# google/speedy

Measured on AMD Instinct MI355X. Metric: Msamples/s processed (16 kHz mono, 3.5x nonlinear), higher is better.
Workload: dtype int16 samples; f64 DFT, f32 features, int32 AMDF/OLA

## Files before the change

include/speedy_hip.h:

```cpp
#ifndef SPEEDY_HIP_H_
#define SPEEDY_HIP_H_
#include <stddef.h>
#include <stdint.h>
#ifdef __cplusplus
extern "C" {
#endif

#ifndef SPX_FEATURE_COUNT
#define SPX_FEATURE_COUNT 15
#endif

typedef struct spx_plan* spx_plan_t;

typedef struct {
  int64_t in_off;
  int64_t n_in;
  int64_t out_off;
  int64_t out_cap;
  int32_t channels;
  float speed;
  float nonlinear;
  float feedback;
} spx_stream_job;

typedef struct {
  float* tension;
  float* speed;
  float* features;
  float* spectrogram;
  float* normalized;
} spx_taps;

const char* spx_last_error(void);
int spx_abi_version(void);

spx_plan_t spx_plan_create(int sample_rate, int match_matlab);
void spx_plan_destroy(spx_plan_t plan);
int spx_plan_frame_step(spx_plan_t plan);
int spx_plan_window_size(spx_plan_t plan);
int spx_plan_fft_size(spx_plan_t plan);
int spx_plan_future(spx_plan_t plan);
int spx_plan_max_required(spx_plan_t plan);
int64_t spx_plan_frames(spx_plan_t plan, int64_t n_in);
int64_t spx_plan_out_capacity(spx_plan_t plan, int64_t n_in, float speed);
int64_t spx_plan_out_capacity_for(spx_plan_t plan, int64_t n_in, float speed, float nonlinear);

size_t spx_batch_workspace_bytes(spx_plan_t plan, const spx_stream_job* jobs, int n_streams);

int spx_batch_run(spx_plan_t plan, const spx_stream_job* jobs, int n_streams, const int16_t* in,
                  int16_t* out, int64_t* n_out, void* workspace, size_t workspace_bytes,
                  const spx_taps* taps, void* hip_stream);

int spx_batch_run_rate(spx_plan_t plan, const spx_stream_job* jobs, const float* rates, int n_streams, const int16_t* in,
                       int16_t* out, int64_t* n_out, void* workspace, size_t workspace_bytes,
                       const spx_taps* taps, void* hip_stream);
size_t spx_batch_workspace_bytes_rate(spx_plan_t plan, const spx_stream_job* jobs, const float* rates, int n_streams);
int64_t spx_plan_out_capacity_rate(spx_plan_t plan, int64_t n_in, float speed, float nonlinear, float rate);

int64_t spx_plan_map_rows(spx_plan_t plan, int64_t n_in, float nonlinear);
int spx_batch_run_map(spx_plan_t plan, const spx_stream_job* jobs, int n_streams, const int16_t* in,
                      int16_t* out, int64_t* n_out, int64_t* map, void* workspace, size_t workspace_bytes,
                      const spx_taps* taps, void* hip_stream);
int spx_map_lookup(spx_plan_t plan, const spx_stream_job* jobs, int n_streams, const int64_t* map, const int64_t* q_off,
                   const int64_t* q, int64_t* r, int inverse, void* hip_stream);
int spx_batch_run_rate_map(spx_plan_t plan, const spx_stream_job* jobs, const float* rates, int n_streams, const int16_t* in,
                           int16_t* out, int64_t* n_out, int64_t* map, void* workspace, size_t workspace_bytes,
                           const spx_taps* taps, void* hip_stream);
int spx_batch_run_float_map(spx_plan_t plan, const spx_stream_job* jobs, const float* rates, int n_streams, const float* in,
                            float* out, int64_t* n_out, int64_t* map, void* workspace, size_t workspace_bytes,
                            const spx_taps* taps, void* hip_stream);

typedef struct { int32_t out_at, a, b, n; } spx_edit_op;
typedef struct { int64_t in_off, out_off; int32_t channels, reserved; } spx_edit_track;
int64_t spx_plan_edit_ops(spx_plan_t plan, int64_t n_in, float speed, float nonlinear);
int spx_batch_run_edits(spx_plan_t plan, const spx_stream_job* jobs, int n_streams, const int16_t* in, int16_t* out, int64_t* n_out,
                        spx_edit_op* ops, const int64_t* ops_cap, int64_t* n_ops, void* workspace, size_t workspace_bytes,
                        const spx_taps* taps, void* hip_stream);
int spx_edit_replay(spx_plan_t plan, const spx_stream_job* jobs, int n_streams, const spx_edit_op* ops, const int64_t* ops_cap,
                    const int64_t* n_ops, const int64_t* n_out, const spx_edit_track* tracks, const int16_t* y_in, int16_t* y_out,
                    void* hip_stream);

typedef struct { int64_t a_off, b_off; int64_t path_off; int32_t n_a, n_b; } spx_dtw_job;
typedef struct { float cost, slope, local_mean, local_std; int32_t n_path, n_local; } spx_dtw_result;
size_t spx_dtw_workspace_bytes(const spx_dtw_job* jobs, int n_pairs, int dim);
int spx_batch_dtw(spx_plan_t plan, const spx_dtw_job* jobs, int n_pairs, int dim, int ld_a, int ld_b, int half_width,
                  const float* a, const float* b, spx_dtw_result* results, int32_t* path,
                  void* workspace, size_t workspace_bytes, void* hip_stream);

size_t spx_batch_workspace_bytes_twopass(spx_plan_t plan, const spx_stream_job* jobs, const double* seconds, int n_streams);
int64_t spx_plan_out_capacity_twopass(spx_plan_t plan, int64_t n_in, double want, float nonlinear);
int spx_batch_run_twopass(spx_plan_t plan, const spx_stream_job* jobs, const double* seconds, int n_streams, const int16_t* in,
                          int16_t* out, int64_t* n_out, int64_t* n_probe, float* speeds, void* workspace, size_t workspace_bytes,
                          const spx_taps* taps, void* hip_stream);
int spx_debug_last_twopass(void);

size_t spx_batch_workspace_bytes_float(spx_plan_t plan, const spx_stream_job* jobs, const float* rates, int n_streams);
int spx_batch_run_float(spx_plan_t plan, const spx_stream_job* jobs, const float* rates, int n_streams, const float* in,
                        float* out, int64_t* n_out, void* workspace, size_t workspace_bytes,
                        const spx_taps* taps, void* hip_stream);
int spx_float_to_short(const float* in, int16_t* out, size_t n, int nonlinear_scale, void* hip_stream);
int spx_short_to_float(const int16_t* in, float* out, size_t n, void* hip_stream);

int spx_batch_run_ahead(spx_plan_t plan, const spx_stream_job* jobs, int n_streams, const int16_t* in,
                        int16_t* out, int64_t* n_out, void* workspace, size_t workspace_bytes,
                        const spx_taps* taps, void* hip_stream);

int spx_batch_run_overlapped(spx_plan_t plan, const spx_stream_job* jobs, int n_streams, const int16_t* in,
                             int16_t* out, int64_t* n_out, void* workspace, size_t workspace_bytes,
                             const spx_taps* taps, void* hip_stream);

int spx_batch_run_ahead_when(spx_plan_t plan, const spx_stream_job* jobs, int n_streams, const int16_t* in,
                             int16_t* out, int64_t* n_out, void* workspace, size_t workspace_bytes,
                             const spx_taps* taps, void* hip_stream, void* in_ready_event);

typedef struct spx_pipeline* spx_pipeline_t;
#define SPX_PIPELINE_DEVICE_OUT 1u
#define SPX_PIPELINE_FLOAT 2u
spx_pipeline_t spx_pipeline_create(spx_plan_t plan, const spx_stream_job* jobs, int n_streams, int depth, unsigned flags);
spx_pipeline_t spx_pipeline_create_mixed(const spx_plan_t* plans, int n_plans, const spx_stream_job* jobs, const int* plan_index,
                                         int n_streams, int depth, unsigned flags);
void spx_pipeline_destroy(spx_pipeline_t p);
int spx_pipeline_depth(spx_pipeline_t p);
size_t spx_pipeline_input_values(spx_pipeline_t p);
int16_t* spx_pipeline_host_input(spx_pipeline_t p);
int64_t spx_pipeline_submit(spx_pipeline_t p, const int16_t* in, int in_is_device);
int64_t spx_pipeline_submit_jobs(spx_pipeline_t p, const spx_stream_job* jobs, const int16_t* in, int in_is_device);
int spx_pipeline_jobs_fit(spx_pipeline_t p, const spx_stream_job* jobs);
int spx_pipeline_input_consumed(spx_pipeline_t p, int64_t ticket);
int spx_pipeline_wait(spx_pipeline_t p, int64_t ticket, const int16_t** out, const int64_t** offsets, const int64_t** counts);

float* spx_pipeline_host_input_float(spx_pipeline_t p);
int64_t spx_pipeline_submit_float(spx_pipeline_t p, const float* in, int in_is_device);
int64_t spx_pipeline_submit_jobs_float(spx_pipeline_t p, const spx_stream_job* jobs, const float* in, int in_is_device);
int spx_pipeline_wait_float(spx_pipeline_t p, int64_t ticket, const float** out, const int64_t** offsets, const int64_t** counts);

spx_pipeline_t spx_pipeline_create_rate(spx_plan_t plan, const spx_stream_job* jobs, const float* rates, int n_streams, int depth,
                                        unsigned flags);
int spx_pipeline_jobs_fit_rate(spx_pipeline_t p, const spx_stream_job* jobs, const float* rates);
int64_t spx_pipeline_submit_jobs_rate(spx_pipeline_t p, const spx_stream_job* jobs, const float* rates, const int16_t* in,
                                      int in_is_device);
int64_t spx_pipeline_submit_jobs_rate_float(spx_pipeline_t p, const spx_stream_job* jobs, const float* rates, const float* in,
                                            int in_is_device);

void* spx_host_alloc(size_t bytes);
void spx_host_free(void* p);

int spx_batch_analyze(spx_plan_t plan, const spx_stream_job* jobs, int n_streams, const int16_t* in,
                      void* workspace, size_t workspace_bytes, const spx_taps* taps, void* hip_stream);
int spx_batch_walk(spx_plan_t plan, const spx_stream_job* jobs, int n_streams, const int16_t* in,
                   int16_t* out, int64_t* n_out, void* workspace, size_t workspace_bytes,
                   const spx_taps* taps, void* hip_stream);

size_t spx_batch_workspace_bytes_mixed(const spx_plan_t* plans, int n_plans, const spx_stream_job* jobs,
                                       const int* plan_index, int n_streams);
int spx_batch_run_mixed(const spx_plan_t* plans, int n_plans, const spx_stream_job* jobs, const int* plan_index,
                        int n_streams, const int16_t* in, int16_t* out, int64_t* n_out, void* workspace,
                        size_t workspace_bytes, void* hip_stream);

int spx_batch_run_mixed_taps(const spx_plan_t* plans, int n_plans, const spx_stream_job* jobs, const int* plan_index,
                             int n_streams, const int16_t* in, int16_t* out, int64_t* n_out, void* workspace,
                             size_t workspace_bytes, const spx_taps* taps, void* hip_stream);
int spx_batch_run_mixed_ahead(const spx_plan_t* plans, int n_plans, const spx_stream_job* jobs, const int* plan_index,
                              int n_streams, const int16_t* in, int16_t* out, int64_t* n_out, void* workspace,
                              size_t workspace_bytes, void* hip_stream);

void spx_set_timing(int enabled);
void spx_set_pipeline_chunks(int chunks);
void spx_set_concurrent(int on);
void spx_set_tension_form(int form);
int spx_debug_last_tension_form(void);
int spx_debug_last_call_chunks(void);
int spx_debug_last_lookup_grid(int* launches);
int spx_debug_last_replay_grid(int* launches);
int spx_debug_last_dtw_grid(int* launches);
int spx_timing_collect(double* sum_ms_analyze, double* sum_ms_walk, int* n_calls);
const char* spx_batch_kernel_names(spx_plan_t plan, int n_streams, int max_channels, int speedup_only);
const char* spx_batch_kernel_names_lean(spx_plan_t plan, int n_streams, int max_channels, int speedup_only);
int spx_debug_last_walk_form(void);
int spx_debug_kernel_vgprs(int which);
int spx_debug_walk_info(int sample_rate, int channels, int n_streams, int speedup_only, int short_jobs, int lean, int* out5);
int spx_debug_analysis_info(int sample_rate, int* out4);
int spx_debug_lane_consts(int sample_rate, void* out, double* tw, double* tw2, float* win);
int spx_debug_mode_resources(int sample_rate, int channels, int n_streams, int speedup_only, long long* out22);
long long spx_debug_fdiv_check(unsigned seed, unsigned denominators, int exp_lo, int exp_hi);
long long spx_debug_xfade_check(int n_lo, int n_hi);
long long spx_debug_arith_check(unsigned seed, unsigned threads, unsigned per_thread);
int spx_debug_select_check(const unsigned* d, int n_vectors, int p0, int n_lags, int max_period, int two_per_lane, int* lag_index,
                           unsigned* kmin);
int spx_debug_select_fold_check(const unsigned* d, int n_vectors, int p0, int n_lags, int want_max, int fresh, int* out3);
int spx_debug_log_check(unsigned first_block, unsigned end_block, unsigned long long* sums);
int spx_debug_last_call_concurrent(void);
double spx_timing_last_tension_ms(void);
double spx_timing_last_rate_ms(void);
double spx_timing_last_map_rows_ms(void);
double spx_timing_last_dtw_ms(void);
double spx_timing_last_dtw_tail_ms(void);

int spx_batch_read_steps(spx_plan_t plan, const spx_stream_job* jobs, int n_streams, const void* workspace,
                         int32_t* steps, void* hip_stream);
int spx_batch_read_steps_mixed(const spx_plan_t* plans, int n_plans, const spx_stream_job* jobs, const int* plan_index,
                               int n_streams, const void* workspace, int32_t* steps, void* hip_stream);

void* spx_device_alloc(size_t bytes);
void spx_device_free(void* p);
int spx_batch_pack_outputs(const spx_stream_job* jobs, int n_streams, const int16_t* out, const int64_t* n_out,
                           int16_t* packed, int64_t* offsets, void* hip_stream);
int spx_copy_to_device(void* dst, const void* src, size_t bytes, void* hip_stream);
int spx_copy_to_host(void* dst, const void* src, size_t bytes, void* hip_stream);
int spx_stream_synchronize(void* hip_stream);

#ifdef __cplusplus
}
#endif
#endif
```

speedy_amd/_lib.py:

```python
import ctypes as C
import os
import subprocess

_HERE = os.path.dirname(os.path.abspath(__file__))
LIB_PATH = os.environ.get("SPEEDY_HIP_LIB") or os.path.join(_HERE, "lib", "libspeedy_hip.so")
_LIB = None

c_short_p = C.POINTER(C.c_short)
c_float_p = C.POINTER(C.c_float)
c_int64_p = C.POINTER(C.c_int64)


class StreamJob(C.Structure):
    _fields_ = [("in_off", C.c_int64), ("n_in", C.c_int64), ("out_off", C.c_int64), ("out_cap", C.c_int64),
                ("channels", C.c_int32), ("speed", C.c_float), ("nonlinear", C.c_float), ("feedback", C.c_float)]


class Taps(C.Structure):
    _fields_ = [("tension", C.c_void_p), ("speed", C.c_void_p), ("features", C.c_void_p),
                ("spectrogram", C.c_void_p), ("normalized", C.c_void_p)]


class EditTrack(C.Structure):
    _fields_ = [("in_off", C.c_int64), ("out_off", C.c_int64), ("channels", C.c_int32), ("reserved", C.c_int32)]


class DtwJob(C.Structure):
    _fields_ = [("a_off", C.c_int64), ("b_off", C.c_int64), ("path_off", C.c_int64), ("n_a", C.c_int32), ("n_b", C.c_int32)]


TENSION_FN =C.CFUNCTYPE(None, C.c_void_p, C.c_int, C.c_float)
FEATURES_FN = C.CFUNCTYPE(None, C.c_void_p, C.c_int, c_float_p)

SYMBOLS = {
    "spx_last_error": (C.c_char_p, []),
    "spx_abi_version": (C.c_int, []),
    "spx_plan_create": (C.c_void_p, [C.c_int, C.c_int]),
    "spx_plan_destroy": (None, [C.c_void_p]),
    "spx_plan_frame_step": (C.c_int, [C.c_void_p]),
    "spx_plan_window_size": (C.c_int, [C.c_void_p]),
    "spx_plan_fft_size": (C.c_int, [C.c_void_p]),
    "spx_plan_future": (C.c_int, [C.c_void_p]),
    "spx_plan_max_required": (C.c_int, [C.c_void_p]),
    "spx_plan_frames": (C.c_int64, [C.c_void_p, C.c_int64]),
    "spx_plan_out_capacity": (C.c_int64, [C.c_void_p, C.c_int64, C.c_float]),
    "spx_plan_out_capacity_for": (C.c_int64, [C.c_void_p, C.c_int64, C.c_float, C.c_float]),
    "spx_batch_workspace_bytes": (C.c_size_t, [C.c_void_p, C.POINTER(StreamJob), C.c_int]),
    "spx_batch_run": (C.c_int, [C.c_void_p, C.POINTER(StreamJob), C.c_int, C.c_void_p, C.c_void_p, C.c_void_p,
                                C.c_void_p, C.c_size_t, C.POINTER(Taps), C.c_void_p]),
    "spx_batch_run_rate": (C.c_int, [C.c_void_p, C.POINTER(StreamJob), c_float_p, C.c_int, C.c_void_p, C.c_void_p, C.c_void_p,
                                     C.c_void_p, C.c_size_t, C.POINTER(Taps), C.c_void_p]),
    "spx_batch_workspace_bytes_rate": (C.c_size_t, [C.c_void_p, C.POINTER(StreamJob), c_float_p, C.c_int]),
    "spx_plan_out_capacity_rate": (C.c_int64, [C.c_void_p, C.c_int64, C.c_float, C.c_float, C.c_float]),
    "spx_plan_map_rows": (C.c_int64, [C.c_void_p, C.c_int64, C.c_float]),
    "spx_batch_run_map": (C.c_int, [C.c_void_p, C.POINTER(StreamJob), C.c_int, C.c_void_p, C.c_void_p, C.c_void_p, C.c_void_p,
                                    C.c_void_p, C.c_size_t, C.POINTER(Taps), C.c_void_p]),
    "spx_map_lookup": (C.c_int, [C.c_void_p, C.POINTER(StreamJob), C.c_int, C.c_void_p, C.c_void_p, C.c_void_p, C.c_void_p,
                                 C.c_int, C.c_void_p]),
    "spx_batch_run_rate_map": (C.c_int, [C.c_void_p, C.POINTER(StreamJob), c_float_p, C.c_int, C.c_void_p, C.c_void_p, C.c_void_p,
                                         C.c_void_p, C.c_void_p, C.c_size_t, C.POINTER(Taps), C.c_void_p]),
    "spx_batch_run_float_map": (C.c_int, [C.c_void_p, C.POINTER(StreamJob), c_float_p, C.c_int, C.c_void_p, C.c_void_p, C.c_void_p,
                                          C.c_void_p, C.c_void_p, C.c_size_t, C.POINTER(Taps), C.c_void_p]),
    "spx_plan_edit_ops": (C.c_int64, [C.c_void_p, C.c_int64, C.c_float, C.c_float]),
    "spx_batch_run_edits": (C.c_int, [C.c_void_p, C.POINTER(StreamJob), C.c_int, C.c_void_p, C.c_void_p, C.c_void_p, C.c_void_p,
                                      c_int64_p, C.c_void_p, C.c_void_p, C.c_size_t, C.POINTER(Taps), C.c_void_p]),
    "spx_edit_replay": (C.c_int, [C.c_void_p, C.POINTER(StreamJob), C.c_int, C.c_void_p, c_int64_p, C.c_void_p, C.c_void_p,
                                  C.POINTER(EditTrack), C.c_void_p, C.c_void_p, C.c_void_p]),
    "spx_dtw_workspace_bytes": (C.c_size_t, [C.POINTER(DtwJob), C.c_int, C.c_int]),
    "spx_batch_dtw": (C.c_int, [C.c_void_p, C.POINTER(DtwJob), C.c_int, C.c_int, C.c_int, C.c_int, C.c_int, C.c_void_p, C.c_void_p,
                                C.c_void_p, C.c_void_p, C.c_void_p, C.c_size_t, C.c_void_p]),
    "spx_debug_last_dtw_grid": (C.c_int, [C.POINTER(C.c_int)]),
    "spx_timing_last_dtw_ms": (C.c_double, []),
    "spx_timing_last_dtw_tail_ms": (C.c_double, []),
    "spx_batch_workspace_bytes_twopass":(C.c_size_t, [C.c_void_p, C.POINTER(StreamJob), C.POINTER(C.c_double), C.c_int]),
    "spx_plan_out_capacity_twopass": (C.c_int64, [C.c_void_p, C.c_int64, C.c_double, C.c_float]),
    "spx_batch_run_twopass": (C.c_int, [C.c_void_p, C.POINTER(StreamJob), C.POINTER(C.c_double), C.c_int, C.c_void_p, C.c_void_p,
                                        C.c_void_p, C.c_void_p, C.c_void_p, C.c_void_p, C.c_size_t, C.POINTER(Taps), C.c_void_p]),
    "spx_debug_last_twopass": (C.c_int, []),
    "spx_batch_workspace_bytes_float": (C.c_size_t, [C.c_void_p, C.POINTER(StreamJob), c_float_p, C.c_int]),
    "spx_batch_run_float": (C.c_int, [C.c_void_p, C.POINTER(StreamJob), c_float_p, C.c_int, C.c_void_p, C.c_void_p, C.c_void_p,
                                      C.c_void_p, C.c_size_t, C.POINTER(Taps), C.c_void_p]),
    "spx_float_to_short": (C.c_int, [C.c_void_p, C.c_void_p, C.c_size_t, C.c_int, C.c_void_p]),
    "spx_short_to_float": (C.c_int, [C.c_void_p, C.c_void_p, C.c_size_t, C.c_void_p]),
    "spx_batch_run_ahead": (C.c_int, [C.c_void_p, C.POINTER(StreamJob), C.c_int, C.c_void_p, C.c_void_p, C.c_void_p,
                                      C.c_void_p, C.c_size_t, C.POINTER(Taps), C.c_void_p]),
    "spx_batch_run_overlapped": (C.c_int, [C.c_void_p, C.POINTER(StreamJob), C.c_int, C.c_void_p, C.c_void_p, C.c_void_p,
                                           C.c_void_p, C.c_size_t, C.POINTER(Taps), C.c_void_p]),
    "spx_batch_run_ahead_when": (C.c_int, [C.c_void_p, C.POINTER(StreamJob), C.c_int, C.c_void_p, C.c_void_p, C.c_void_p,
                                           C.c_void_p, C.c_size_t, C.POINTER(Taps), C.c_void_p, C.c_void_p]),
    "spx_batch_workspace_bytes_mixed": (C.c_size_t, [C.POINTER(C.c_void_p), C.c_int, C.POINTER(StreamJob), C.POINTER(C.c_int), C.c_int]),
    "spx_batch_run_mixed": (C.c_int, [C.POINTER(C.c_void_p), C.c_int, C.POINTER(StreamJob), C.POINTER(C.c_int), C.c_int,
                                      C.c_void_p, C.c_void_p, C.c_void_p, C.c_void_p, C.c_size_t, C.c_void_p]),
    "spx_batch_run_mixed_ahead": (C.c_int, [C.POINTER(C.c_void_p), C.c_int, C.POINTER(StreamJob), C.POINTER(C.c_int), C.c_int,
                                      C.c_void_p, C.c_void_p, C.c_void_p, C.c_void_p, C.c_size_t, C.c_void_p]),
    "spx_batch_run_mixed_taps": (C.c_int, [C.POINTER(C.c_void_p), C.c_int, C.POINTER(StreamJob), C.POINTER(C.c_int), C.c_int,
                                           C.c_void_p, C.c_void_p, C.c_void_p, C.c_void_p, C.c_size_t, C.POINTER(Taps), C.c_void_p]),
    "spx_batch_read_steps": (C.c_int, [C.c_void_p, C.POINTER(StreamJob), C.c_int, C.c_void_p, C.POINTER(C.c_int32), C.c_void_p]),
    "spx_batch_read_steps_mixed": (C.c_int, [C.POINTER(C.c_void_p), C.c_int, C.POINTER(StreamJob), C.POINTER(C.c_int), C.c_int,
                                             C.c_void_p, C.POINTER(C.c_int32), C.c_void_p]),
    "spx_batch_analyze": (C.c_int, [C.c_void_p, C.POINTER(StreamJob), C.c_int, C.c_void_p, C.c_void_p,
                                    C.c_size_t, C.POINTER(Taps), C.c_void_p]),
    "spx_batch_walk": (C.c_int, [C.c_void_p, C.POINTER(StreamJob), C.c_int, C.c_void_p, C.c_void_p, C.c_void_p,
                                 C.c_void_p, C.c_size_t, C.POINTER(Taps), C.c_void_p]),
    "spx_set_timing": (None, [C.c_int]),
    "spx_set_pipeline_chunks": (None, [C.c_int]),
    "spx_set_concurrent": (None, [C.c_int]),
    "spx_set_tension_form": (None, [C.c_int]),
    "spx_debug_last_tension_form": (C.c_int, []),
    "spx_debug_last_call_chunks": (C.c_int, []),
    "spx_debug_last_lookup_grid": (C.c_int, [C.POINTER(C.c_int)]),
    "spx_debug_last_replay_grid": (C.c_int, [C.POINTER(C.c_int)]),
    "spx_timing_collect": (C.c_int, [C.POINTER(C.c_double), C.POINTER(C.c_double), C.POINTER(C.c_int)]),
    "spx_timing_last_tension_ms": (C.c_double, []),
    "spx_timing_last_rate_ms": (C.c_double, []),
    "spx_timing_last_map_rows_ms": (C.c_double, []),
    "spx_batch_kernel_names": (C.c_char_p, [C.c_void_p, C.c_int, C.c_int, C.c_int]),
    "spx_batch_kernel_names_lean": (C.c_char_p, [C.c_void_p, C.c_int, C.c_int, C.c_int]),
    "spx_debug_last_walk_form": (C.c_int, []),
    "spx_debug_kernel_vgprs": (C.c_int, [C.c_int]),
    "spx_debug_last_call_concurrent": (C.c_int, []),
    "spx_debug_fdiv_check": (C.c_longlong, [C.c_uint, C.c_uint, C.c_int, C.c_int]),
    "spx_debug_xfade_check": (C.c_longlong, [C.c_int, C.c_int]),
    "spx_debug_select_check": (C.c_int, [C.POINTER(C.c_uint), C.c_int, C.c_int, C.c_int, C.c_int, C.c_int, C.POINTER(C.c_int), C.POINTER(C.c_uint)]),
    "spx_debug_select_fold_check": (C.c_int, [C.POINTER(C.c_uint), C.c_int, C.c_int, C.c_int, C.c_int, C.c_int, C.POINTER(C.c_int)]),
    "spx_debug_arith_check": (C.c_longlong, [C.c_uint, C.c_uint, C.c_uint]),
    "spx_debug_log_check": (C.c_int, [C.c_uint, C.c_uint, C.POINTER(C.c_ulonglong)]),
    "spx_debug_walk_info": (C.c_int, [C.c_int, C.c_int, C.c_int, C.c_int, C.c_int, C.c_int, C.POINTER(C.c_int)]),
    "spx_debug_analysis_info": (C.c_int, [C.c_int, C.POINTER(C.c_int)]),
    "spx_debug_lane_consts": (C.c_int, [C.c_int, C.c_void_p, C.POINTER(C.c_double), C.POINTER(C.c_double), c_float_p]),
    "spx_debug_mode_resources": (C.c_int, [C.c_int, C.c_int, C.c_int, C.c_int, C.POINTER(C.c_longlong)]),
    "spx_pipeline_create": (C.c_void_p, [C.c_void_p, C.POINTER(StreamJob), C.c_int, C.c_int, C.c_uint]),
    "spx_pipeline_create_mixed": (C.c_void_p, [C.POINTER(C.c_void_p), C.c_int, C.POINTER(StreamJob), C.POINTER(C.c_int), C.c_int, C.c_int, C.c_uint]),
    "spx_pipeline_destroy": (None, [C.c_void_p]),
    "spx_pipeline_depth": (C.c_int, [C.c_void_p]),
    "spx_pipeline_input_values": (C.c_size_t, [C.c_void_p]),
    "spx_pipeline_host_input": (C.c_void_p, [C.c_void_p]),
    "spx_pipeline_submit": (C.c_int64, [C.c_void_p, C.c_void_p, C.c_int]),
    "spx_pipeline_submit_jobs": (C.c_int64, [C.c_void_p, C.POINTER(StreamJob), C.c_void_p, C.c_int]),
    "spx_pipeline_jobs_fit": (C.c_int, [C.c_void_p, C.POINTER(StreamJob)]),
    "spx_pipeline_input_consumed": (C.c_int, [C.c_void_p, C.c_int64]),
    "spx_pipeline_wait": (C.c_int, [C.c_void_p, C.c_int64, C.POINTER(C.c_void_p), C.POINTER(C.c_void_p), C.POINTER(C.c_void_p)]),
    "spx_pipeline_host_input_float": (C.c_void_p, [C.c_void_p]),
    "spx_pipeline_submit_float": (C.c_int64, [C.c_void_p, C.c_void_p, C.c_int]),
    "spx_pipeline_submit_jobs_float": (C.c_int64, [C.c_void_p, C.POINTER(StreamJob), C.c_void_p, C.c_int]),
    "spx_pipeline_wait_float": (C.c_int, [C.c_void_p, C.c_int64, C.POINTER(C.c_void_p), C.POINTER(C.c_void_p), C.POINTER(C.c_void_p)]),
    "spx_pipeline_create_rate": (C.c_void_p, [C.c_void_p, C.POINTER(StreamJob), c_float_p, C.c_int, C.c_int, C.c_uint]),
    "spx_pipeline_jobs_fit_rate": (C.c_int, [C.c_void_p, C.POINTER(StreamJob), c_float_p]),
    "spx_pipeline_submit_jobs_rate": (C.c_int64, [C.c_void_p, C.POINTER(StreamJob), c_float_p, C.c_void_p, C.c_int]),
    "spx_pipeline_submit_jobs_rate_float": (C.c_int64, [C.c_void_p, C.POINTER(StreamJob), c_float_p, C.c_void_p, C.c_int]),
    "spx_host_alloc": (C.c_void_p, [C.c_size_t]),
    "spx_host_free": (None, [C.c_void_p]),
    "spx_device_alloc": (C.c_void_p, [C.c_size_t]),
    "spx_device_free": (None, [C.c_void_p]),
    "spx_copy_to_device": (C.c_int, [C.c_void_p, C.c_void_p, C.c_size_t, C.c_void_p]),
    "spx_copy_to_host": (C.c_int, [C.c_void_p, C.c_void_p, C.c_size_t, C.c_void_p]),
    "spx_batch_pack_outputs": (C.c_int, [C.c_void_p, C.c_int, C.c_void_p, C.c_void_p, C.c_void_p, C.c_void_p, C.c_void_p]),
    "spx_stream_synchronize": (C.c_int, [C.c_void_p]),
    "sonicCreateStream": (C.c_void_p, [C.c_int, C.c_int]),
    "sonicDestroyStream": (None, [C.c_void_p]),
    "sonicWriteShortToStream": (C.c_int, [C.c_void_p, c_short_p, C.c_int]),
    "sonicReadShortFromStream": (C.c_int, [C.c_void_p, c_short_p, C.c_int]),
    "sonicWriteFloatToStream": (C.c_int, [C.c_void_p, c_float_p, C.c_int]),
    "sonicReadFloatFromStream": (C.c_int, [C.c_void_p, c_float_p, C.c_int]),
    "sonicSetRate": (None, [C.c_void_p, C.c_float]),
    "sonicSetSpeed": (None, [C.c_void_p, C.c_float]),
    "sonicFlushStream": (C.c_int, [C.c_void_p]),
    "sonicEnableNonlinearSpeedup": (None, [C.c_void_p, C.c_float]),
    "sonicSetDurationFeedbackStrength": (None, [C.c_void_p, C.c_float]),
    "getSonicBufferSize": (C.c_int, [C.c_void_p]),
    "sonicSpectrogramSize": (C.c_int, [C.c_void_p]),
    "sonicTensionCallback": (None, [C.c_void_p, TENSION_FN]),
    "getSonicTensionCallback": (C.c_void_p, [C.c_void_p]),
    "sonicSpeedCallback": (None, [C.c_void_p, TENSION_FN]),
    "getSonicSpeedCallback": (C.c_void_p, [C.c_void_p]),
    "sonicFeaturesCallback": (None, [C.c_void_p, FEATURES_FN]),
    "getSonicFeaturesCallback": (C.c_void_p, [C.c_void_p]),
    "sonicSpectrogramCallback": (None, [C.c_void_p, FEATURES_FN]),
    "getSonicSpectrogramCallback": (C.c_void_p, [C.c_void_p]),
    "sonicNormalizedSpectrogramCallback": (None, [C.c_void_p, FEATURES_FN]),
    "getSonicNormalizedSpectrogramCallback": (C.c_void_p, [C.c_void_p]),
    "sonicIntGetNumChannels": (C.c_int, [C.c_void_p]),
    "sonicIntGetSampleRate": (C.c_int, [C.c_void_p]),
    "sonicIntGetSpeed": (C.c_float, [C.c_void_p]),
    "sonicIntCreateStream": (C.c_void_p, [C.c_int, C.c_int]),
    "sonicIntDestroyStream": (None, [C.c_void_p]),
    "sonicIntSetSpeed": (None, [C.c_void_p, C.c_float]),
    "sonicIntSetRate": (None, [C.c_void_p, C.c_float]),
    "sonicIntWriteShortToStream": (C.c_int, [C.c_void_p, c_short_p, C.c_int]),
    "sonicIntWriteFloatToStream": (C.c_int, [C.c_void_p, c_float_p, C.c_int]),
    "sonicIntReadShortFromStream": (C.c_int, [C.c_void_p, c_short_p, C.c_int]),
    "sonicIntReadFloatFromStream": (C.c_int, [C.c_void_p, c_float_p, C.c_int]),
    "sonicIntFlushStream": (C.c_int, [C.c_void_p]),
    "sonicIntSamplesAvailable": (C.c_int, [C.c_void_p]),
    "sonicIntSetUserData": (None, [C.c_void_p, C.c_void_p]),
    "sonicIntGetUserData": (C.c_void_p, [C.c_void_p]),
    "speedyCreateStream": (C.c_void_p, [C.c_int]),
    "speedyDestroyStream": (None, [C.c_void_p]),
    "speedyInputFrameSize": (C.c_int, [C.c_void_p]),
    "speedyInputFrameStep": (C.c_int, [C.c_void_p]),
    "speedyFFTSize": (C.c_int, [C.c_void_p]),
    "speedyBinToFreq": (C.c_float, [C.c_void_p, C.c_int]),
    "speedyFreqToBin": (C.c_int, [C.c_void_p, C.c_float]),
    "speedyAddData": (None, [C.c_void_p, c_float_p, C.c_int64]),
    "speedyAddDataShort": (None, [C.c_void_p, c_short_p, C.c_int64]),
    "speedyComputeTension": (C.c_int, [C.c_void_p, C.c_int64, c_float_p]),
    "speedyComputeSpeedFromTension": (C.c_float, [C.c_float, C.c_float, C.c_float, C.c_void_p]),
    "speedyGetCurrentTime": (C.c_int64, [C.c_void_p]),
    "speedySpectrogram": (c_float_p, [C.c_void_p, c_float_p]),
    "speedyGetSpectrogram": (c_float_p, [C.c_void_p]),
    "speedyGetSpectrogramAtTime": (c_float_p, [C.c_void_p, C.c_int64]),
    "speedyGetNormalizedSpectrogram": (c_float_p, [C.c_void_p]),
    "speedyGetInternalState": (c_float_p, [C.c_void_p]),
    "speedyGetEnergyCompressed": (C.c_float, [C.c_void_p]),
    "speedyGetSpeechChanges": (C.c_float, [C.c_void_p]),
    "speedyHipHysteresisFuture": (C.c_int, [C.c_void_p]),
    "speedyHipHysteresisPast": (C.c_int, [C.c_void_p]),
    "speedyComputeSpectralDifference": (None, [C.c_void_p, c_float_p, c_float_p, C.c_int64]),
    "speedyComputeLocalEnergy": (None, [C.c_void_p, c_float_p, C.c_int64]),
    "speedySaveSpectrogramData": (None, [C.c_void_p, c_float_p, C.c_int64]),
    "speedyPreemphasisFilter": (None, [C.c_void_p, c_float_p, C.c_int]),
    "speedyEvaluateHysteresis": (C.c_float, [C.c_void_p, C.c_int64]),
    "speedyAddToHysteresisBuffer": (None, [C.c_void_p, C.c_float, C.c_int64]),
    "speedyGetInternalSpectrogram": (c_float_p, [C.c_void_p]),
    "speedyGetInternalNormalizedSpectrogram": (c_float_p, [C.c_void_p]),
    "speedyNormalizeByEnergy": (C.c_float, [c_float_p, c_float_p, C.c_int]),
    "CreateFirstOrderFilter": (C.c_void_p, [C.c_float]),
    "DesignFirstOrderLowpassFilter": (None, [C.c_void_p, C.c_float]),
    "IterateFirstOrderFilter": (C.c_float, [C.c_void_p, C.c_float]),
    "ResetFirstOrderFilter": (None, [C.c_void_p]),
    "DeleteFirstOrderFilter": (None, [C.c_void_p]),
    "speedyHipSetMatchMatlab": (None, [C.c_int]),
    "speedyHipCreateSonicStream": (C.c_void_p, [C.c_int, C.c_int, C.c_int]),
    "speedyHipSetCoalescing": (None, [C.c_int]),
    "speedyHipGetCoalescing": (C.c_int, []),
    "speedyHipCreateSonicStreamEx": (C.c_void_p, [C.c_int, C.c_int, C.c_int, C.c_int]),
    "speedyHipPoolStats": (None, [C.POINTER(C.c_ulonglong), C.POINTER(C.c_ulonglong)]),
    "sonicSamplesAvailable": (C.c_int, [C.c_void_p]),
    "speedyHipLastError": (C.c_char_p, []),
}


def build():
    subprocess.check_call(["make", "-s", "-C", os.path.join(_HERE, "csrc")])


def lib():
    global _LIB
    if _LIB is not None:
        return _LIB
    if not os.path.exists(LIB_PATH):
        raise RuntimeError(f"{LIB_PATH} is missing: run `python -c 'import __graft_entry__ as g; g.build()'` "
                           "(the product has no CPU fallback)")
    import torch
    L = C.CDLL(LIB_PATH)
    for name, (res, args) in SYMBOLS.items():
        if os.environ.get("SPEEDY_HIP_LIB") and not hasattr(L, name):
            continue
        fn = getattr(L, name)
        fn.restype = res
        fn.argtypes = args
    _LIB = L
# ... 2 lines not shown
```

speedy_amd/csrc/spx_analysis.hip:

```cpp
#include <stdlib.h>

#include "spx_internal.h"
#include "spx_walk_common.h"

#ifndef SPX_TF
#define SPX_TF 16
#endif

#ifdef SPX_STAMPS
__device__ unsigned long long g_spx_astamps[16];
#define ASTAMP_DECL unsigned long long as_last = __builtin_readcyclecounter(), as_acc[10] = {0,0,0,0,0,0,0,0,0,0};
#define ASTAMP(i) do { const unsigned long long t_ = __builtin_readcyclecounter(); as_acc[i] += t_ - as_last; as_last = t_; } while (0)
#define ASTAMP_FLUSH if (threadIdx.x == 0 && blockIdx.x == 7) for (int i_ = 0; i_ < 10; i_++) g_spx_astamps[i_] += as_acc[i_];
extern "C" void spx_debug_astamps(unsigned long long* out, int reset) {
  (void)hipMemcpyFromSymbol(out, HIP_SYMBOL(g_spx_astamps), sizeof(unsigned long long) * 16);
  if (reset) { unsigned long long z[16] = {0}; (void)hipMemcpyToSymbol(HIP_SYMBOL(g_spx_astamps), z, sizeof(z)); }
}
#else
#define ASTAMP_DECL
#define ASTAMP(i)
#define ASTAMP_FLUSH
#endif

#ifndef SPX_TF_SMALL
// ... 267 lines not shown
  } else if constexpr (R == 3) {
    const cplx t1 = {a[1].r + a[2].r, a[1].i + a[2].i};
    const cplx t2 = {spx_bf3h(a[0].r, t1.r), spx_bf3h(a[0].i, t1.i)};
    const cplx t3 = {S3_1 * (a[1].r - a[2].r), S3_1 * (a[1].i - a[2].i)};
    o[0] = {a[0].r + t1.r, a[0].i + t1.i};
    o[1] = {t2.r + t3.i, t2.i - t3.r};
    o[2] = {t2.r - t3.i, t2.i + t3.r};
  } else if constexpr (R == 4) {
    const cplx t0 = {a[0].r + a[2].r, a[0].i + a[2].i}, t1 = {a[0].r - a[2].r, a[0].i - a[2].i};
    const cplx t2 = {a[1].r + a[3].r, a[1].i + a[3].i}, t3 = {a[1].r - a[3].r, a[1].i - a[3].i};
    o[0] = {t0.r + t2.r, t0.i + t2.i};
    o[2] = {t0.r - t2.r, t0.i - t2.i};
    o[1] = {t1.r + t3.i, t1.i - t3.r};
    o[3] = {t1.r - t3.i, t1.i + t3.r};
  } else {
    const cplx t1 = {a[1].r + a[4].r, a[1].i + a[4].i}, t2 = {a[2].r + a[3].r, a[2].i + a[3].i};
    const cplx t3 = {a[1].r - a[4].r, a[1].i - a[4].i}, t4 = {a[2].r - a[3].r, a[2].i - a[3].i};
    o[0] = {(a[0].r + t1.r) + t2.r, (a[0].i + t1.i) + t2.i};
    const cplx m1 = {spx_bf5m(a[0].r, C5_1, t1.r, C5_2, t2.r), spx_bf5m(a[0].i, C5_1, t1.i, C5_2, t2.i)};
    const cplx m2 = {spx_bf5m(a[0].r, C5_2, t1.r, C5_1, t2.r), spx_bf5m(a[0].i, C5_2, t1.i, C5_1, t2.i)};
    const cplx n1 = {spx_bf5n(S5_1, t3.r, S5_2, t4.r), spx_bf5n(S5_1, t3.i, S5_2, t4.i)};
    const cplx n2 = {spx_bf5d(S5_2, t3.r, S5_1, t4.r), spx_bf5d(S5_2, t3.i, S5_1, t4.i)};
    o[1] = {m1.r + n1.i, m1.i - n1.r};
    o[4] = {m1.r - n1.i, m1.i + n1.r};
    o[2] = {m2.r + n2.i, m2.i - n2.r};
    o[3] = {m2.r - n2.i, m2.i + n2.r};
  }
}

template <int W> struct ct_plan { static constexpr int n = 0; };
template <> struct ct_plan<120> { static constexpr int n = 4; static constexpr int r[4] = {4, 2, 3, 5}; };
template <> struct ct_plan<180> { static constexpr int n = 4; static constexpr int r[4] = {4, 3, 3, 5}; };
template <> struct ct_plan<360> { static constexpr int n = 5; static constexpr int r[5] = {4, 2, 3, 3, 5}; };
template <> struct ct_plan<480> { static constexpr int n = 5; static constexpr int r[5] = {4, 4, 2, 3, 5}; };
template <> struct ct_plan<720> { static constexpr int n = 5; static constexpr int r[5] = {4, 4, 3, 3, 5}; };

template <int NPTS, int R, int S, class Load>
__device__ __forceinline__ void ct_stage(double* buf, const double2* __restrict__ twp, const int lane, Load load) {
  constexpr int SPAN = NPTS / R, NP = (SPAN + 63) / 64;
  constexpr bool LAST = (S * R == NPTS);
  cplx a[NP][R];
#pragma unroll
  for (int u = 0; u < NP; u++) {
#pragma unroll
    for (int i = 0; i < R; i++) a[u][i] = load(u, i);
  }
  wave_sync();
#pragma unroll
  for (int u = 0; u < NP; u++) {
    const int b = lane + 64 * u;
    if (b < SPAN) {
      cplx o[R];
      ct_bfly<R>(a[u], o);
      const int p = b / S, q = b - p * S;
      const int base = q + S * R * p, tp = S * p;
      st(buf, base, o[0]);
#pragma unroll
      for (int j = 1; j < R; j++) st(buf, base + j * S, LAST ? o[j] : cmul_tw(o[j], twp[j * tp]));
    }
  }
  wave_sync();
}
template <int NPTS, int R>
struct ct_from_buf {
  const double* buf;
  int lane;
  __device__ __forceinline__ cplx operator()(int u, int i) const {
    constexpr int SPAN = NPTS / R;
    const int b = (lane + 64 * u < SPAN) ? lane + 64 * u : 0;
    return ld(buf, b + i * SPAN);
  }
};

template <int W, int ST, int S>
__device__ __forceinline__ void ct_stages_from(double* buf, const double2* __restrict__ twp, const int lane) {
  if constexpr (ST < ct_plan<W>::n) {
    constexpr int R = ct_plan<W>::r[ST];
    ct_stage<W, R, S>(buf, twp, lane, ct_from_buf<W, R>{buf, lane});
    ct_stages_from<W, ST + 1, S * R>(buf, twp, lane);
  }
}

template <int NPTS, int R>
__device__ __forceinline__ void ct_stage_prime_last(double* buf, const int lane, const double (&wc)[R - 1], const double (&ws)[R - 1]) {
  constexpr int SPAN = NPTS / R, H = (R - 1) / 2;
  static_assert(SPAN <= 64, "one pass");
  if (lane < SPAN) {
    cplx a[R];
#pragma unroll
    for (int i = 0; i < R; i++) a[i] = ld(buf, lane + SPAN * i);
    cplx uu[H], vv[H];
    cplx B0 = a[0];
#pragma unroll
    for (int i = 1; i <= H; i++) {
      uu[i - 1] = {a[i].r + a[R - i].r, a[i].i + a[R - i].i};
      vv[i - 1] = {a[i].r - a[R - i].r, a[i].i - a[R - i].i};
      B0.r = B0.r + uu[i - 1].r; B0.i = B0.i + uu[i - 1].i;
    }
    st(buf, lane, B0);
#pragma unroll
    for (int jj = 1; jj <= H; jj++) {
      cplx Pj = a[0], Qj = {0.0, 0.0};
#pragma unroll
      for (int i = 1; i <= H; i++) {
        const double wx = wc[(i * jj) % R - 1], wy = ws[(i * jj) % R - 1];
        Pj.r = spx_acc(Pj.r, wx, uu[i - 1].r); Pj.i = spx_acc(Pj.i, wx, uu[i - 1].i);
        if (i == 1) { Qj.r = wy * vv[0].r; Qj.i = wy * vv[0].i; }
        else { Qj.r = spx_acc(Qj.r, wy, vv[i - 1].r); Qj.i = spx_acc(Qj.i, wy, vv[i - 1].i); }
      }
      st(buf, lane + SPAN * jj, cplx{Pj.r - Qj.i, Pj.i + Qj.r});
      st(buf, lane + SPAN * (R - jj), cplx{Pj.r + Qj.i, Pj.i - Qj.r});
    }
  }
  wave_sync();
}

template <class T>
__device__ __forceinline__ const T* per_frame(const T* p) {
  asm volatile("" : "+s"(p));
  return p;
}
__device__ __forceinline__ double uniform_f64(double v) {
  return __longlong_as_double(((long long)__builtin_amdgcn_readfirstlane((int)(__double_as_longlong(v) >> 32)) << 32) |
                              (unsigned)__builtin_amdgcn_readfirstlane((int)__double_as_longlong(v)));
}

#ifdef SPX_PREEMPH_V1
__device__ __forceinline__ float spx_preemph_win_f32(double md, double mpd, float w) {
  const float x = (float)(md / 32768.0), xp = (float)(mpd / 32768.0);
  const float y = (float)(1.0 * (double)x - 0.97 * (double)xp);
  return y * w;
}
#else
__device__ __forceinline__ float spx_preemph_win_f32(double md, double mpd, float w15) {
  const float yy = (float)(md - 0.97 * mpd);
  return yy * w15;
}
#endif
__device__ __forceinline__ double spx_preemph_win(double md, double mpd, float w) { return (double)spx_preemph_win_f32(md, mpd, w); }
__device__ __forceinline__ cplx packed_point(const short* fr, int n, int j, int prev0, float w0, float w1) {
  const int i0 = 2 * n;
  const int m0 = fr[i0], m1 = fr[i0 + 1];
  const int mp0 = (i0 > 0) ? (int)fr[i0 - 1] : ((j > 0) ? (int)fr[prev0] : 0);
  const double d0 = (double)m0;
  return {spx_preemph_win(d0, (double)mp0, w0 * SPX_WIN_SCALE), spx_preemph_win((double)m1, d0, w1 * SPX_WIN_SCALE)};
}

#ifndef SPX_AN_W_330
#define SPX_AN_W_330 3
#endif
#ifndef SPX_AN_W_BIG
#define SPX_AN_W_BIG 2
#endif
template <int TF, int WCT>
__global__ void __launch_bounds__(SPX_BLOCK, an_lean_layout(TF, WCT) ? 5 : (WCT == 240 || WCT == 120 || WCT == 180) ? 4 : WCT == 330 ? SPX_AN_W_330 : (WCT == 661 || WCT == 720) ? SPX_AN_W_BIG : (WCT == 480 || WCT == 360) ? 2 : 1)
spx_analysis_kernel(SpxPlanDev P, const SpxStreamDev* __restrict__ streams, int n_streams,
                    const int16_t* __restrict__ in_base, SpxFrameRec* __restrict__ rec, SpxTapsDev taps,
                    const int* __restrict__ tile_order, int* tile_flags, const float* __restrict__ frames,
                    int frame_mode) {
  extern __shared__ __attribute__((aligned(16))) unsigned char lds[];
  const int W = WCT ? WCT : P.W, B = P.B, N = 2 * W;
  const int tid = threadIdx.x, lane = tid & 63, wave = tid >> 6;

  const int tile = tile_order ? tile_order[blockIdx.x] : (int)blockIdx.x;
  int lo = 0, hi = n_streams - 1;
  while (lo < hi) {
    int mid = (lo + hi + 1) >> 1;
    if (streams[mid].first_tile <= tile) lo = mid; else hi = mid - 1;
  }
  const SpxStreamDev S = streams[lo];
  const int T = S.n_frames;
  const int j0 = S.frame_begin + (tile - S.first_tile) * TF;
  const int j1 = min(j0 + TF, T);
  const int C = S.channels;
  const int16_t* __restrict__ in = in_base + S.in_off;

  constexpr bool LT = an_lean_layout(TF, WCT);
  const size_t wb = work_bytes(W, TF, WCT != 0, (WCT != 0) ? 4 : P.dft_waves);
  const size_t mags_b = (((size_t)(TF + 1) * spx_mag_stride(W) * sizeof(float)) + 15) & ~(size_t)15;
  const size_t small_b = (((size_t)3 * (TF + 1) * sizeof(float)) + 15) & ~(size_t)15;
  double* work = reinterpret_cast<double*>(LT ? lds + an_lt_front_bytes() : lds);
  float* mags = reinterpret_cast<float*>(LT ? lds : lds + wb);
  float* fE = reinterpret_cast<float*>(LT ? lds + an_lt_front_bytes() + an_lt_small_off() : lds + wb + mags_b);
  float* fThr = fE + (TF + 1);
  float* fInv = fThr + (TF + 1);
  const int MS = spx_mag_stride(W);
  unsigned char* const terms_base = reinterpret_cast<unsigned char*>(work) + (LT ? an_lt_terms_off() : 0);
  static_assert(!LT || an_lt_terms_off() + (size_t)2 * SPX_TF * (spx_cb(SPX_TF) + 1) * sizeof(double) + SPX_LOG_LDS_BYTES <= (size_t)4 * 2 * 240 * sizeof(double),
                "two blocks of log terms and the log table inside the work area (terms_bytes, work_bytes)");

  const double* ltw = P.tw;
  const double* ltw2 = P.tw2;
  short* smono = reinterpret_cast<short*>(LT ? lds + an_lt_front_bytes() + wb : lds + wb + mags_b + small_b);
  const bool direct = LT && frame_mode == 3;

  double* bufA = work + (size_t)wave * (WCT != 0 ? 2 : 4) * W;
  double* bufB = (WCT != 0) ? bufA : bufA + 2 * W;

  const int jfirst = (j0 > 0) ? j0 - 1 : 0;
  const int64_t sbase = (int64_t)jfirst * B;
  const int nstage = (j1 - jfirst) * B + (W - B);
  if (frames != nullptr || direct) {
  } else if (C == 1) {
    const int16_t* __restrict__ src = in + sbase;
    for (int k0 = tid; k0 < nstage; k0 += 8 * SPX_BLOCK) {
      short v[8];
#pragma unroll
      for (int u = 0; u < 8; u++) { const int k = k0 + u * SPX_BLOCK; v[u] = (k < nstage) ? src[k] : (short)0; }
#pragma unroll
      for (int u = 0; u < 8; u++) { const int k = k0 + u * SPX_BLOCK; if (k < nstage) smono[k] = v[u]; }
    }
  } else {
    for (int k = tid; k < nstage; k += SPX_BLOCK) smono[k] = (short)mono_sample(in, sbase + k, C);
  }
  __syncthreads();

  ASTAMP_DECL
  if constexpr (LT) {
    const int b = lane;
    const bool on60 = b < 60, on48 = b < 48;
    const int bb = on60 ? b : 0;
    typedef double lc_v2d __attribute__((ext_vector_type(2)));
    typedef float lc_v4f __attribute__((ext_vector_type(4)));
    typedef const __attribute__((address_space(1))) lc_v2d* lc_ptr;
    typedef const __attribute__((address_space(1))) lc_v4f* lc_ptr4;
    const double2* const lc0 = reinterpret_cast<const double2*>(P.lane_consts);
    auto take6 = [&](auto fr, int j, int (&m)[6]) {
      m[0] = fr[0]; m[1] = fr[1]; m[2] = fr[120]; m[3] = fr[121]; m[5] = fr[119];
      m[4] = fr[bb > 0 ? -1 : (240 - B) - 1];
      if (bb == 0 && j == 0) m[4] = 0;
    };
    auto fetch6 = [&](int s, int (&m)[6]) {
      const int j = j0 - 1 + s;
      if (s <= TF && j >= 0 && j < j1) take6(in + (int64_t)j * B + 2 * bb, j, m);
    };
    int nx[6] = {0, 0, 0, 0, 0, 0};
    float hold[4] = {0.0f, 0.0f, 0.0f, 0.0f};
    if (direct) fetch6(wave, nx);
    for (int s = wave; s <= TF; s += 4) {
      const int j = j0 - 1 + s;
      const bool keep = s + 4 > TF;
      float* mrow = mags + (size_t)s * MS;
      if (j < 0 || j >= j1) {
        if (!keep) for (int k = lane; k < 240; k += SPX_WAVE) mrow[k] = 0.0f;
#pragma unroll
        for (int u = 0; u < 4; u++) hold[u] = 0.0f;
        if (direct) fetch6(s + 4, nx);
        continue;
      }
      int ln = lane;
      asm volatile("" : "+v"(ln));
      __builtin_assume(ln >= 0 && ln < SPX_WAVE);
      const lc_ptr lcb[4] = {(lc_ptr)per_frame(lc0), (lc_ptr)per_frame(lc0 + 256), (lc_ptr)per_frame(lc0 + 512), (lc_ptr)per_frame(lc0 + 768)};
      typedef const __attribute__((address_space(1))) unsigned char* lc_bytes;
      unsigned lane_off = 16u * (unsigned)lane;
      asm volatile("" : "+v"(lane_off));
      auto lc = [&](int c) -> double2 {
        const lc_v2d v = *(lc_ptr)((lc_bytes)lcb[c >> 2] + lane_off + 1024u * (unsigned)(c & 3));
        return make_double2(v.x, v.y);
      };
      int m[6];
      if (direct) {
#pragma unroll
        for (int u = 0; u < 6; u++) m[u] = nx[u];
      } else {
        take6(smono + (size_t)(j - jfirst) * B + 2 * bb, j, m);
      }
      {
        const lc_v4f wn = *(lc_ptr4)((lc_bytes)lcb[SPX_LC_WN >> 2] + lane_off + 1024u * (SPX_LC_WN & 3));
        const double2 w1a = lc(SPX_LC_W1 + 0), w1b = lc(SPX_LC_W1 + 1), w1c = lc(SPX_LC_W1 + 2);
        if (on60) {
          const double d0 = (double)m[0], d2 = (double)m[2];
          const cplx a0 = {spx_preemph_win(d0, (double)m[4], wn.x), spx_preemph_win((double)m[1], d0, wn.y)},
                     a1 = {spx_preemph_win(d2, (double)m[5], wn.z), spx_preemph_win((double)m[3], d2, wn.w)};
          const cplx b0 = {a0.r + a1.r, a0.i + a1.i}, b2 = {a0.r - a1.r, a0.i - a1.i};
          const cplx b1 = {a0.r + a1.i, a0.i - a1.r}, b3 = {a0.r - a1.i, a0.i + a1.r};
          st(bufA, 4 * ln, b0);
          st(bufA, 4 * ln + 1, cmul_tw(b1, w1a));
          st(bufA, 4 * ln + 2, cmul_tw(b2, w1b));
          st(bufA, 4 * ln + 3, cmul_tw(b3, w1c));
        }
      }
      {
        const double2 w2a = lc(SPX_LC_W2 + 0), w2b = lc(SPX_LC_W2 + 1), w2c = lc(SPX_LC_W2 + 2);
        wave_sync();
        ASTAMP(0);
        if (on60) {
          const cplx a0 = ld(bufA, ln), a1 = ld(bufA, ln + 60), a2 = ld(bufA, ln + 120), a3 = ld(bufA, ln + 180);
          wave_sync();
          const cplx t0 = {a0.r + a2.r, a0.i + a2.i}, t1 = {a0.r - a2.r, a0.i - a2.i};
          const cplx t2 = {a1.r + a3.r, a1.i + a3.i}, t3 = {a1.r - a3.r, a1.i - a3.i};
          const cplx b0 = {t0.r + t2.r, t0.i + t2.i}, b2 = {t0.r - t2.r, t0.i - t2.i};
          const cplx b1 = {t1.r + t3.i, t1.i - t3.r}, b3 = {t1.r - t3.i, t1.i + t3.r};
          const int o = (ln & 3) + 16 * (ln >> 2);
          st(bufB, o, b0);
          st(bufB, o + 4, cmul_tw(b1, w2a));
          st(bufB, o + 8, cmul_tw(b2, w2b));
          st(bufB, o + 12, cmul_tw(b3, w2c));
        }
      }
      {
        double2 w3[2][2];
#pragma unroll
        for (int u = 0; u < 2; u++) { w3[u][0] = lc(SPX_LC_W3 + 2 * u); w3[u][1] = lc(SPX_LC_W3 + 2 * u + 1); }
        wave_sync();
        cplx q0[2], q1[2], q2[2];
#pragma unroll
        for (int u = 0; u < 2; u++) {
          const int b3i = (ln + 64 * u < 80) ? ln + 64 * u : 0;
          q0[u] = ld(bufB, b3i); q1[u] = ld(bufB, b3i + 80); q2[u] = ld(bufB, b3i + 160);
        }
        wave_sync();
#pragma unroll
        for (int u = 0; u < 2; u++) {
          const int b3i = ln + 64 * u;
          if (b3i < 80) {
            const cplx a0 = q0[u], a1 = q1[u], a2 = q2[u];
            const cplx t1 = {a1.r + a2.r, a1.i + a2.i};
            const cplx t2 = {spx_bf3h(a0.r, t1.r), spx_bf3h(a0.i, t1.i)};
            const cplx t3 = {S3_1 * (a1.r - a2.r), S3_1 * (a1.i - a2.i)};
            const cplx b0 = {a0.r + t1.r, a0.i + t1.i};
            const cplx b1 = {t2.r + t3.i, t2.i - t3.r}, b2 = {t2.r - t3.i, t2.i + t3.r};
            const int o = (b3i & 15) + 48 * (b3i >> 4);
            st(bufA, o, b0);
            st(bufA, o + 16, cmul_tw(b1, w3[u][0]));
            st(bufA, o + 32, cmul_tw(b2, w3[u][1]));
          }
        }
      }
      wave_sync();
      if (on48) {
        const cplx a0 = ld(bufA, ln), a1 = ld(bufA, ln + 48), a2 = ld(bufA, ln + 96), a3 = ld(bufA, ln + 144),
                   a4 = ld(bufA, ln + 192);
        wave_sync();
        const cplx t1 = {a1.r + a4.r, a1.i + a4.i}, t2 = {a2.r + a3.r, a2.i + a3.i};
        const cplx t3 = {a1.r - a4.r, a1.i - a4.i}, t4 = {a2.r - a3.r, a2.i - a3.i};
        const cplx b0 = {(a0.r + t1.r) + t2.r, (a0.i + t1.i) + t2.i};
        const cplx m1 = {spx_bf5m(a0.r, C5_1, t1.r, C5_2, t2.r), spx_bf5m(a0.i, C5_1, t1.i, C5_2, t2.i)};
        const cplx m2 = {spx_bf5m(a0.r, C5_2, t1.r, C5_1, t2.r), spx_bf5m(a0.i, C5_2, t1.i, C5_1, t2.i)};
        const cplx n1 = {spx_bf5n(S5_1, t3.r, S5_2, t4.r), spx_bf5n(S5_1, t3.i, S5_2, t4.i)};
        const cplx n2 = {spx_bf5d(S5_2, t3.r, S5_1, t4.r), spx_bf5d(S5_2, t3.i, S5_1, t4.i)};
        const cplx b1 = {m1.r + n1.i, m1.i - n1.r}, b4 = {m1.r - n1.i, m1.i + n1.r};
        const cplx b2 = {m2.r + n2.i, m2.i - n2.r}, b3 = {m2.r - n2.i, m2.i + n2.r};
        st(bufB, ln, b0);
        st(bufB, ln + 48, b1);
        st(bufB, ln + 96, b2);
        st(bufB, ln + 144, b3);
        st(bufB, ln + 192, b4);
      }
      if (direct) fetch6(s + 4, nx);
      double2 wu[4];
#pragma unroll
      for (int u = 0; u < 4; u++) wu[u] = lc(SPX_LC_WU + u);
      wave_sync();
      ASTAMP(1);
      float* spec_out = taps.spectrogram ? taps.spectrogram + (size_t)(S.frame_off + j) * 480 : nullptr;
#pragma unroll
      for (int u = 0; u < 4; u++) {
        const int k = ln + 64 * u;
        if (k < 240) {
          const int k2 = (k == 0) ? 0 : 240 - k;
          const cplx a = ld(bufB, k), c = ld(bufB, k2);
          const double b_r = c.r, b_i = -c.i;
          const float mag = spx_untangle_mag(a.r, a.i, b_r, b_i, wu[u]);
          hold[u] = mag;
          if (!keep) mrow[k] = mag;
          if (spec_out) {
            spec_out[k] = mag;
            if (k > 0) spec_out[480 - k] = mag;
            else spec_out[240] = (float)__builtin_fabs(a.r - a.i);
          }
        }
      }
      wave_sync();
      ASTAMP(2);
    }
    __syncthreads();
    {
      float* mrow = mags + (size_t)(wave == 0 ? TF : TF - 4 + wave) * MS;
#pragma unroll
      for (int u = 0; u < 4; u++) {
        const int k = lane + 64 * u;
        if (k < 240) mrow[k] = hold[u];
      }
    }
  } else if constexpr (WCT == 240) {
    const double2* twp = reinterpret_cast<const double2*>(P.tw);
    const double2* tw2p = reinterpret_cast<const double2*>(P.tw2);
    const int b = lane;
    const bool on60 = b < 60, on48 = b < 48;
    const int bb = on60 ? b : 0;
    double2 w1[3], w2[3], w3[2][2], wu[4];
    float wn[4];
#pragma unroll
    for (int j = 1; j < 4; j++) { w1[j - 1] = twp[bb * j]; w2[j - 1] = twp[4 * (bb >> 2) * j]; }
#pragma unroll
    for (int u = 0; u < 2; u++) {
      const int b3 = lane + 64 * u, p3 = (b3 < 80) ? (b3 >> 4) : 0;
      w3[u][0] = twp[16 * p3];
      w3[u][1] = twp[32 * p3];
    }
#pragma unroll
    for (int u = 0; u < 4; u++) { const int k = lane + 64 * u; wu[u] = tw2p[k < 240 ? k : 0]; }
    wn[0] = P.window[2 * bb]; wn[1] = P.window[2 * bb + 1]; wn[2] = P.window[2 * bb + 120]; wn[3] = P.window[2 * bb + 121];
#pragma unroll
    for (int k = 0; k < 4; k++) wn[k] *= SPX_WIN_SCALE;
    for (int s = wave; s <= TF; s += 4) {
      const int j = j0 - 1 + s;
      float* mrow = mags + (size_t)s * MS;
      if (j < 0 || j >= j1) {
        for (int k = lane; k < 240; k += SPX_WAVE) mrow[k] = 0.0f;
        continue;
      }
      const short* fr = smono + (size_t)(j - jfirst) * B;
      if (on60) {
        const int i0 = 2 * b, i1 = 2 * b + 120;
        const int m0 = fr[i0], m1 = fr[i0 + 1], m2 = fr[i1], m3 = fr[i1 + 1];
        const int mp0 = (i0 > 0) ? (int)fr[i0 - 1] : ((j > 0) ? (int)fr[(240 - B) - 1] : 0);
        const int mp2 = fr[i1 - 1];
        const double d0 = (double)m0, d2 = (double)m2;
        const cplx a0 = {spx_preemph_win(d0, (double)mp0, wn[0]), spx_preemph_win((double)m1, d0, wn[1])},
                   a1 = {spx_preemph_win(d2, (double)mp2, wn[2]), spx_preemph_win((double)m3, d2, wn[3])};
        const cplx b0 = {a0.r + a1.r, a0.i + a1.i}, b2 = {a0.r - a1.r, a0.i - a1.i};
        const cplx b1 = {a0.r + a1.i, a0.i - a1.r}, b3 = {a0.r - a1.i, a0.i + a1.r};
        st(bufA, 4 * b, b0);
        st(bufA, 4 * b + 1, cmul_tw(b1, w1[0]));
        st(bufA, 4 * b + 2, cmul_tw(b2, w1[1]));
        st(bufA, 4 * b + 3, cmul_tw(b3, w1[2]));
      }
      wave_sync();
      ASTAMP(0);
      if (on60) {
        const cplx a0 = ld(bufA, b), a1 = ld(bufA, b + 60), a2 = ld(bufA, b + 120), a3 = ld(bufA, b + 180);
        wave_sync();
        const cplx t0 = {a0.r + a2.r, a0.i + a2.i}, t1 = {a0.r - a2.r, a0.i - a2.i};
        const cplx t2 = {a1.r + a3.r, a1.i + a3.i}, t3 = {a1.r - a3.r, a1.i - a3.i};
        const cplx b0 = {t0.r + t2.r, t0.i + t2.i}, b2 = {t0.r - t2.r, t0.i - t2.i};
        const cplx b1 = {t1.r + t3.i, t1.i - t3.r}, b3 = {t1.r - t3.i, t1.i + t3.r};
        const int o = (b & 3) + 16 * (b >> 2);
        st(bufB, o, b0);
        st(bufB, o + 4, cmul_tw(b1, w2[0]));
        st(bufB, o + 8, cmul_tw(b2, w2[1]));
        st(bufB, o + 12, cmul_tw(b3, w2[2]));
      }
      wave_sync();
      {
        cplx q0[2], q1[2], q2[2];
#pragma unroll
        for (int u = 0; u < 2; u++) {
          const int b3i = (lane + 64 * u < 80) ? lane + 64 * u : 0;
          q0[u] = ld(bufB, b3i); q1[u] = ld(bufB, b3i + 80); q2[u] = ld(bufB, b3i + 160);
        }
        wave_sync();
#pragma unroll
        for (int u = 0; u < 2; u++) {
          const int b3i = lane + 64 * u;
          if (b3i < 80) {
            const cplx a0 = q0[u], a1 = q1[u], a2 = q2[u];
            const cplx t1 = {a1.r + a2.r, a1.i + a2.i};
            const cplx t2 = {spx_bf3h(a0.r, t1.r), spx_bf3h(a0.i, t1.i)};
            const cplx t3 = {S3_1 * (a1.r - a2.r), S3_1 * (a1.i - a2.i)};
            const cplx b0 = {a0.r + t1.r, a0.i + t1.i};
            const cplx b1 = {t2.r + t3.i, t2.i - t3.r}, b2 = {t2.r - t3.i, t2.i + t3.r};
            const int o = (b3i & 15) + 48 * (b3i >> 4);
            st(bufA, o, b0);
            st(bufA, o + 16, cmul_tw(b1, w3[u][0]));
            st(bufA, o + 32, cmul_tw(b2, w3[u][1]));
          }
        }
      }
      wave_sync();
      if (on48) {
        const cplx a0 = ld(bufA, b), a1 = ld(bufA, b + 48), a2 = ld(bufA, b + 96), a3 = ld(bufA, b + 144),
                   a4 = ld(bufA, b + 192);
        wave_sync();
        const cplx t1 = {a1.r + a4.r, a1.i + a4.i}, t2 = {a2.r + a3.r, a2.i + a3.i};
        const cplx t3 = {a1.r - a4.r, a1.i - a4.i}, t4 = {a2.r - a3.r, a2.i - a3.i};
        const cplx b0 = {(a0.r + t1.r) + t2.r, (a0.i + t1.i) + t2.i};
        const cplx m1 = {spx_bf5m(a0.r, C5_1, t1.r, C5_2, t2.r), spx_bf5m(a0.i, C5_1, t1.i, C5_2, t2.i)};
        const cplx m2 = {spx_bf5m(a0.r, C5_2, t1.r, C5_1, t2.r), spx_bf5m(a0.i, C5_2, t1.i, C5_1, t2.i)};
        const cplx n1 = {spx_bf5n(S5_1, t3.r, S5_2, t4.r), spx_bf5n(S5_1, t3.i, S5_2, t4.i)};
        const cplx n2 = {spx_bf5d(S5_2, t3.r, S5_1, t4.r), spx_bf5d(S5_2, t3.i, S5_1, t4.i)};
        const cplx b1 = {m1.r + n1.i, m1.i - n1.r}, b4 = {m1.r - n1.i, m1.i + n1.r};
        const cplx b2 = {m2.r + n2.i, m2.i - n2.r}, b3 = {m2.r - n2.i, m2.i + n2.r};
        st(bufB, b, b0);
        st(bufB, b + 48, b1);
        st(bufB, b + 96, b2);
        st(bufB, b + 144, b3);
        st(bufB, b + 192, b4);
      }
      wave_sync();
      ASTAMP(1);
      float* spec_out = taps.spectrogram ? taps.spectrogram + (size_t)(S.frame_off + j) * 480 : nullptr;
#pragma unroll
      for (int u = 0; u < 4; u++) {
        const int k = lane + 64 * u;
        if (k < 240) {
          const int k2 = (k == 0) ? 0 : 240 - k;
          const cplx a = ld(bufB, k), c = ld(bufB, k2);
          const double b_r = c.r, b_i = -c.i;
          const float mag = spx_untangle_mag(a.r, a.i, b_r, b_i, wu[u]);
          mrow[k] = mag;
          if (spec_out) {
            spec_out[k] = mag;
            if (k > 0) spec_out[480 - k] = mag;
            else spec_out[240] = (float)__builtin_fabs(a.r - a.i);
          }
        }
      }
      wave_sync();
      ASTAMP(2);
    }
  } else if constexpr (WCT == 330) {
    const double2* twp = reinterpret_cast<const double2*>(P.tw);
    const double2* tw2p = reinterpret_cast<const double2*>(P.tw2);
    double2 w1[3], w2[2][2];
    float wn[3][2];
#pragma unroll
    for (int u = 0; u < 3; u++) {
      const int b1 = (lane + 64 * u < 165) ? lane + 64 * u : 0;
      w1[u] = twp[b1];
      wn[u][0] = P.window[2 * b1] * SPX_WIN_SCALE; wn[u][1] = P.window[2 * b1 + 1] * SPX_WIN_SCALE;
    }
#pragma unroll
    for (int u = 0; u < 2; u++) {
      const int p2 = (lane + 64 * u < 110) ? ((lane + 64 * u) >> 1) : 0;
      w2[u][0] = twp[2 * p2];
      w2[u][1] = twp[4 * p2];
    }
    double wc[10], ws[10];
#pragma unroll
    for (int k = 1; k <= 10; k++) {
      const double2 w = twp[k * 30];
      wc[k - 1] = __longlong_as_double(((long long)__builtin_amdgcn_readfirstlane((int)(__double_as_longlong(w.x) >> 32)) << 32) |
                                       (unsigned)__builtin_amdgcn_readfirstlane((int)__double_as_longlong(w.x)));
      ws[k - 1] = __longlong_as_double(((long long)__builtin_amdgcn_readfirstlane((int)(__double_as_longlong(w.y) >> 32)) << 32) |
                                       (unsigned)__builtin_amdgcn_readfirstlane((int)__double_as_longlong(w.y)));
// ... 487 lines not shown
      const float eps = 2.2204e-16f;
      const float nc = cur * fInv[sl], nl = last * fInv[sl - 1];
      const float ratio = spx_fdiv32(nc + eps, nl + eps);
      term = __builtin_fabs(log_of_ratio(ratio));
    }
    return term;
  };
  auto write_rec = [&](int f, float lsd) {
    const float lowthr = (float)(0.04 * (double)1.41421f);
    const float e = fE[f + 1];
    SpxFrameRec r;
    r.energy = e;
    r.lsd = (e <= lowthr) ? 0.0f : lsd;
    rec[S.frame_off + j0 + f] = r;
  };
  if (taps.normalized) {
    for (int idx = tid; idx < nfr * W; idx += SPX_BLOCK) {
      const int f = idx / W, i = idx - f * W;
      const int j = j0 + f;
      const int row = j + (S.unit_time0 ? 0 : 1);
      if (row < T + (S.unit_time0 ? 1 : 0))
        taps.normalized[(size_t)(S.frame_off + row) * W + i] = mags[(size_t)(f + 1) * MS + i] * fInv[f + 1];
    }
    if (S.unit_time0) {
    } else if (j0 == 0) {
      for (int i = tid; i < W; i += SPX_BLOCK) taps.normalized[(size_t)S.frame_off * W + i] = 0.0f;
    } else if (j0 == S.frame_begin) {
      for (int i = tid; i < W; i += SPX_BLOCK)
        taps.normalized[(size_t)(S.frame_off + j0) * W + i] = mags[i] * fInv[0];
    }
  }
  if constexpr (WCT != 0) {
    constexpr int CB = spx_cb(TF);
    constexpr int CBS = CB + 1;
    static_assert(TF * CB == 2 * (SPX_BLOCK - SPX_WAVE), "two terms per lane of waves 1..3 and block");
    double* tblk = reinterpret_cast<double*>(terms_base);
    constexpr int NBLK = (WCT - 1 + CB - 1) / CB;
    float lsd = 0.0f;
    int fi[2], ci[2];
    bool ok[2];
#ifndef SPX_TERMS_V1
    const float* rowc[2];
    const float* rowl[2];
    float thrv[2], invc[2], invl[2];
#endif
#pragma unroll
    for (int t = 0; t < 2; t++) {
      const int it = tid - SPX_WAVE + t * (SPX_BLOCK - SPX_WAVE);
      fi[t] = wave > 0 ? it / CB : 0;
      ci[t] = wave > 0 ? it - fi[t] * CB : 0;
      ok[t] = wave > 0 && fi[t] < nfr;
#ifndef SPX_TERMS_V1
      const int fl = ok[t] ? fi[t] : 0;
      rowc[t] = mags + (size_t)(fl + 1) * MS;
      rowl[t] = mags + (size_t)fl * MS;
      thrv[t] = fThr[fl + 1];
      invc[t] = fInv[fl + 1];
      invl[t] = fInv[fl];
#endif
    }
    for (int k = 0; k <= NBLK; k++) {
      if (wave > 0) {
        if (k < NBLK) {
          double* tb = tblk + (size_t)(k & 1) * TF * CBS;
          bool gate[2];
          float xr[2];
#pragma unroll
          for (int t = 0; t < 2; t++) {
            const int i = 1 + k * CB + ci[t];
            const bool in = ok[t] && i < WCT;
#ifdef SPX_TERMS_V1
            const int fl = in ? fi[t] : 0, il = in ? i : 1;
            const float cur = mags[(size_t)(fl + 1) * MS + il], last = mags[(size_t)fl * MS + il];
            const float thr = fThr[fl + 1];
            const float fic = fInv[fl + 1], fil = fInv[fl];
#else
            const int il = (i < WCT) ? i : 1;
            const float cur = rowc[t][il], last = rowl[t][il];
            const float thr = thrv[t], fic = invc[t], fil = invl[t];
#endif
            gate[t] = in && cur > thr && last > thr;
            const float eps = 2.2204e-16f;
            const float nc = cur * fic, nl = last * fil;
            const float ratio = spx_fdiv32(nc + eps, nl + eps);
            xr[t] = gate[t] ? ratio : 2.0f;
          }
#ifdef SPX_LOG_V1
          const spx_log_parts p0 = spx_log_main((double)xr[0]), p1 = spx_log_main((double)xr[1]);
          const double t0 = gate[0] ? __builtin_fabs(spx_log_finish(p0, (double)xr[0])) : 0.0;
          const double t1 = gate[1] ? __builtin_fabs(spx_log_finish(p1, (double)xr[1])) : 0.0;
#else
          const double l0 = log_of_ratio(xr[0]), l1 = log_of_ratio(xr[1]);
          const double t0 = gate[0] ? __builtin_fabs(l0) : 0.0;
          const double t1 = gate[1] ? __builtin_fabs(l1) : 0.0;
#endif
          if (ok[0]) tb[fi[0] * CBS + ci[0]] = t0;
          if (ok[1]) tb[fi[1] * CBS + ci[1]] = t1;
        }
      } else if (k > 0 && tid < nfr) {
        const double* tb = tblk + (size_t)((k - 1) & 1) * TF * CBS + tid * CBS;
        const int i0 = 1 + (k - 1) * CB;
        __builtin_amdgcn_s_setprio(3);
        (void)i0;
        static_assert(CB % 8 == 0, "batches of eight");
        double tv[8];
#pragma unroll
        for (int u = 0; u < 8; u++) tv[u] = tb[u];
#pragma unroll
        for (int c = 0; c < CB; c += 8) {
          double nx[8];
          if (c + 8 < CB) {
#pragma unroll
            for (int u = 0; u < 8; u++) nx[u] = tb[c + 8 + u];
          }
#pragma unroll
          for (int u = 0; u < 8; u++) lsd = (float)((double)lsd + tv[u]);
          if (c + 8 < CB) {
#pragma unroll
            for (int u = 0; u < 8; u++) tv[u] = nx[u];
          }
        }
        __builtin_amdgcn_s_setprio(0);
      }
      ASTAMP(6);
      __syncthreads();
      ASTAMP(7);
    }
    if (tid < nfr) write_rec(tid, lsd);
  } else {
  double* terms = work;
  for (int idx = tid; idx < nfr * (W - 1); idx += SPX_BLOCK) {
    const int f = idx / (W - 1);
    const int i = 1 + (idx - f * (W - 1));
    terms[(size_t)f * (W + 1) + i] = log_term(f, i);
  }
  __syncthreads();
  ASTAMP(6);

  if (tid < nfr) {
    const double* trow = terms + (size_t)tid * (W + 1);
    float lsd = 0.0f;
    int i = 1;
    for (; i + 8 <= W; i += 8) {
      double tv[8];
#pragma unroll
      for (int u = 0; u < 8; u++) tv[u] = trow[i + u];
#pragma unroll
      for (int u = 0; u < 8; u++) lsd = (float)((double)lsd + tv[u]);
    }
    for (; i < W; i++) lsd = (float)((double)lsd + trow[i]);
    write_rec(tid, lsd);
  }
  }
  if (tile_flags) {
    asm volatile("s_waitcnt vmcnt(0)" ::: "memory");
    __syncthreads();
    if (tid == 0) {
      __builtin_amdgcn_fence(__ATOMIC_RELEASE, "agent");
      asm volatile("s_waitcnt vmcnt(0)" ::: "memory");
      __hip_atomic_store(&tile_flags[tile], 1, __ATOMIC_RELAXED, __HIP_MEMORY_SCOPE_AGENT);
    }
  }
  ASTAMP(7);
  ASTAMP_FLUSH
}

__global__ void spx_arith_check_kernel(unsigned seed, unsigned per_thread, unsigned long long* bad) {
  unsigned long long st = (unsigned long long)seed * 0x9E3779B97F4A7C15ull + (blockIdx.x * blockDim.x + threadIdx.x) * 0xD1B54A32D192ED03ull + 1;
  auto next = [&]() { st ^= st >> 12; st ^= st << 25; st ^= st >> 27; return st * 0x2545F4914F6CDD1Dull; };
  unsigned long long miss = 0;
  for (unsigned i = 0; i < per_thread; i++) {
    const unsigned long long a = next(), b = next(), c = next();
    const float fn = __uint_as_float((unsigned)((127 - 53 + (a % 57)) << 23) | (unsigned)((a >> 8) & 0x7fffff));
    const float fd = __uint_as_float((unsigned)((127 - 53 + (b % 57)) << 23) | (unsigned)((b >> 8) & 0x7fffff));
    if (__float_as_uint(spx_fdiv32(fn, fd)) != __float_as_uint(fn / fd)) miss++;
    const long long fb = ((long long)(1023 - 21 + (c % 20)) << 52) | (long long)((c >> 8) & 0xfffffffffffffll) | ((c >> 63) ? (1ll << 63) : 0);
    const double f = __longlong_as_double(fb);
    if (__double_as_longlong(spx_fdiv64(f, 2.0 + f)) != __double_as_longlong(f / (2.0 + f))) miss++;
    const long long xb = ((long long)(1023 - 800 + (a >> 33) % 1811) << 52) | (long long)((b >> 10) & 0xfffffffffffffll);
    const double x = ((c & 1023) == 0) ? 0.0 : __longlong_as_double(xb);
    if (__float_as_uint(spx_sqrt64_to_f32(x)) != __float_as_uint((float)__builtin_sqrt(x))) miss++;
  }
  if (miss) atomicAdd(bad, miss);
}
extern "C" long long spx_debug_arith_check(unsigned seed, unsigned threads, unsigned per_thread) {
  unsigned long long* d = nullptr;
  unsigned long long h = 0;
  if (hipMalloc(&d, sizeof(h)) != hipSuccess) return -1;
  if (hipMemcpy(d, &h, sizeof(h), hipMemcpyHostToDevice) != hipSuccess) { (void)hipFree(d); return -1; }
  const unsigned blocks = (threads + 255) / 256;
  hipLaunchKernelGGL(spx_arith_check_kernel, dim3(blocks), dim3(256), 0, nullptr, seed, per_thread, d);
  const bool ok = hipDeviceSynchronize() == hipSuccess && hipMemcpy(&h, d, sizeof(h), hipMemcpyDeviceToHost) == hipSuccess;
  (void)hipFree(d);
  return ok ? (long long)h : -1;
}

__global__ void __launch_bounds__(256) spx_log_check_kernel(unsigned first_block, unsigned long long* __restrict__ sums) {
#ifndef SPX_LOG_V1
  __shared__ SpxLogEntry tab[128];
  __shared__ unsigned long long acc;
  if (threadIdx.x < 128) reinterpret_cast<uint4*>(tab)[threadIdx.x] = reinterpret_cast<const uint4*>(spx_log_table_dev)[threadIdx.x];
  if (threadIdx.x == 0) acc = 0;
  __syncthreads();
  const unsigned b = first_block + blockIdx.x;
  unsigned long long sum = 0;
  for (unsigned i = threadIdx.x; i < (1u << 20); i += 256) {
    const float x = __uint_as_float((b << 20) | i);
    sum += (unsigned long long)__double_as_longlong(spx_log_v2_f32(x, tab));
  }
  atomicAdd(&acc, sum);
  __syncthreads();
  if (threadIdx.x == 0) sums[b] = acc;
#endif
}
extern "C" int spx_debug_log_check(unsigned first_block, unsigned end_block, unsigned long long* sums) {
#ifdef SPX_LOG_V1
  (void)first_block; (void)end_block; (void)sums;
  return -3;
#else
  if (first_block < 8) first_block = 8;
  if (end_block > 2040) end_block = 2040;
  if (!sums || first_block >= end_block) return -1;
  unsigned long long* d = nullptr;
  if (hipMalloc(&d, 2040 * sizeof(unsigned long long)) != hipSuccess) return -1;
  bool ok = hipMemset(d, 0, 2040 * sizeof(unsigned long long)) == hipSuccess;
  if (ok) hipLaunchKernelGGL(spx_log_check_kernel, dim3(end_block - first_block), dim3(256), 0, nullptr, first_block, d);
  ok = ok && hipDeviceSynchronize() == hipSuccess && hipMemcpy(sums, d, 2040 * sizeof(unsigned long long), hipMemcpyDeviceToHost) == hipSuccess;
  (void)hipFree(d);
  return ok ? 0 : -1;
#endif
}

SpxKernelChoice spx_analysis_select(int tile_frames, int ctw) {
#define AN_K(TFV, WV) SpxKernelChoice{"spx_analysis_kernel", reinterpret_cast<const void*>(spx_analysis_kernel<TFV, WV>), SPX_BLOCK, 2, {TFV, WV}}
  static_assert(std::is_same<decltype(spx_analysis_kernel<SPX_TF_TINY, 0>), SpxAnalysisArgs>::value, "SpxAnalysisArgs is the kernel's argument list");
  if (tile_frames == SPX_TF_TINY) return AN_K(SPX_TF_TINY, 0);
  if (tile_frames == SPX_TF_SMALL)
    return ctw == 240 ? AN_K(SPX_TF_SMALL, 240) : ctw == 330 ? AN_K(SPX_TF_SMALL, 330) : ctw == 720 ? AN_K(SPX_TF_SMALL, 720)
         : ctw == 661 ? AN_K(SPX_TF_SMALL, 661) : ctw == 120 ? AN_K(SPX_TF_SMALL, 120) : AN_K(SPX_TF_SMALL, 0);
  return ctw == 240 ? AN_K(SPX_TF, 240) : ctw == 330 ? AN_K(SPX_TF, 330) : ctw == 120 ? AN_K(SPX_TF, 120) : ctw == 360 ? AN_K(SPX_TF, 360)
       : ctw == 180 ? AN_K(SPX_TF, 180) : ctw == 480 ? AN_K(SPX_TF, 480) : AN_K(SPX_TF, 0);
#undef AN_K
}
int spx_analysis_vgprs(const SpxPlanDev& P, int* scratch_bytes) {
  return spx_kernel_vgprs(spx_analysis_select(P.tile_frames, plan_ct_window(P)).fn, scratch_bytes);
}

void spx_launch_analysis(const SpxPlanDev& P, const SpxStreamDev* streams, int n_streams, int n_tiles,
                         const int16_t* in, SpxFrameRec* rec, SpxTapsDev taps, const int* tile_order, int* tile_flags,
                         bool mono, hipStream_t st) {
  if (n_tiles <= 0) return;
  const int ctw = plan_ct_window(P);
  const bool direct = mono && an_lean_layout(P.tile_frames, ctw);
  SpxLaunch<SpxAnalysisArgs>::go(spx_analysis_select(P.tile_frames, ctw), n_tiles, analysis_lds_bytes(P, ctw, direct), st, P, streams,
                                 n_streams, in, rec, taps, tile_order, tile_flags, nullptr, direct ? 3 : 0);
}

void spx_launch_analysis_frames(const SpxPlanDev& P, const SpxStreamDev* streams, int n_tiles, const float* frames,
                                bool preemph, SpxFrameRec* rec, SpxTapsDev taps, hipStream_t st) {
  if (n_tiles <= 0) return;
  SpxPlanDev Q = P;
  if (Q.tile_frames != SPX_TF_SMALL && Q.tile_frames != SPX_TF_TINY) Q.tile_frames = SPX_TF;
  SpxLaunch<SpxAnalysisArgs>::go(spx_analysis_select(Q.tile_frames, 0), n_tiles, analysis_lds_bytes(Q, 0, false), st, Q, streams, 1, nullptr, rec,
                                 taps, nullptr, nullptr, frames, preemph ? 1 : 2);
}
```

speedy_amd/csrc/spx_diag.hip:

```cpp
#include "spx_engine.h"

extern "C" {
static const char* kernel_names(spx_plan_t plan, int n_streams, int max_channels, int speedup_only, bool lean);
const char* spx_batch_kernel_names(spx_plan_t plan, int n_streams, int max_channels, int speedup_only) {
  return kernel_names(plan, n_streams, max_channels, speedup_only, false);
}
const char* spx_batch_kernel_names_lean(spx_plan_t plan, int n_streams, int max_channels, int speedup_only) {
  return kernel_names(plan, n_streams, max_channels, speedup_only, true);
}
static const char* kernel_names(spx_plan_t plan, int n_streams, int max_channels, int speedup_only, bool lean) {
  static thread_local char buf[256];
  const SpxPlanDev& d = plan->dev;
  const SpxWalkConfig c = spx_walk_config(d, {.n_streams = n_streams, .max_channels = max_channels, .speedup_only = speedup_only != 0,
                                              .any_speed = speedup_only == 0, .lean = lean});
  size_t at = 0;
  auto put = [&](const SpxKernelChoice& k) {
    at += snprintf(buf + at, sizeof(buf) - at, "%s<", k.name);
    for (int i = 0; i < k.n_targs; i++) at += snprintf(buf + at, sizeof(buf) - at, i ? ", %d" : "%d", k.targs[i]);
    at += snprintf(buf + at, sizeof(buf) - at, ">");
  };
  put(spx_analysis_select(d.tile_frames, spx_analysis_ct_window(d)));
  at += snprintf(buf + at, sizeof(buf) - at, ";spx_tension_kernel;");
  put(c.kernel);
  return buf;
}

int spx_debug_last_call_concurrent(void) { return g_last_concurrent.load(std::memory_order_relaxed); }
int spx_debug_kernel_vgprs(int which) {
  if (which == 0) return spx_tension_vgprs();
  const int rate = (which == 2 || which == 4) ? 22050 : 16000;
  const SpxPlanDev* P = spx_internal_shared_plan(rate, 0);
  if (!P) return -1;
  switch (which) {
    case 1: return spx_walk_vgprs(*P, {.n_streams = 256, .max_channels = 1, .speedup_only = true}, nullptr);
    case 2: return spx_walk_vgprs(*P, {.n_streams = 256, .max_channels = 1, .speedup_only = true, .lean = true}, nullptr);
    case 3: case 4: return spx_analysis_vgprs(*P);
    case 5: return spx_walk_vgprs(*P, {.n_streams = 256, .max_channels = 2, .speedup_only = true}, nullptr);
    default: return -1;
  }
}

int spx_debug_walk_info(int sample_rate, int channels, int n_streams, int speedup_only, int short_jobs, int lean, int* out) {
  const SpxPlanDev* P = spx_internal_shared_plan(sample_rate, 0);
  if (!P || !out) return -1;
  const SpxWalkConfig c = spx_walk_config(*P, {.n_streams = n_streams, .max_channels = channels, .speedup_only = speedup_only != 0,
                                               .any_speed = speedup_only == 0, .short_jobs = short_jobs != 0, .lean = lean != 0});
  int scratch = -1;
  out[0] = spx_kernel_vgprs(c.kernel.fn, &scratch);
  out[1] = scratch;
  out[2] = (int)c.lds;
  out[3] = c.fast_kernel ? 16 * c.nwm + c.nwc : 0;
  out[4] = c.waves;
  return 0;
}
int spx_debug_analysis_info(int sample_rate, int* out) {
  const SpxPlanDev* P = spx_internal_shared_plan(sample_rate, 0);
  if (!P || !out) return -1;
  int scratch = -1;
  out[0] = spx_analysis_vgprs(*P, &scratch);
  out[1] = scratch;
  out[2] = (int)spx_analysis_lds_bytes(*P, true);
  out[3] = P->dft_waves;
  return 0;
}

void spx_set_timing(int enabled) { g_timing = enabled != 0; }
void spx_set_concurrent(int on) { g_concurrent = on != 0; }
void spx_set_tension_form(int form) { g_tension_form = form != 0; }
int spx_debug_last_tension_form(void) { return g_last_tension_form.load(std::memory_order_relaxed); }
int spx_debug_last_call_chunks(void) { return g_last_call_chunks.load(std::memory_order_relaxed); }
void spx_set_pipeline_chunks(int chunks) { g_chunks_set = true; g_chunks = chunks < 1 ? 1 : (chunks > SPX_MAX_CHUNKS ? SPX_MAX_CHUNKS : chunks); }
static double g_last_tension_ms = 0.0, g_last_rate_ms = 0.0, g_last_map_rows_ms = 0.0, g_last_dtw_ms = 0.0, g_last_dtw_tail_ms = 0.0;
double spx_timing_last_tension_ms(void) { return g_last_tension_ms; }
double spx_timing_last_rate_ms(void) { return g_last_rate_ms; }
double spx_timing_last_map_rows_ms(void) { return g_last_map_rows_ms; }
double spx_timing_last_dtw_ms(void) { return g_last_dtw_ms; }
double spx_timing_last_dtw_tail_ms(void) { return g_last_dtw_tail_ms; }
int spx_timing_collect(double* sum_ms_analyze, double* sum_ms_walk, int* n_calls) {
  std::lock_guard<std::mutex> g(g_tmu);
  double a = 0, w = 0, t = 0, r = 0, m = 0, df = 0, dt = 0;
  for (auto& ev : g_ev_pending) {
    HIPCHK(hipEventSynchronize(ev.b));
    float ms = 0;
    HIPCHK(hipEventElapsedTime(&ms, ev.a, ev.b));
    if (ev.kind == 0) a += ms; else if (ev.kind == 1) w += ms; else if (ev.kind == 3) r += ms; else if (ev.kind == 4) m += ms;
    else if (ev.kind == 5) df += ms; else if (ev.kind == 6) dt += ms; else t += ms;
    g_ev_free.push_back(ev.a);
    g_ev_free.push_back(ev.b);
  }
  g_ev_pending.clear();
  g_last_tension_ms = t;
  g_last_rate_ms = r;
  g_last_map_rows_ms = m;
  g_last_dtw_ms = df + dt;
  g_last_dtw_tail_ms = dt;
  if (sum_ms_analyze) *sum_ms_analyze = a;
  if (sum_ms_walk) *sum_ms_walk = w;
  if (n_calls) *n_calls = g_calls_pending;
  g_calls_pending = 0;
  return 0;
}

void* spx_device_alloc(size_t bytes) {
  void* p = nullptr;
  if (hipMalloc(&p, bytes ? bytes : 1) != hipSuccess) { fail(-2, "spx_device_alloc failed"); return nullptr; }
  return p;
}
void spx_device_free(void* p) { if (p) (void)hipFree(p); }
int spx_copy_to_device(void* dst, const void* src, size_t bytes, void* hs) {
  HIPCHK(hipMemcpyAsync(dst, src, bytes, hipMemcpyHostToDevice, static_cast<hipStream_t>(hs)));
  return 0;
}
}

__global__ void __launch_bounds__(256)
spx_pack_offsets_kernel(const int64_t* __restrict__ n_out, const int* __restrict__ channels,
                        const int64_t* __restrict__ caps, int n, int64_t* __restrict__ offsets) {
  __shared__ int64_t sh[256];
  __shared__ int64_t carry;
  const int t = threadIdx.x;
  if (t == 0) carry = 0;
  __syncthreads();
  for (int i0 = 0; i0 < n; i0 += 256) {
    const int i = i0 + t;
    int64_t v = 0;
    if (i < n) {
      const int64_t k = n_out[i];
      int64_t f = (k == INT64_MIN ? 0 : (k > 0 ? k : -k));
      if (f > caps[i]) f = caps[i];
      v = f * channels[i];
    }
    sh[t] = v;
    __syncthreads();
    for (int d = 1; d < 256; d <<= 1) {
      const int64_t add = (t >= d) ? sh[t - d] : 0;
      __syncthreads();
      sh[t] += add;
      __syncthreads();
    }
    const int64_t base = carry;
    if (i < n) offsets[i] = base + sh[t] - v;
    __syncthreads();
    if (t == 255) carry = base + sh[255];
    __syncthreads();
  }
  if (t == 0) offsets[n] = carry;
}
__global__ void __launch_bounds__(256)
spx_pack_copy_kernel(const int16_t* __restrict__ out, const int64_t* __restrict__ out_offs,
                     const int64_t* __restrict__ offsets, int16_t* __restrict__ packed) {
  const int i = blockIdx.x;
  const int16_t* src = out + out_offs[i];
  int16_t* dst = packed + offsets[i];
  const int64_t cnt = offsets[i + 1] - offsets[i];
  const int64_t stride = (int64_t)gridDim.y * 256 * 8;
  for (int64_t e0 = ((int64_t)blockIdx.y * 256 + threadIdx.x); e0 < cnt; e0 += stride) {
    int16_t v[8];
#pragma unroll
    for (int u = 0; u < 8; u++) { const int64_t e = e0 + (int64_t)u * gridDim.y * 256; v[u] = (e < cnt) ? src[e] : (int16_t)0; }
#pragma unroll
    for (int u = 0; u < 8; u++) { const int64_t e = e0 + (int64_t)u * gridDim.y * 256; if (e < cnt) dst[e] = v[u]; }
  }
}

extern "C" {
int spx_batch_pack_outputs(const spx_stream_job* jobs, int n, const int16_t* out, const int64_t* n_out, int16_t* packed,
                           int64_t* offsets, void* hs) {
  if (!jobs || n <= 0 || !out || !n_out || !packed || !offsets) return fail(-1, "spx_batch_pack_outputs: bad arguments");
  hipStream_t st = static_cast<hipStream_t>(hs);
  const size_t need = (size_t)n * (2 * sizeof(int64_t) + sizeof(int));
  void* d_tab = nullptr;
  if (hipMallocAsync(&d_tab, need, st) != hipSuccess) return fail(-2, "spx_batch_pack_outputs: allocation failed");
  static thread_local SpxStage G;
  if (G.acquire(need)) return -2;
  unsigned char* h = static_cast<unsigned char*>(G.p);
  int64_t* h_off = reinterpret_cast<int64_t*>(h);
  int64_t* h_cap = h_off + n;
  int* h_ch = reinterpret_cast<int*>(h + (size_t)n * 2 * sizeof(int64_t));
  for (int i = 0; i < n; i++) { h_off[i] = jobs[i].out_off; h_cap[i] = jobs[i].out_cap; h_ch[i] = jobs[i].channels; }
  HIPCHK(hipMemcpyAsync(d_tab, h, need, hipMemcpyHostToDevice, st));
  if (G.release(st)) return -2;
  const int64_t* d_off = reinterpret_cast<const int64_t*>(d_tab);
  const int* d_ch = reinterpret_cast<const int*>(static_cast<unsigned char*>(d_tab) + (size_t)n * 2 * sizeof(int64_t));
  hipLaunchKernelGGL(spx_pack_offsets_kernel, dim3(1), dim3(256), 0, st, n_out, d_ch, d_off + n, n, offsets);
  hipLaunchKernelGGL(spx_pack_copy_kernel, dim3(n, 4), dim3(256), 0, st, out, d_off, offsets, packed);
  (void)hipFreeAsync(d_tab, st);
  HIPCHK(hipGetLastError());
  return 0;
}

int spx_copy_to_host(void* dst, const void* src, size_t bytes, void* hs) {
  HIPCHK(hipMemcpyAsync(dst, src, bytes, hipMemcpyDeviceToHost, static_cast<hipStream_t>(hs)));
  return 0;
}
int spx_stream_synchronize(void* hs) {
  HIPCHK(hipStreamSynchronize(static_cast<hipStream_t>(hs)));
  return 0;
}

}
```

speedy_amd/csrc/spx_engine.h:

```cpp
#pragma once
#include <algorithm>
#include <math.h>
#include <cmath>
#include <stdio.h>
#include <string.h>

#include <atomic>
#include <map>
#include <mutex>
#include <string>
#include <vector>

#include "../../include/speedy_hip.h"
#include "spx_internal.h"
#include "spx_jobs.h"
#include "spx_mode.h"

#ifndef M_PI
#define M_PI 3.14159265358979323846
#endif


extern thread_local std::string g_spx_err;
static inline int fail(int code, const std::string& msg) {
  g_spx_err = msg;
  return code;
}
#define HIPCHK(expr)                                                                          \
  do {                                                                                        \
    hipError_t e_ = (expr);                                                                   \
    if (e_ != hipSuccess) return fail(-2, std::string(#expr) + ": " + hipGetErrorString(e_)); \
  } while (0)

#include <dlfcn.h>
struct SpxRoctx {
  int (*push)(const char*) = nullptr;
  int (*pop)() = nullptr;
  SpxRoctx() {
    void* h = dlopen("librocprofiler-sdk-roctx.so", RTLD_LAZY | RTLD_LOCAL);
    if (!h) h = dlopen("librocprofiler-sdk-roctx.so.1", RTLD_LAZY | RTLD_LOCAL);
    if (!h) h = dlopen("libroctx64.so", RTLD_LAZY | RTLD_LOCAL);
    if (!h) h = dlopen("libroctx64.so.4", RTLD_LAZY | RTLD_LOCAL);
    if (h) {
      push = reinterpret_cast<int (*)(const char*)>(dlsym(h, "roctxRangePushA"));
      pop = reinterpret_cast<int (*)()>(dlsym(h, "roctxRangePop"));
      if (!push || !pop) { push = nullptr; pop = nullptr; }
    }
  }
};
struct SpxRange {
  static SpxRoctx& api() { static SpxRoctx a; return a; }
  explicit SpxRange(const char* name) { if (api().push) api().push(name); }
  ~SpxRange() { if (api().pop) api().pop(); }
};

#define SPX_MAX_CHUNKS 16
#define SPX_MAX_WALK_STREAMS 4
#define SPX_RING (2 * SPX_MAX_WALK_STREAMS)
struct SpxStage {
  void* p = nullptr;
  size_t cap = 0;
  hipEvent_t done = nullptr;
  int acquire(size_t bytes);
  int release(hipStream_t on);
  void destroy();
};
struct SpxStagePair {
  SpxStage slot[2];
  int next = 0;
  SpxStage& take() { SpxStage& s = slot[next]; next ^= 1; return s; }
  void destroy() { for (auto& s : slot) s.destroy(); }
};
struct SpxCarve {
  size_t o;
  explicit SpxCarve(size_t base = 0) : o((base + 255) & ~(size_t)255) {}
  size_t take(size_t bytes) { const size_t at = o; o += (bytes + 255) & ~(size_t)255; return at; }
};
struct spx_plan {
  SpxPlanDev dev;
  int device = 0;
  int cu_count = 1;
  size_t lds_per_cu = 65536;
  std::mutex mu;
  SpxStagePair stage;
  struct Trial {
    SpxModeTrial state = {-1, 0, -1};
    hipEvent_t ev[4] = {nullptr, nullptr, nullptr, nullptr};
  } trial;
  std::map<long long, SpxModeResources> res_cache;
  std::map<const void*, int> split_of;
  void* tables = nullptr;
  hipStream_t side = nullptr;
  hipStream_t side2 = nullptr;
  hipEvent_t ev_tension = nullptr;
  hipEvent_t ev_chunk[SPX_MAX_CHUNKS] = {};
  hipEvent_t ev_walk[SPX_RING] = {};
  bool ev_walk_valid[SPX_RING] = {};
  void* ring_ws[SPX_RING] = {};
  hipStream_t ring_st[SPX_RING] = {};
  int ahead_calls = 0;
  hipEvent_t ev_call[2] = {nullptr, nullptr};
  const void* ahead_last_out = nullptr;
  const void* ahead_last_nout = nullptr;
  bool ev_call_valid[2] = {false, false};
  hipStream_t ev_call_st[2] = {nullptr, nullptr};
  std::vector<std::pair<const int*, int>> mixed_started;
  const int* ahead_started = nullptr;
  int ahead_n = 0;
  hipStream_t mix = nullptr;
  hipEvent_t ev_join = nullptr, ev_fork = nullptr, ev_an = nullptr;
  std::mutex mix_mu;
  SpxStagePair mix_stage;
};

struct EvPair { hipEvent_t a, b; int kind; };
extern std::atomic<bool> g_timing;
extern std::atomic<int> g_last_concurrent;
extern std::atomic<int> g_concurrent;
extern std::atomic<int> g_tension_form;
extern std::atomic<int> g_last_tension_form;
extern std::atomic<int> g_last_call_chunks;
extern std::atomic<bool> g_chunks_set;
extern std::atomic<int> g_chunks;
extern std::mutex g_tmu;
extern std::vector<EvPair> g_ev_pending;
extern std::vector<hipEvent_t> g_ev_free;
extern int g_calls_pending;
struct SpxDevGuard {
  std::mutex mu;
  hipEvent_t last = nullptr;
  hipStream_t last_stream = nullptr;
  bool valid = false;
};
extern SpxDevGuard g_guard[64];
struct SpxGuardScope {
  SpxDevGuard& guard;
  std::unique_lock<std::mutex> lock;
  bool idle_start = false;
  explicit SpxGuardScope(int device) : guard(g_guard[(device >= 0 && device < 64) ? device : 0]), lock(guard.mu, std::defer_lock) {}
  template <class Redecide>
  void enter(hipStream_t st, Redecide&& redecide) {
    lock.lock();
    const hipError_t q = guard.valid ? hipEventQuery(guard.last) : hipSuccess;
    (void)hipGetLastError();
    idle_start = (q == hipSuccess);
    if (guard.valid && guard.last_stream != st && q == hipErrorNotReady) {
      redecide();
      lock.unlock();
    }
  }
  int leave_event(hipStream_t st);
};

static inline int64_t frames_for(const SpxPlanDev& d, int64_t n_in) {
  if (n_in < d.W + 1) return 0;
  return (n_in - d.W - 1) / d.B + 1;
}
static inline int64_t spx_map_rows(const SpxPlanDev& d, int64_t n_in, bool nonlinear) { return nonlinear ? n_in / d.B + 1 : 1; }
spx_plan* shared_plan_full(int sample_rate, int match_matlab);

struct Layout {
  size_t off_streams, off_states, off_rec, off_scratch, off_order, off_flags, off_ready, total;
  int64_t max_tiles;
  int64_t total_frames;
};
Layout layout_for(const SpxPlanDev& d, const spx_stream_job* jobs, int n);
int dev_side_streams(int dev, hipStream_t* side, hipStream_t* side2);
int walk_stream_count();
int dev_walk_streams(int dev, hipStream_t* w, int n);
int ring_note(spx_plan* plan, hipStream_t st);
int ring_wait(spx_plan* plan, hipStream_t sa, const void* ws, hipStream_t st, bool* waited_prev);
bool ring_previous_in_flight(spx_plan* plan);
int ring_record(spx_plan* plan, hipStream_t on, void* ws, hipStream_t st, const void* out, const void* n_out, bool detached = false);
SpxModeEnv mode_env();
bool device_ours_cb(void* ctx);
struct SpxSpeedClass { int maxC; bool speedup_only, any_speed; };
SpxSpeedClass speed_class(const spx_stream_job* jobs, int n);
SpxModeWalk mode_walk(const SpxPlanDev& d, const SpxWalkAsk& ask);
void spx_launch_gate(const int* started, int n_walk, unsigned max_spins, hipStream_t st);
struct SpxForce { int concurrent; bool idle_start; int total_streams; hipEvent_t after_analysis; hipStream_t ahead_sa; const int** started_out;
                  bool no_exclusive;
};
struct SpxRateCall {
  std::vector<int64_t> walk_out_off, walk_out_cap;
  std::vector<unsigned char> no_trunc;
  std::vector<int> table;
  SpxRateJob* d_table = nullptr;
  int64_t* d_tsm_n = nullptr;
  const int16_t* tsm_base = nullptr;
  int max_blocks = 1;
};
void spx_launch_map_rate_rows(const SpxRateJob* jobs, const SpxStreamDev* streams, int n_streams, int B, int64_t max_rows,
                              const int64_t* n_out, int64_t* map, hipStream_t hs);
struct SpxRetargetCall {
  std::vector<int> table;
  void* d_table = nullptr;
  const int64_t* n_probe = nullptr;
  float* speeds = nullptr;
};
void spx_launch_retarget(const void* d_table, int n, int copies, const int64_t* n_probe, float* speeds, SpxStreamDev* streams, hipStream_t st);
struct SpxCall {
  spx_plan_t plan;
  const spx_stream_job* jobs;
  int n;
  const int16_t* in;
  int16_t* out;
  int64_t* n_out;
  void* ws;
  size_t ws_bytes;
  const spx_taps* taps;
  void* hs;
};
struct SpxCallOpts {
  bool do_a = true, do_w = true;
  const SpxForce* force = nullptr;
  const SpxRateCall* rate = nullptr;
  int64_t* map = nullptr;
  const SpxEditsCall* edits = nullptr;
  const SpxRetargetCall* retarget = nullptr;
  bool ahead_req = false;
  bool overlap_req = false;
  void* in_ready = nullptr;
  bool split_part = false;
  bool sub = false;
  void* done_event = nullptr;
  bool detached = false;
};
int run_impl(const SpxCall& c, const SpxCallOpts& opt = SpxCallOpts());
SpxModeRuntime mode_runtime(spx_plan* plan);
spx_taps taps_advance(const spx_taps& t, int64_t rows, int64_t spec, int64_t norm);
SpxJobLimits spx_job_limits(spx_plan_t plan);
int spx_check_jobs(spx_plan_t plan, const spx_stream_job* jobs, int n, bool rate_call = false, bool short_window = false, bool device_speeds = false);
int spx_read_steps(const SpxPlanDev& d, const spx_stream_job* jobs, int n, const void* ws, int32_t* steps, hipStream_t st);

void spx_internal_set_error(const char* msg);
int spx_internal_run(const SpxCall& c, bool ahead, bool overlap, void* in_ready, void* done_event, bool detached);
int spx_internal_rate_check(spx_plan_t plan, float rate);
size_t spx_internal_rate_workspace_all(spx_plan_t plan, const spx_stream_job* jobs, int n);
int spx_internal_run_rate(const SpxCall& c, const float* rates, void* in_ready, void* done_event);
int spx_internal_run_mixed(const spx_plan_t* plans, int n_plans, const spx_stream_job* jobs, const int* plan_index, int n, const int16_t* in,
                           int16_t* out, int64_t* n_out, void* ws, size_t ws_bytes, void* hs, bool ahead, void* in_ready,
                           void* done_event, bool detached);
size_t spx_conv_table_bytes(int n);
int spx_conv_table_fill(void* pinned, const spx_stream_job* jobs, int n, int* max_in, int* max_out);
void spx_conv_table_upload(const void* pinned, void* d_tab, int n, hipStream_t st);
void spx_conv_launch_in(const void* d_tab, int n, int max_in, const float* in, int16_t* st_in, hipStream_t st);
void spx_conv_launch_out(const void* d_tab, int n, int max_out, const int64_t* n_out, const int16_t* st_out, float* out, hipStream_t st);
```

speedy_amd/csrc/spx_engine.hip:

```cpp
#include "spx_engine.h"

__attribute__((constructor(101))) static void spx_default_hw_queues() {
  if (getenv("SPX_KEEP_HW_QUEUES") || getenv("GPU_MAX_HW_QUEUES")) return;
  setenv("GPU_MAX_HW_QUEUES", "8", 0);
  if (getenv("SPX_DEBUG_MODE")) fprintf(stderr, "[spx] GPU_MAX_HW_QUEUES was unset: set to 8 at load time (SPX_KEEP_HW_QUEUES=1 leaves the environment alone)\n");
}

thread_local std::string g_spx_err;

std::atomic<bool> g_timing{false};
std::atomic<int> g_last_concurrent{0};
std::atomic<int> g_concurrent{1};
std::atomic<int> g_tension_form{0};
std::atomic<int> g_last_tension_form{SPX_TENSION_POLL};
std::atomic<int> g_last_call_chunks{0};
std::atomic<bool> g_chunks_set{false};
std::atomic<int> g_chunks{1};
std::mutex g_tmu;
std::vector<EvPair> g_ev_pending;
std::vector<hipEvent_t> g_ev_free;
int g_calls_pending = 0;

SpxDevGuard g_guard[64];

int spx_kernel_vgprs(const void* fn, int* scratch_bytes) {
  static std::mutex mu;
  static std::map<const void*, std::pair<int, int>> cache;
  std::lock_guard<std::mutex> g(mu);
  auto it = cache.find(fn);
  if (it == cache.end()) {
    hipFuncAttributes a;
    int regs = 128, scratch = -1;
    if (hipFuncGetAttributes(&a, fn) == hipSuccess) { regs = (a.numRegs + 7) & ~7; scratch = (int)a.localSizeBytes; }
    (void)hipGetLastError();
    it = cache.emplace(fn, std::make_pair(regs, scratch)).first;
  }
  if (scratch_bytes) *scratch_bytes = it->second.second;
  return it->second.first;
}

#include <fcntl.h>
#include <sys/file.h>
#include <unistd.h>
static bool device_is_ours(int dev) {
  static std::mutex mu;
  static int state[64];
  static int lock_fd[64];
  static pid_t owner = 0;
  if (dev < 0 || dev >= 64) return false;
  std::lock_guard<std::mutex> g(mu);
  if (owner != getpid()) {
    for (int d = 0; d < 64; d++) { if (owner && state[d] > 0 && lock_fd[d] > 0) close(lock_fd[d]); state[d] = 0; lock_fd[d] = -1; }
    owner = getpid();
  }
  if (state[dev]) return state[dev] > 0;
  state[dev] = -1;
  if (getenv("SPX_SHARED_GPU")) return false;
  char bus[64] = "dev";
  if (hipDeviceGetPCIBusId(bus, (int)sizeof(bus), dev) != hipSuccess) { (void)hipGetLastError(); snprintf(bus, sizeof(bus), "ordinal%d", dev); }
  for (char* c = bus; *c; c++) if (*c == ':' || *c == '/') *c = '_';
  const char* dir = getenv("SPX_LOCK_DIR");
  if (!dir) dir = "/tmp";
  char path[256];
  snprintf(path, sizeof(path), "%s/spx_concurrent_%s.lock", dir, bus);
  int fd = open(path, O_CREAT | O_RDWR | O_CLOEXEC | O_NOFOLLOW, 0644);
  if (fd < 0) fd = open(path, O_RDONLY | O_CLOEXEC | O_NOFOLLOW);
  if (fd < 0) return false;
  if (flock(fd, LOCK_EX | LOCK_NB) != 0) { close(fd); return false; }
  state[dev] = 1;
  lock_fd[dev] = fd;
  return true;
}


int SpxStage::acquire(size_t bytes) {
  if (done) HIPCHK(hipEventSynchronize(done));
  else HIPCHK(hipEventCreateWithFlags(&done, hipEventDisableTiming));
  if (cap < bytes) {
    if (p) (void)hipHostFree(p);
    p = nullptr; cap = 0;
    const size_t grown = bytes * 2 + 4096;
    HIPCHK(hipHostMalloc(&p, grown, hipHostMallocDefault));
    cap = grown;
  }
  return 0;
}
int SpxStage::release(hipStream_t on) {
  HIPCHK(hipEventRecord(done, on));
  return 0;
}
void SpxStage::destroy() {
  if (done) { (void)hipEventSynchronize(done); (void)hipEventDestroy(done); }
  if (p) (void)hipHostFree(p);
  p = nullptr; cap = 0; done = nullptr;
}
int SpxGuardScope::leave_event(hipStream_t st) {
  if (!guard.last) HIPCHK(hipEventCreateWithFlags(&guard.last, hipEventDisableTiming));
  HIPCHK(hipEventRecord(guard.last, st));
  guard.last_stream = st;
  guard.valid = true;
  return 0;
}

Layout layout_for(const SpxPlanDev& d, const spx_stream_job* jobs, int n) {
  Layout L;
  int64_t tf = 0;
  for (int i = 0; i < n; i++) tf += (jobs[i].nonlinear != 0.0f) ? frames_for(d, jobs[i].n_in) : 0;
  L.total_frames = tf;
  SpxCarve ws;
  L.off_streams = ws.take(sizeof(SpxStreamDev) * (size_t)n * SPX_MAX_CHUNKS);
  L.off_states = ws.take(sizeof(SpxStreamState) * (size_t)n);
  L.off_rec = ws.take(sizeof(SpxFrameRec) * (size_t)(tf + 1));
  L.off_scratch = ws.take(sizeof(float) * 4 * (size_t)(tf + 1));
  const int TFr = std::min(spx_analysis_small_tile_frames(), d.tile_frames > 0 ? d.tile_frames : spx_analysis_small_tile_frames());
  L.max_tiles = tf / TFr + n + 1;
  L.off_order = ws.take(sizeof(int) * (size_t)L.max_tiles);
  L.off_flags = ws.take(sizeof(int) * (size_t)L.max_tiles);
  L.off_ready = ws.take(sizeof(int) * ((size_t)n + 1));
  L.total = ws.o;
  return L;
}


static void build_streams(const SpxPlanDev& d, const spx_stream_job* jobs, int n, int nch,
                          std::vector<SpxStreamDev>& v, std::vector<int>& tiles_per_chunk, const SpxRateCall* rc = nullptr,
                          bool with_map = false, const int64_t* ops_cap = nullptr) {
  v.resize((size_t)n * nch);
  tiles_per_chunk.assign(nch, 0);
  int64_t fo = 0, map_row = 0;
  const int TF = d.tile_frames;
  for (int i = 0; i < n; i++) {
    const spx_stream_job& j = jobs[i];
    const bool nonlinear = j.nonlinear != 0.0f;
    const int64_t Ttot = nonlinear ? frames_for(d, j.n_in) : 0;
    int64_t Tprev = 0;
    for (int c = 0; c < nch; c++) {
      int64_t n_c = j.n_in;
      if (c < nch - 1) n_c = (j.n_in * (c + 1) / nch) / d.B * d.B;
      SpxStreamDev& s = v[(size_t)c * n + i];
      s.in_off = j.in_off; s.n_in = n_c; s.out_off = j.out_off; s.out_cap = j.out_cap;
      s.channels = j.channels; s.speed = j.speed; s.nonlinear = j.nonlinear; s.feedback = j.feedback;
      const int64_t T = nonlinear ? frames_for(d, n_c) : 0;
      s.n_frames = (int32_t)T;
      s.frame_begin = (int32_t)Tprev;
      s.flags = (c == 0 ? SPX_F_INIT : 0) | (c == nch - 1 ? SPX_F_FLUSH : 0);
      if (rc) {
        s.out_off = rc->walk_out_off[i]; s.out_cap = rc->walk_out_cap[i];
        if (rc->no_trunc[i]) s.flags |= SPX_F_NO_TRUNC;
      }
      s.frame_off = fo;
      s.first_tile = tiles_per_chunk[c];
      tiles_per_chunk[c] += (int)((T - Tprev + TF - 1) / TF);
      Tprev = T;
      if (with_map || ops_cap) s.map_row = (int32_t)map_row;
    }
    fo += Ttot;
    map_row += ops_cap ? ops_cap[i] : spx_map_rows(d, j.n_in, nonlinear);
  }
}

static SpxTapsDev taps_of(const spx_taps* t) {
  SpxTapsDev d = {nullptr, nullptr, nullptr, nullptr, nullptr};
  if (t) { d.tension = t->tension; d.speed = t->speed; d.features = t->features;
           d.spectrogram = t->spectrogram; d.normalized = t->normalized; }
  return d;
}

__global__ void spx_gate_kernel(const int* started, int n_walk, unsigned max_spins) {
  if (threadIdx.x == 0) {
    for (unsigned i = 0; i < max_spins; i++) {
      if (__hip_atomic_load(started, __ATOMIC_RELAXED, __HIP_MEMORY_SCOPE_AGENT) >= n_walk) break;
      __builtin_amdgcn_s_sleep(8);
    }
  }
}
void spx_launch_gate(const int* started, int n_walk, unsigned max_spins, hipStream_t st) {
  hipLaunchKernelGGL(spx_gate_kernel, dim3(1), dim3(64), 0, st, started, n_walk, max_spins);
}
__global__ void __launch_bounds__(256)
spx_stage_kernel(const unsigned* __restrict__ src, unsigned* __restrict__ dst_a, unsigned n_a, unsigned* __restrict__ dst_b,
                 unsigned n_b, unsigned* __restrict__ zero_a, unsigned nz_a, unsigned* __restrict__ zero_b, unsigned nz_b,
                 const int* gate_started, int gate_n, unsigned gate_spins) {
  const unsigned stride = gridDim.x * blockDim.x, t0 = blockIdx.x * blockDim.x + threadIdx.x;
  for (unsigned i = t0; i < n_a; i += stride) dst_a[i] = src[i];
  for (unsigned i = t0; i < n_b; i += stride) dst_b[i] = src[n_a + i];
  for (unsigned i = t0; i < nz_a; i += stride) zero_a[i] = 0u;
  for (unsigned i = t0; i < nz_b; i += stride) zero_b[i] = 0u;
  if (gate_started != nullptr && t0 == 0) {
    for (unsigned i = 0; i < gate_spins; i++) {
      if (__hip_atomic_load(gate_started, __ATOMIC_RELAXED, __HIP_MEMORY_SCOPE_AGENT) >= gate_n) break;
      __builtin_amdgcn_s_sleep(8);
    }
  }
}
static hipEvent_t take_event() {
  std::lock_guard<std::mutex> g(g_tmu);
  if (!g_ev_free.empty()) { hipEvent_t e = g_ev_free.back(); g_ev_free.pop_back(); return e; }
  hipEvent_t e;
  (void)hipEventCreate(&e);
  return e;
}
int dev_side_streams(int dev, hipStream_t* side, hipStream_t* side2) {
  static std::mutex mu;
  static hipStream_t s1[64], s2[64];
  const int d = (dev >= 0 && dev < 64) ? dev : 0;
  std::lock_guard<std::mutex> g(mu);
  if (!s1[d]) {
    if (hipStreamCreateWithFlags(&s1[d], hipStreamNonBlocking) != hipSuccess) { s1[d] = nullptr; return -1; }
    if (hipStreamCreateWithFlags(&s2[d], hipStreamNonBlocking) != hipSuccess) { (void)hipStreamDestroy(s1[d]); s1[d] = nullptr; s2[d] = nullptr; return -1; }
  }
  *side = s1[d]; *side2 = s2[d];
  return 0;
}

#ifndef SPX_WALK_STREAMS
#define SPX_WALK_STREAMS 3
#endif
int walk_stream_count() { return SPX_WALK_STREAMS; }
int dev_walk_streams(int dev, hipStream_t* w, int n) {
  static std::mutex mu;
  static hipStream_t s3[64][SPX_MAX_WALK_STREAMS];
  hipStream_t side = nullptr, side2 = nullptr;
  if (dev_side_streams(dev, &side, &side2)) return -1;
  const int d = (dev >= 0 && dev < 64) ? dev : 0;
  std::lock_guard<std::mutex> g(mu);
  w[0] = side2;
  for (int i = 1; i < n && i < SPX_MAX_WALK_STREAMS; i++) {
    if (!s3[d][i] && hipStreamCreateWithFlags(&s3[d][i], hipStreamNonBlocking) != hipSuccess) { s3[d][i] = nullptr; return -1; }
    w[i] = s3[d][i];
  }
  return 0;
}

int ring_note(spx_plan* plan, hipStream_t st) {
  const int cur = plan->ahead_calls & 1;
  if (!plan->ev_call[cur]) HIPCHK(hipEventCreateWithFlags(&plan->ev_call[cur], hipEventDisableTiming));
  HIPCHK(hipEventRecord(plan->ev_call[cur], st));
  plan->ev_call_valid[cur] = true;
  plan->ev_call_st[cur] = st;
  return 0;
}
int ring_wait(spx_plan* plan, hipStream_t sa, const void* ws, hipStream_t st, bool* waited_prev) {
  const int c = plan->ahead_calls % SPX_RING;
  if (waited_prev) *waited_prev = false;
  for (int back = SPX_RING; back >= 1; back--) {
    const int j = (c + SPX_RING - back) % SPX_RING;
    if (!plan->ev_walk_valid[j]) continue;
    if (back > SPX_RING / 2 || plan->ring_ws[j] == ws || plan->ring_st[j] != st) {
      HIPCHK(hipStreamWaitEvent(sa, plan->ev_walk[j], 0));
      if (back == 1 && waited_prev) *waited_prev = true;
    }
  }
  return 0;
}
bool ring_previous_in_flight(spx_plan* plan) {
  const int j = (plan->ahead_calls + SPX_RING - 1) % SPX_RING;
  const bool f = plan->ev_walk_valid[j] && hipEventQuery(plan->ev_walk[j]) == hipErrorNotReady;
  (void)hipGetLastError();
  return f;
}
int ring_record(spx_plan* plan, hipStream_t on, void* ws, hipStream_t st, const void* out, const void* n_out, bool detached) {
  const int c = plan->ahead_calls % SPX_RING;
  if (!plan->ev_walk[c]) HIPCHK(hipEventCreateWithFlags(&plan->ev_walk[c], hipEventDisableTiming));
  HIPCHK(hipEventRecord(plan->ev_walk[c], on));
  if (on != st && !detached) HIPCHK(hipStreamWaitEvent(st, plan->ev_walk[c], 0));
  plan->ev_walk_valid[c] = true;
  plan->ring_ws[c] = ws;
  plan->ring_st[c] = st;
  plan->ahead_last_out = out;
  plan->ahead_last_nout = n_out;
  plan->ahead_calls++;
  return 0;
}

// ... 41 lines not shown
    if (!ok) c.any_speed = false;
  }
  if (c.speedup_only) c.any_speed = false;
  return c;
}
SpxModeWalk mode_walk(const SpxPlanDev& d, const SpxWalkAsk& ask) {
  const SpxWalkConfig c = spx_walk_config(d, ask);
  SpxModeWalk w;
  w.lds = c.lds; w.waves = c.waves; w.fast_kernel = c.fast_kernel; w.nwc = c.nwc;
  w.vgprs = spx_kernel_vgprs(c.kernel.fn);
  return w;
}
static const SpxModeResources& mode_resources(spx_plan* plan, int n, int maxC, bool speedup_only, bool any_speed = false, bool short_window = false) {
  const long long key = ((long long)n << 16) ^ ((long long)maxC << 3) ^ (short_window ? 4 : 0) ^ (any_speed ? 2 : 0) ^ (speedup_only ? 1 : 0);
  auto it = plan->res_cache.find(key);
  if (it != plan->res_cache.end()) return it->second;
  const SpxPlanDev& d = plan->dev;
  SpxModeResources R;
  memset(&R, 0, sizeof(R));
  R.cu_count = plan->cu_count;
  R.lds_per_cu = plan->lds_per_cu;
  R.walk = mode_walk(d, {.n_streams = n, .max_channels = maxC, .speedup_only = speedup_only, .any_speed = any_speed, .short_window = short_window});
  R.walk_lean = R.walk;
  if (maxC == 1 && n <= plan->cu_count && R.walk.fast_kernel && R.walk.nwc > 0) {
    R.walk_lean = mode_walk(d, {.n_streams = n, .max_channels = maxC, .speedup_only = speedup_only, .any_speed = any_speed, .lean = true});
    R.lean_valid = true;
  }
  R.tension_lds = spx_tension_lds_bytes();
  R.tension_vgprs = spx_tension_vgprs();
  R.tile_default = d.tile_frames;
  R.tile_big = spx_analysis_tile_frames();
  R.tile_small = spx_analysis_small_tile_frames();
  SpxPlanDev d8 = d;
  d8.tile_frames = R.tile_small;
  R.an_lds_default = spx_analysis_lds_bytes(d, maxC == 1);
  R.an_vgprs_default = spx_analysis_vgprs(d);
  R.an_lds_small = spx_analysis_lds_bytes(d8, maxC == 1);
  R.an_vgprs_small = spx_analysis_vgprs(d8);
  if (plan->res_cache.size() > 64) plan->res_cache.clear();
  return plan->res_cache.emplace(key, R).first->second;
}
extern "C" int spx_debug_mode_resources(int sample_rate, int channels, int n_streams, int speedup_only, long long* out) {
  spx_plan* plan = shared_plan_full(sample_rate, 0);
  if (!plan || !out || n_streams < 1) return -1;
  std::lock_guard<std::mutex> g(plan->mu);
  const SpxModeResources& R = mode_resources(plan, n_streams, channels < 1 ? 1 : channels, speedup_only != 0, speedup_only == 0);
  const long long v[22] = {R.cu_count, (long long)R.lds_per_cu, (long long)R.walk.lds, R.walk.waves, R.walk.vgprs, R.walk.fast_kernel, R.walk.nwc,
                           (long long)R.walk_lean.lds, R.walk_lean.waves, R.walk_lean.vgprs, R.walk_lean.fast_kernel, R.walk_lean.nwc, R.lean_valid,
                           (long long)R.tension_lds, R.tension_vgprs, R.tile_default, R.tile_big, R.tile_small, (long long)R.an_lds_default,
                           (long long)R.an_lds_small, R.an_vgprs_default, R.an_vgprs_small};
  for (int i = 0; i < 22; i++) out[i] = v[i];
  return 0;
}

static int stage_tables(spx_plan* plan, const std::vector<SpxStreamDev>& sv, const std::vector<int>& order, SpxStreamDev* dstreams,
                        int* d_order, int* d_flags, unsigned n_flags, int* d_ready, unsigned n_ready, hipStream_t on, hipEvent_t* done,
                        const int* gate_started = nullptr, int gate_n = 0, unsigned gate_spins = 0) {
  const size_t b_sv = sizeof(SpxStreamDev) * sv.size(), b_or = sizeof(int) * order.size();
  SpxStage& G = plan->stage.take();
  if (G.acquire(b_sv + b_or)) return -2;
  unsigned char* hp = static_cast<unsigned char*>(G.p);
  memcpy(hp, sv.data(), b_sv);
  if (b_or) memcpy(hp + b_sv, order.data(), b_or);
  hipLaunchKernelGGL(spx_stage_kernel, dim3(64), dim3(256), 0, on, reinterpret_cast<const unsigned*>(hp),
                     reinterpret_cast<unsigned*>(dstreams), (unsigned)(b_sv / 4), reinterpret_cast<unsigned*>(d_order), (unsigned)(b_or / 4),
                     reinterpret_cast<unsigned*>(d_flags), n_flags, reinterpret_cast<unsigned*>(d_ready), n_ready, gate_started, gate_n, gate_spins);
  if (G.release(on)) return -2;
  *done = G.done;
  return 0;
}

struct SpxTimed {
  hipEvent_t a = nullptr, b = nullptr;
  hipStream_t s = nullptr;
  int kind = 0;
  SpxTimed(bool on, int kind_, hipStream_t s_) : s(s_), kind(kind_) {
    if (on) { a = take_event(); b = take_event(); (void)hipEventRecord(a, s); }
  }
  ~SpxTimed() {
    if (!a) return;
    (void)hipEventRecord(b, s);
    std::lock_guard<std::mutex> g(g_tmu);
    g_ev_pending.push_back({a, b, kind});
  }
};

int run_impl(const SpxCall& call, const SpxCallOpts& opt) {
  const auto& [plan, jobs, n, in, out, n_out, ws, ws_bytes, taps, hs] = call;
  const bool do_a = opt.do_a, do_w = opt.do_w;
  const SpxForce* force = opt.force;
  const bool general = opt.rate != nullptr || opt.map != nullptr || opt.edits != nullptr;
  if (spx_check_jobs(plan, jobs, n, general, force && force->no_exclusive, opt.retarget != nullptr)) return -1;
  SpxRange range_(do_a && do_w ? "spx_batch_run" : (do_a ? "spx_batch_analyze" : "spx_batch_walk"));
  SpxPlanDev d = plan->dev;
  Layout L = layout_for(d, jobs, n);
  if (ws_bytes < L.total || !ws) return fail(-1, "spx_batch: workspace too small");
  const SpxSpeedClass SC = speed_class(jobs, n);
  const int maxC = SC.maxC;
  const bool retarget = opt.retarget != nullptr;
  const bool speedup_only = SC.speedup_only && !general && !retarget, any_speed = retarget ? !general : (SC.any_speed && !general);
  std::lock_guard<std::mutex> plan_lock(plan->mu);
  if (!opt.split_part) plan->split_of.erase(ws);
  const bool short_window_res = opt.force && opt.force->no_exclusive;
  const SpxModeResources& R = mode_resources(plan, n, maxC, speedup_only, any_speed, short_window_res);
  hipStream_t st = static_cast<hipStream_t>(hs);
  const SpxModeShape S = mode_shape(n, maxC, L.total_frames > 0, opt);
  SpxModeEnv E = mode_env();
  if (general || retarget) E.concurrent_enabled = false;
  SpxModeRuntime T = mode_runtime(plan);
  const int two_back = (plan->ahead_calls + SPX_RING - 2) % SPX_RING;
  T.two_workspaces = plan->ev_walk_valid[two_back] && plan->ring_ws[two_back] == ws;
  T.trial_key = ((long long)n << 40) ^ ((long long)L.total_frames << 8) ^ (maxC << 3) ^ (any_speed ? 4 : 0) ^ (speedup_only ? 2 : 0) ^ (opt.overlap_req ? 1 : 0);
  spx_plan::Trial& TR = plan->trial;
  if (TR.state.key == T.trial_key && TR.state.choice < 0 && TR.state.calls >= 3 && TR.ev[1] && TR.ev[3] &&
      hipEventQuery(TR.ev[1]) == hipSuccess && hipEventQuery(TR.ev[3]) == hipSuccess)
    T.trial_times_ready = hipEventElapsedTime(&T.ms_seq, TR.ev[0], TR.ev[1]) == hipSuccess &&
                          hipEventElapsedTime(&T.ms_con, TR.ev[2], TR.ev[3]) == hipSuccess;
  (void)hipGetLastError();
  SpxMode M = spx_choose_mode(S, R, E, T, TR.state);
  SpxGuardScope guard(plan->device);
  if (M.want_concurrent && !force)
    guard.enter(st, [&] { T.guard_busy = true; M = spx_choose_mode(S, R, E, T, TR.state); });
  const bool idle_start = force ? force->idle_start : guard.idle_start;
  static const bool dbg_trial = getenv("SPX_DEBUG_TRIAL") != nullptr;
  if (dbg_trial && TR.state.choice < 0 && M.trial_next.choice >= 0 && T.trial_times_ready)
    fprintf(stderr, "[spx trial] n=%d maxC=%d: concurrent %.3f ms, in sequence %.3f ms -> %s\n", n, maxC, T.ms_con, T.ms_seq,
            M.trial_next.choice ? "concurrent" : "sequence");
  TR.state = M.trial_next;
  d.tile_frames = M.tile_frames;
  const int nch = M.nch;
  const bool concurrent = M.concurrent, ahead = M.ahead;
  const bool chunk_ahead = M.chunk_ahead && !force;
  std::vector<SpxStreamDev> sv;
  std::vector<int> tiles;
  build_streams(d, jobs, n, nch, sv, tiles, opt.rate, opt.map != nullptr, opt.edits ? opt.edits->ops_cap : nullptr);
  if (opt.rate && (concurrent || ahead || chunk_ahead || !do_a || !do_w || force)) return fail(-1, "spx_batch_run_rate: internal: not a plain call in sequence");
  if (opt.map && (concurrent || ahead || chunk_ahead || !do_a || !do_w || force)) return fail(-1, "spx_batch_run_map: internal: not a plain call in sequence");
  if (opt.edits && (concurrent || ahead || chunk_ahead || !do_a || !do_w || force || opt.rate || opt.map || retarget))
    return fail(-1, "spx_batch_run_edits: internal: not a plain call in sequence");
  if (retarget && (concurrent || ahead || chunk_ahead || !do_w || force || opt.rate || opt.map || opt.edits || opt.ahead_req || opt.detached))
    return fail(-1, "spx_batch_run_twopass: internal: not a plain call in sequence");
  if (opt.map && (R.walk.fast_kernel || spx_walk_config(d, {.n_streams = n, .max_channels = maxC}).mode != 0))
    return fail(-1, "spx_batch_run_map: internal: no general walk kernel for this batch");
  if (opt.edits && (R.walk.fast_kernel || spx_walk_config(d, {.n_streams = n, .max_channels = maxC}).mode != 0))
    return fail(-1, "spx_batch_run_edits: internal: no general walk kernel for this batch");
  unsigned char* w = static_cast<unsigned char*>(ws);
  SpxStreamDev* dstreams = reinterpret_cast<SpxStreamDev*>(w + L.off_streams);
  SpxStreamState* states = reinterpret_cast<SpxStreamState*>(w + L.off_states);
  SpxFrameRec* rec = reinterpret_cast<SpxFrameRec*>(w + L.off_rec);
  float* scratch = reinterpret_cast<float*>(w + L.off_scratch);
  int* d_order = reinterpret_cast<int*>(w + L.off_order);
  int* d_flags = reinterpret_cast<int*>(w + L.off_flags);
  int* d_ready = reinterpret_cast<int*>(w + L.off_ready);
  SpxTapsDev td = taps_of(taps);
  const bool timed = g_timing.load() && ((do_a && do_w) || retarget);
  if (do_a && do_w) g_last_concurrent.store(concurrent ? 1 : (ahead ? 2 : 0), std::memory_order_relaxed);
  if (do_a && do_w) g_last_call_chunks.store(nch, std::memory_order_relaxed);
  static const bool dbg_mode = getenv("SPX_DEBUG_MODE") != nullptr;
  if (dbg_mode)
    fprintf(stderr, "[spx mode] rate %d n %d maxC %d: co_resident %d doubtful %d lean %d want_concurrent %d chunks %d tiles %d -> %s%s\n",
            d.rate, n, maxC, (int)M.co_resident, (int)M.doubtful, (int)M.launch_lean, (int)M.want_concurrent, nch, tiles[0],
            concurrent ? "concurrent" : (ahead ? (M.seq_ahead ? "ahead (kernels in sequence)" : "ahead") : (chunk_ahead ? "sequence, producers ahead" : "sequence")),
            M.walk2 ? ", walk kernels overlapping" : "");
  hipStream_t stw = st;
  const bool detached = opt.detached && M.walk2 && !force;
  if (do_w && !force && !detached && ring_note(plan, st)) return -2;
  if (do_w && !force && detached) { plan->ev_call_valid[plan->ahead_calls & 1] = false; plan->ev_call_st[plan->ahead_calls & 1] = nullptr; }
  if (M.walk2) {
    hipStream_t wst[SPX_MAX_WALK_STREAMS];
    const int nws = walk_stream_count();
    if (dev_walk_streams(plan->device, wst, nws)) return fail(-1, "spx_batch: no walk streams");
    const int cur = plan->ahead_calls & 1;
    stw = wst[plan->ahead_calls % nws];
    const bool same_out = !opt.sub && (out == plan->ahead_last_out || n_out == plan->ahead_last_nout);
    const bool foreign_prev = !plan->ev_call_valid[cur ^ 1] || plan->ev_call_st[cur ^ 1] != st;
    if (detached) { }
    else if (same_out || (foreign_prev && plan->ahead_calls > 0)) HIPCHK(hipStreamWaitEvent(stw, plan->ev_call[cur], 0));
    else if (plan->ev_call_valid[cur ^ 1]) HIPCHK(hipStreamWaitEvent(stw, plan->ev_call[cur ^ 1], 0));
  }
  hipStream_t sa = st;
  if (nch > 1 || concurrent || ahead) {
    if (!plan->side) {
      if (dev_side_streams(plan->device, &plan->side, &plan->side2)) return fail(-1, "spx_batch: no side streams");
      HIPCHK(hipEventCreateWithFlags(&plan->ev_tension, hipEventDisableTiming));
      for (auto& e : plan->ev_chunk) HIPCHK(hipEventCreateWithFlags(&e, hipEventDisableTiming));
    }
    sa = M.ahead_forced ? force->ahead_sa : plan->side;
  }
  std::vector<int> order;
  if (concurrent) {
    order.reserve((size_t)tiles[0]);
    std::vector<int> cnt(n);
    int maxT = 0;
    for (int i = 0; i < n; i++) {
      cnt[i] = (i + 1 < n ? sv[i + 1].first_tile : tiles[0]) - sv[i].first_tile;
      if (cnt[i] > maxT) maxT = cnt[i];
    }
    for (int t = 0; t < maxT; t++)
      for (int i = 0; i < n; i++)
        if (t < cnt[i]) order.push_back(sv[i].first_tile + t);
  }
  bool waited_prev = false;
  if ((ahead || chunk_ahead) && !force) {
    if (ring_wait(plan, sa, ws, st, &waited_prev)) return -2;
    if (opt.in_ready) HIPCHK(hipStreamWaitEvent(sa, static_cast<hipEvent_t>(opt.in_ready), 0));
  }
  if (!ahead && !chunk_ahead && opt.in_ready) HIPCHK(hipStreamWaitEvent(st, static_cast<hipEvent_t>(opt.in_ready), 0));
  hipEvent_t staged_ev = nullptr;
  const bool ahead_gate = ahead && !force && plan->ahead_started != nullptr && plan->ahead_n > 0 && !waited_prev &&
                          ring_previous_in_flight(plan);
  const std::vector<int>& side_table = opt.rate ? opt.rate->table : (retarget ? opt.retarget->table : order);
  int* const d_side_table = opt.rate ? reinterpret_cast<int*>(opt.rate->d_table) : (retarget ? static_cast<int*>(opt.retarget->d_table) : d_order);
  const int rc = stage_tables(plan, sv, side_table, dstreams, d_side_table, d_flags, concurrent ? (unsigned)tiles[0] : 0u, d_ready,
                    (concurrent || ahead) ? (unsigned)n + 1u : 0u, (ahead || chunk_ahead) ? sa : st, &staged_ev,
                    ahead_gate ? plan->ahead_started : nullptr, plan->ahead_n, 8000u);
  if (rc) return rc;
  if (retarget) spx_launch_retarget(opt.retarget->d_table, n, nch, opt.retarget->n_probe, opt.retarget->speeds, dstreams, st);
  if (M.trial_slot >= 0) {
    hipEvent_t& e0 = TR.ev[2 * M.trial_slot];
    if (!e0) HIPCHK(hipEventCreate(&e0));
    HIPCHK(hipEventRecord(e0, st));
  }
  if (sa != st && !ahead && !chunk_ahead) {
    HIPCHK(hipStreamWaitEvent(sa, staged_ev, 0));
    if (concurrent) HIPCHK(hipStreamWaitEvent(plan->side2, staged_ev, 0));
  }
  for (int c = 0; c < nch; c++) {
    SpxStreamDev* dj = dstreams + (size_t)c * n;
    if (concurrent && do_w && idle_start) spx_launch_gate(d_ready + n, n, 1200u, sa);
    if (do_a && tiles[c] > 0) {
      SpxTimed tm(timed, 0, sa);
      spx_launch_analysis(d, dj, n, tiles[c], in, rec, td, concurrent ? d_order : nullptr, concurrent ? d_flags : nullptr, maxC == 1, sa);
    }
    if (force && force->after_analysis && c == nch - 1) HIPCHK(hipEventRecord(force->after_analysis, sa));
    if (sa != st) HIPCHK(hipEventRecord(plan->ev_chunk[c], sa));
    if (sa != st && !concurrent && !ahead) HIPCHK(hipStreamWaitEvent(st, plan->ev_chunk[c], 0));
    if (do_w) {
      hipStream_t stn = concurrent ? plan->side2 : (ahead ? sa : st);
      {
        SpxTimed tm(timed, 2, stn);
        const int form = (!concurrent && g_tension_form.load(std::memory_order_relaxed) == 0) ? SPX_TENSION_SEQ : SPX_TENSION_POLL;
        g_last_tension_form = spx_launch_tension(d, dj, n, states, rec, scratch, td, concurrent ? d_flags : nullptr, (concurrent || ahead) ? d_ready : nullptr, stn, form);
      }
      if (concurrent || ahead) HIPCHK(hipEventRecord(plan->ev_tension, stn));
      if (ahead) HIPCHK(hipStreamWaitEvent(stw, plan->ev_tension, 0));
      {
        SpxTimed tm(timed, 1, stw);
        const SpxWalkAsk ask = {.n_streams = n, .max_channels = maxC, .speedup_only = speedup_only, .any_speed = any_speed, .lean = M.launch_lean,
                                .short_window = short_window_res || (!force && M.walk2 && !M.launch_lean && maxC > 1)};
        spx_launch_walk(d, ask, dj, in, out, opt.rate ? opt.rate->d_tsm_n : n_out, states, scratch, (concurrent || ahead) ? d_ready : nullptr,
                        (M.exclusive_cu && !(force && force->no_exclusive)) ? R.lds_per_cu / 2 + 1024 : 0, stw, opt.map, opt.edits);
      }
      if (opt.rate && c == nch - 1) {
        SpxTimed tm(timed, 3, stw);
        spx_launch_rate_batch(opt.rate->d_table, n, opt.rate->max_blocks, states, opt.rate->d_tsm_n, opt.rate->tsm_base, out, n_out, stw);
      }
      if (opt.rate && opt.map && c == nch - 1) {
        SpxTimed tm(timed, 4, stw);
        int64_t max_rows = 1;
        for (int i = 0; i < n; i++) max_rows = std::max(max_rows, spx_map_rows(d, jobs[i].n_in, jobs[i].nonlinear != 0.0f));
        spx_launch_map_rate_rows(opt.rate->d_table, dj, n, d.B, max_rows, n_out, opt.map, stw);
      }
      if (M.ahead_forced && force->started_out) *force->started_out = d_ready + n;
      if (c == nch - 1 && !force) {
        if (ring_record(plan, stw, ws, st, out, n_out, detached)) return -2;
        plan->ahead_started = (concurrent || ahead) ? d_ready + n : nullptr;
        plan->ahead_n = n;
        plan->mixed_started.clear();
      }
    }
    if (concurrent) {
      HIPCHK(hipStreamWaitEvent(st, plan->ev_chunk[c], 0));
      HIPCHK(hipStreamWaitEvent(st, plan->ev_tension, 0));
    }
  }
  if (concurrent && !force && guard.leave_event(st)) return -2;
  if (M.trial_slot >= 0) {
    hipEvent_t& e1 = TR.ev[2 * M.trial_slot + 1];
    if (!e1) HIPCHK(hipEventCreate(&e1));
    HIPCHK(hipEventRecord(e1, st));
  }
  if (opt.done_event && do_w) HIPCHK(hipEventRecord(static_cast<hipEvent_t>(opt.done_event), detached ? stw : st));
  if (timed) { std::lock_guard<std::mutex> g(g_tmu); g_calls_pending++; }
  HIPCHK(hipGetLastError());
  return 0;
}

#define SPX_SPLIT_LIMIT 4
struct SplitPlan { int k; std::vector<int> first; std::vector<size_t> ws_off, ws_bytes; size_t total; };
static SplitPlan split_geometry(const spx_plan* plan, const spx_stream_job* jobs, int n, int max_mult) {
  SplitPlan P;
  P.k = 1; P.total = 0;
  const int cu = plan->cu_count > 0 ? plan->cu_count : 1;
  if (max_mult > SPX_SPLIT_LIMIT) max_mult = SPX_SPLIT_LIMIT;
  if (n <= cu || n > max_mult * cu) return P;
  P.k = (n + cu - 1) / cu;
  SpxCarve ws;
  for (int i = 0; i < P.k; i++) {
    const int a = (int)((long long)n * i / P.k), b = (int)((long long)n * (i + 1) / P.k);
    P.first.push_back(a);
    const size_t bytes = layout_for(plan->dev, jobs + a, b - a).total;
    P.ws_off.push_back(ws.take(bytes)); P.ws_bytes.push_back(bytes);
  }
  P.first.push_back(n);
  P.total = ws.o;
  return P;
}
static int run_split(const SpxCall& call, const SpxCallOpts& opt) {
  const auto& [plan, jobs, n, in, out, n_out, ws, ws_bytes, taps, hs] = call;
  if (!plan || !jobs || n <= 0) return fail(-1, "spx_batch: bad arguments");
  SplitPlan P = split_geometry(plan, jobs, n, opt.ahead_req && opt.overlap_req ? 2 : 1);
  if (P.k > 1 && (g_chunks_set.load() || ws_bytes < P.total)) P.k = 1;
  if (P.k > 1) {
    const SpxSpeedClass SC = speed_class(jobs, n);
    const int maxC = SC.maxC;
    std::lock_guard<std::mutex> plan_lock(plan->mu);
    const int m = P.first[1] - P.first[0];
    const SpxModeResources& R = mode_resources(plan, m, maxC, SC.speedup_only, SC.any_speed);
    SpxCallOpts overlapped;
    overlapped.ahead_req = overlapped.overlap_req = true;
    SpxModeRuntime T = mode_runtime(plan);
    T.trial_key = -2;
    const SpxModeTrial none = {-1, 0, -1};
    const SpxMode M = spx_choose_mode(mode_shape(m, maxC, true, overlapped), R, mode_env(), T, none);
    if (!(M.ahead && M.walk2)) P.k = 1;
  }
  if (P.k <= 1) return run_impl(call, opt);
  for (int i = 0; i < P.k; i++)
    if (spx_check_jobs(plan, jobs + P.first[i], P.first[i + 1] - P.first[i])) return -1;
  { std::lock_guard<std::mutex> g(plan->mu); if (plan->split_of.size() > 64) plan->split_of.clear(); plan->split_of[ws] = P.k; }
  int64_t rows = 0;
  for (int i = 0; i < P.k; i++) {
    const int a = P.first[i], m = P.first[i + 1] - a;
    spx_taps t;
    if (taps) {
      t = taps_advance(*taps, rows, rows * (int64_t)plan->dev.N, rows * (int64_t)plan->dev.W);
      for (int j = a; j < a + m; j++) rows += jobs[j].nonlinear != 0.0f ? frames_for(plan->dev, jobs[j].n_in) : 0;
    }
    SpxCallOpts o;
    o.ahead_req = o.overlap_req = true;
    o.split_part = true;
    o.sub = i > 0;
    o.in_ready = opt.in_ready;
    if (i == P.k - 1) o.done_event = opt.done_event;
    const int rc = run_impl({plan, jobs + a, m, in, out, n_out + a, static_cast<unsigned char*>(ws) + P.ws_off[i], P.ws_bytes[i],
                             taps ? &t : nullptr, hs}, o);
    if (rc) return rc;
  }
  return 0;
}

int spx_internal_run(const SpxCall& c, bool ahead, bool overlap, void* in_ready, void* done_event, bool detached) {
  SpxCallOpts o;
  o.ahead_req = ahead; o.overlap_req = overlap; o.in_ready = in_ready; o.done_event = done_event; o.detached = detached;
  return run_split(c, o);
}

SpxJobLimits spx_job_limits(spx_plan_t plan) { return {plan->dev.W, plan->dev.B, spx_internal_analysis_fits(plan->dev)}; }
int spx_check_jobs(spx_plan_t plan, const spx_stream_job* jobs, int n, bool rate_call, bool short_window, bool device_speeds) {
  if (!plan || !jobs || n <= 0) return fail(-1, "spx_batch: bad arguments");
  const SpxJobLimits L = spx_job_limits(plan);
  for (int i = 0; i < n; i++) {
    const SpxJobFault f = spx_check_job(L, jobs[i]);
    if (f != SPX_JOB_OK) return fail(-1, std::string("spx_batch: ") + spx_job_fault_text(f));
  }
  const SpxSpeedClass SC = speed_class(jobs, n);
  std::lock_guard<std::mutex> plan_lock(plan->mu);
  const SpxModeResources& R = mode_resources(plan, n, SC.maxC, SC.speedup_only && !rate_call && !device_speeds,
                                             device_speeds ? !rate_call : (SC.any_speed && !rate_call), short_window);
  if (R.walk.lds > 160 * 1024)
    return fail(-1, "spx_batch: too many channels for the walk kernel's LDS window");
  return 0;
}

extern "C" {
size_t spx_batch_workspace_bytes(spx_plan_t plan, const spx_stream_job* jobs, int n_streams) {
  if (!plan || !jobs || n_streams < 1) return 0;
  return std::max(layout_for(plan->dev, jobs, n_streams).total, split_geometry(plan, jobs, n_streams, SPX_SPLIT_LIMIT).total);
}
int spx_batch_run(spx_plan_t plan, const spx_stream_job* jobs, int n, const int16_t* in, int16_t* out,
                  int64_t* n_out, void* ws, size_t ws_bytes, const spx_taps* taps, void* hs) {
  return run_split({plan, jobs, n, in, out, n_out, ws, ws_bytes, taps, hs}, SpxCallOpts());
}
int spx_batch_run_ahead(spx_plan_t plan, const spx_stream_job* jobs, int n, const int16_t* in, int16_t* out,
                        int64_t* n_out, void* ws, size_t ws_bytes, const spx_taps* taps, void* hs) {
  return spx_internal_run({plan, jobs, n, in, out, n_out, ws, ws_bytes, taps, hs}, true, false, nullptr, nullptr, false);
}
int spx_batch_run_overlapped(spx_plan_t plan, const spx_stream_job* jobs, int n, const int16_t* in, int16_t* out,
                             int64_t* n_out, void* ws, size_t ws_bytes, const spx_taps* taps, void* hs) {
  return spx_internal_run({plan, jobs, n, in, out, n_out, ws, ws_bytes, taps, hs}, true, true, nullptr, nullptr, false);
}
int spx_batch_run_ahead_when(spx_plan_t plan, const spx_stream_job* jobs, int n, const int16_t* in, int16_t* out,
                             int64_t* n_out, void* ws, size_t ws_bytes, const spx_taps* taps, void* hs, void* in_ready_event) {
  return spx_internal_run({plan, jobs, n, in, out, n_out, ws, ws_bytes, taps, hs}, true, false, in_ready_event, nullptr, false);
}
int spx_batch_analyze(spx_plan_t plan, const spx_stream_job* jobs, int n, const int16_t* in, void* ws,
                      size_t ws_bytes, const spx_taps* taps, void* hs) {
  SpxCallOpts o;
  o.do_w = false;
  return run_impl({plan, jobs, n, in, nullptr, nullptr, ws, ws_bytes, taps, hs}, o);
}
int spx_batch_walk(spx_plan_t plan, const spx_stream_job* jobs, int n, const int16_t* in, int16_t* out,
                   int64_t* n_out, void* ws, size_t ws_bytes, const spx_taps* taps, void* hs) {
  SpxCallOpts o;
  o.do_a = false;
  return run_impl({plan, jobs, n, in, out, n_out, ws, ws_bytes, taps, hs}, o);
}

}

static int rate_ratio(int sample_rate, float rate, int* old_rate, int* new_rate) {
  if (!(rate > 0.0f) || !std::isfinite(rate)) return fail(-1, "sonicSetRate: rate must be finite and > 0");
  const float q = sample_rate / rate;
  if (!(q < 2147483520.0f)) return fail(-1, "sonicSetRate: rate too small for this sample rate");
  int o = sample_rate, w = (int)q;
  while (w > (1 << 14) || o > (1 << 14)) { w >>= 1; o >>= 1; }
  if (w < 1) return fail(-1, "sonicSetRate: rate too large for this sample rate");
  if (o < 1) return fail(-1, "sonicSetRate: rate too small for this sample rate");
  *old_rate = o; *new_rate = w;
  return 0;
}
static int64_t rate_frames(int64_t m, int old_rate, int new_rate) {
  return m >= 2 ? ((m - 1) * (int64_t)new_rate + old_rate - 1) / old_rate : 0;
}
struct RateLayout { size_t off_table, off_tsm_n, off_tsm, total; std::vector<int64_t> tsm_off, tsm_cap; };
static void rate_layout(spx_plan_t plan, const spx_stream_job* jobs, const float* rates, int n, RateLayout& RL) {
  SpxCarve ws(spx_batch_workspace_bytes(plan, jobs, n));
  RL.off_table = ws.take(sizeof(SpxRateJob) * (size_t)n);
  RL.off_tsm_n = ws.take(sizeof(int64_t) * (size_t)n);
  RL.off_tsm = ws.o;
  RL.tsm_off.assign(n, 0); RL.tsm_cap.assign(n, 0);
  int64_t v = 0;
  for (int i = 0; i < n; i++) {
    if (rates && rates[i] == 1.0f) continue;
    RL.tsm_off[i] = v;
    RL.tsm_cap[i] = spx_internal_out_bound(plan->dev, jobs[i].n_in, jobs[i].speed, jobs[i].nonlinear != 0.0f);
    v += (RL.tsm_cap[i] * jobs[i].channels + 7) & ~(int64_t)7;
  }
  RL.total = ws.o + sizeof(int16_t) * (size_t)v + 128;
}
static int rate_call_build(const SpxCall& call, const float* rates, SpxRateCall& RC, bool* any_out) {
  const auto& [plan, jobs, n, in, out, n_out, ws, ws_bytes, taps, hs] = call;
  bool any = false;
  std::vector<int> oldR(n, 1), newR(n, 1);
  if (rates)
    for (int i = 0; i < n; i++) {
      if (rate_ratio(plan->dev.rate, rates[i], &oldR[i], &newR[i])) return -1;
      any = any || rates[i] != 1.0f;
    }
  *any_out = any;
  if (!any) return 0;
  if (!in || !out || !n_out || !ws || (reinterpret_cast<uintptr_t>(out) & 1)) return fail(-1, "spx_batch_run_rate: bad arguments");
  if (spx_check_jobs(plan, jobs, n, true)) return -1;
  RateLayout RL;
  rate_layout(plan, jobs, rates, n, RL);
  if (ws_bytes < RL.total) return fail(-1, "spx_batch_run_rate: workspace too small (spx_batch_workspace_bytes_rate)");
  unsigned char* w = static_cast<unsigned char*>(ws);
  RC.d_table = reinterpret_cast<SpxRateJob*>(w + RL.off_table);
  RC.d_tsm_n = reinterpret_cast<int64_t*>(w + RL.off_tsm_n);
  RC.tsm_base = reinterpret_cast<const int16_t*>(w + RL.off_tsm);
  const int64_t tsm_from_out = (int64_t)((reinterpret_cast<intptr_t>(RC.tsm_base) - reinterpret_cast<intptr_t>(out)) / (intptr_t)sizeof(int16_t));
  RC.walk_out_off.resize(n); RC.walk_out_cap.resize(n); RC.no_trunc.resize(n);
  std::vector<SpxRateJob> tab((size_t)n);
  memset(tab.data(), 0, sizeof(SpxRateJob) * (size_t)n);
  for (int i = 0; i < n; i++) {
    const bool resample = rates[i] != 1.0f;
    SpxRateJob& J = tab[i];
    J.fin_off = jobs[i].out_off; J.fin_cap = jobs[i].out_cap;
    J.channels = jobs[i].channels; J.old_rate = oldR[i]; J.new_rate = newR[i]; J.rate = rates[i];
    J.bypass = resample ? 0 : 1;
    J.tsm_off = RL.tsm_off[i]; J.tsm_cap = RL.tsm_cap[i];
    J.n_blocks = 1;
    if (resample && jobs[i].out_cap > 0) J.n_blocks = spx_rate_batch_blocks(std::min(jobs[i].out_cap, rate_frames(J.tsm_cap, J.old_rate, J.new_rate)), J.channels);
    if (J.n_blocks > RC.max_blocks) RC.max_blocks = J.n_blocks;
    RC.no_trunc[i] = resample ? 1 : 0;
    RC.walk_out_off[i] = resample ? tsm_from_out + RL.tsm_off[i] : jobs[i].out_off;
    RC.walk_out_cap[i] = resample ? RL.tsm_cap[i] : jobs[i].out_cap;
  }
  static_assert(sizeof(SpxRateJob) % sizeof(int) == 0, "the staging kernel copies 32-bit words");
  RC.table.resize(sizeof(SpxRateJob) / sizeof(int) * (size_t)n);
  memcpy(RC.table.data(), tab.data(), sizeof(SpxRateJob) * (size_t)n);
  return 0;
}
int spx_internal_rate_check(spx_plan_t plan, float rate) {
  int o = 1, w = 1;
  return plan ? rate_ratio(plan->dev.rate, rate, &o, &w) : fail(-1, "spx_batch: bad arguments");
}
size_t spx_internal_rate_workspace_all(spx_plan_t plan, const spx_stream_job* jobs, int n) {
  if (spx_check_jobs(plan, jobs, n, true)) return 0;
  RateLayout RL;
  rate_layout(plan, jobs, nullptr, n, RL);
  return RL.total;
}
int spx_internal_run_rate(const SpxCall& c, const float* rates, void* in_ready, void* done_event) {
  if (!c.plan || !c.jobs || c.n <= 0) return fail(-1, "spx_batch: bad arguments");
// ... 86 lines not shown
```

speedy_amd/csrc/spx_internal.h:

```cpp
#pragma once
#include <hip/hip_runtime.h>
#include <stdint.h>

#include <stdlib.h>
#include <type_traits>


#define SPX_FAST_MAX_SPEED 1.0e18f

#define SPX_MAX_STAGES 16
#define SPX_WAVE 64
#define SPX_BLOCK 256
#define SPX_FEATURE_COUNT 15

struct SpxPlanDev {
  int rate;
  int B;
  int W;
  int N;
  int F;
  int Pp;
  int nstages;
  int radix[SPX_MAX_STAGES];
  int minPeriod, maxPeriod, maxRequired, skip;
  int tile_frames;
  int dft_waves;
  float alpha;
  float one_minus_alpha;
  const double* tw;
  const double* tw2;
  const float* window;
  const float* taperF;
  const float* taperP;
  int rader;
  int nstagesM;
  int radixM[SPX_MAX_STAGES];
  const double* twM;
  const double* bfft;
  const int* perm;
  const int* iperm;
  const int* qlog;
  const void* lane_consts;
};
#ifdef SPX_PREEMPH_V1
#define SPX_WIN_SCALE 1.0f
#else
#define SPX_WIN_SCALE 0x1p-15f
#endif
#define SPX_LC_W1 0
#define SPX_LC_W2 3
#define SPX_LC_W3 6
#define SPX_LC_WU 10
#define SPX_LC_WN 14
#define SPX_LC_ENTRIES 15
#define SPX_LC_BYTES (SPX_LC_ENTRIES * 64 * 16)
void spx_lane_consts_fill(const double* tw, const double* tw2, const float* win, unsigned char* out);

#define SPX_F_INIT 1
#define SPX_F_FLUSH 2
#define SPX_F_TENSION_RANGE 4
#define SPX_F_NO_SPEED 8
#define SPX_F_NO_TRUNC 16
#define SPX_F_SPEED_SET 32
#define SPX_F_KEEP_SPEED 64
#define SPX_F_HANDED_IN 128
struct SpxStreamDev {
  int64_t in_off, n_in, out_off, out_cap;
  int64_t frame_off;
  int32_t n_frames;
  int32_t frame_begin;
  int32_t channels;
  int32_t flags;
  float speed, nonlinear, feedback;
  int32_t first_tile;
  int64_t tsm_shift;
  int32_t tension_skip;
  int32_t unit_time0;
  int32_t tension_to;
  int32_t handed_in;
  int32_t ring_bufs;
  int32_t map_row;
};

struct SpxWalkState {
  int64_t base;
  int64_t out_n;
  int64_t avail;
  int remaining;
  int prevPeriod, prevMinDiff;
  int overflow;
  int prevPeriod_toggle;
  int steps;
};
struct SpxStreamState {
  SpxWalkState w;
  float lp;
  float lpf;
  float cur_dur;
  float des_dur;
  float curSpeed;
  int handed;
  int flush_remaining;
  int flush_out_mark;
  int tension_first;
  int pad2_;
};

#define SPX_RATE_MAX_CHANNELS 16
struct SpxRateState {
  int64_t tsm_seen;
  int64_t final_n;
  int32_t old_pos, new_pos;
  int32_t has_left;
  int32_t overflow;
  int16_t left[SPX_RATE_MAX_CHANNELS];
};
void spx_launch_rate(SpxRateState* rs, const SpxStreamState* st, const int64_t* tsm_n, const int16_t* tsm, int16_t* fin,
                     int64_t fin_cap, int channels, int old_rate, int new_rate, float rate, int bypass, int flush,
                     hipStream_t hs);

struct SpxRateJob {
  int64_t tsm_off;
  int64_t tsm_cap;
  int64_t fin_off;
  int64_t fin_cap;
  int32_t channels;
  int32_t old_rate, new_rate;
  int32_t bypass;
  float rate;
  int32_t n_blocks;
  int64_t pad_;
};
int spx_rate_batch_blocks(int64_t frames, int channels);
void spx_launch_rate_batch(const SpxRateJob* jobs, int n_streams, int max_blocks, const SpxStreamState* states, const int64_t* tsm_n,
                           const int16_t* tsm_base, int16_t* fin_base, int64_t* n_out, hipStream_t hs);

struct SpxFrameRec {
  float energy;
  float lsd;
};

struct SpxTapsDev {
  float* tension;
  float* speed;
  float* features;
  float* spectrogram;
  float* normalized;
};

void spx_launch_analysis(const SpxPlanDev& P, const SpxStreamDev* streams, int n_streams, int n_tiles,
                         const int16_t* in, SpxFrameRec* rec, SpxTapsDev taps, const int* tile_order, int* tile_flags,
                         bool mono, hipStream_t st);
void spx_launch_analysis_frames(const SpxPlanDev& P, const SpxStreamDev* streams, int n_tiles, const float* frames,
                                bool preemph, SpxFrameRec* rec, SpxTapsDev taps, hipStream_t st);
#define SPX_TENSION_POLL 0
#define SPX_TENSION_SEQ 1
int spx_launch_tension(const SpxPlanDev& P, const SpxStreamDev* streams, int n_streams, SpxStreamState* states,
                       const SpxFrameRec* rec, float* scratch, SpxTapsDev taps, const int* tile_flags, int* speed_ready,
                       hipStream_t st, int form = SPX_TENSION_POLL);
void spx_launch_tension_seq(const SpxPlanDev& P, const SpxStreamDev* streams, int n_streams, SpxStreamState* states,
                            const SpxFrameRec* rec, float* scratch, SpxTapsDev taps, int* speed_ready, hipStream_t st);
bool spx_tension_seq_serves(const SpxPlanDev& P);
struct SpxKernelChoice {
  const char* name;
  const void* fn;
  int block;
  int n_targs;
  int targs[5];
};
using SpxAnalysisArgs = void(SpxPlanDev, const SpxStreamDev*, int, const int16_t*, SpxFrameRec*, SpxTapsDev, const int*, int*, const float*, int);
using SpxWalkArgs = void(SpxPlanDev, const SpxStreamDev*, const int16_t*, int16_t*, int64_t*, SpxStreamState*, const float*, int, const int*);
using SpxWalkMapArgs = void(SpxPlanDev, const SpxStreamDev*, const int16_t*, int16_t*, int64_t*, SpxStreamState*, const float*, int, const int*, int64_t*);
using SpxWalkEditsArgs = void(SpxPlanDev, const SpxStreamDev*, const int16_t*, int16_t*, int64_t*, SpxStreamState*, const float*, int, const int*, int4*, int64_t*, int);
using SpxWalkFastArgs =void(SpxPlanDev, const SpxStreamDev*, const int16_t*, int16_t*, int64_t*, SpxStreamState*, const float*, const int*, int);
template <typename F> struct SpxLaunch;
template <typename... P> struct SpxLaunch<void(P...)> {
  static void go(const SpxKernelChoice& k, int grid, size_t lds, hipStream_t st, P... p) {
    void* args[] = {&p...};
    (void)hipLaunchKernel(k.fn, dim3(grid), dim3(k.block), args, lds, st);
  }
};
struct SpxWalkAsk {
  int n_streams = 0;
  int max_channels = 1;
  bool speedup_only = false;
  bool any_speed = false;
  bool short_jobs = false;
  bool lean = false;
  bool short_window = false;
};
struct SpxEditsCall {
  void* ops;
  const int64_t* ops_cap;
  int64_t* n_ops;
  int64_t total;
};
void spx_launch_walk(const SpxPlanDev& P, const SpxWalkAsk& ask, const SpxStreamDev* streams, const int16_t* in, int16_t* out,
                     int64_t* n_out, SpxStreamState* states, const float* scratch, const int* speed_ready, size_t lds_min,
                     hipStream_t st, int64_t* map = nullptr, const SpxEditsCall* edits = nullptr);
size_t spx_analysis_lds_bytes(const SpxPlanDev& P, bool mono);
int spx_analysis_ct_window(const SpxPlanDev& P);
void spx_host_dft(int n, const int* radix, int nstages, const double* tw, const double* in, double* out);
size_t spx_walk_lds_bytes(const SpxPlanDev& P, int max_channels, bool speedup_only);
struct SpxWalkConfig {
  int mode;
  bool fast_kernel;
  int nw;
  int nwm, nwc, wcap;
  int waves;
  size_t lds;
  bool slow;
  SpxKernelChoice kernel;
};
SpxWalkConfig spx_walk_config(const SpxPlanDev& P, const SpxWalkAsk& ask);
SpxKernelChoice spx_walk_select(int nw, int mode);
SpxKernelChoice spx_walk_map_select(int nw);
SpxKernelChoice spx_walk_edits_select(int nw);
size_t spx_walk_fast_lds_bytes(const SpxPlanDev& P, int wcap);
bool spx_walk_fast_supports(const SpxPlanDev& P, int nwm);
SpxKernelChoice spx_walk_fast_select(const SpxPlanDev& P, int nwm, int nwc, int wcap, int max_channels, bool slow);
SpxKernelChoice spx_analysis_select(int tile_frames, int ct_window);
#define SPX_NOUT_LOST_PRODUCER INT64_MIN
size_t spx_tension_lds_bytes();
int spx_kernel_vgprs(const void* fn, int* scratch_bytes = nullptr);
int spx_tension_vgprs();
int spx_analysis_vgprs(const SpxPlanDev& P, int* scratch_bytes = nullptr);
int spx_walk_vgprs(const SpxPlanDev& P, const SpxWalkAsk& ask, int* scratch_bytes);
void spx_launch_speed_from_tension(SpxStreamState* state, float tension, float Rg, float feedback, float* speed_out,
                                   hipStream_t st);
int spx_analysis_tile_frames();
int spx_analysis_small_tile_frames();
int spx_analysis_tiny_tile_frames();
int spx_analysis_prefers_small_tile(const SpxPlanDev& P);

struct spx_plan;
int64_t spx_internal_out_bound(const SpxPlanDev& P, int64_t n_in, float speed, bool nonlinear);
const SpxPlanDev* spx_internal_shared_plan(int sample_rate, int match_matlab);
bool spx_internal_analysis_fits(const SpxPlanDev& d);
int64_t spx_internal_frames_for(const SpxPlanDev& d, int64_t n_in);
```

Baseline: 51040.

## Share seam frame magnitudes between adjacent analysis tiles via global flags

Adds a 'seam' mode to the lean analysis kernel. Each tile publishes its last frame's spectral magnitudes to a global seam buffer with an agent-scope flag. The next tile spins, with a bounded spin count, to pick that row up instead of recomputing its overlapping halo frame, and falls back to computing it if the wait times out. Wave 0 is reordered to do the seam frame first, and the workspace gains seam counters and rows. The cost is inter-workgroup spinning, extra global traffic, and the risk of stalls when producer tiles are not yet resident.

```diff
diff --git a/include/speedy_hip.h b/include/speedy_hip.h
--- a/include/speedy_hip.h
+++ b/include/speedy_hip.h
@@ -169,6 +169,10 @@
 void spx_set_concurrent(int on);
 void spx_set_tension_form(int form);
 int spx_debug_last_tension_form(void);
+void spx_set_analysis_seam(int on);
+int spx_debug_last_analysis_seam(void);
+void spx_set_analysis_seam_spins(unsigned spins);
+long long spx_debug_seam_fallbacks(const void* workspace);
 int spx_debug_last_call_chunks(void);
 int spx_debug_last_lookup_grid(int* launches);
 int spx_debug_last_replay_grid(int* launches);
diff --git a/speedy_amd/_lib.py b/speedy_amd/_lib.py
--- a/speedy_amd/_lib.py
+++ b/speedy_amd/_lib.py
@@ -107,6 +107,10 @@
     "spx_set_concurrent": (None, [C.c_int]),
     "spx_set_tension_form": (None, [C.c_int]),
     "spx_debug_last_tension_form": (C.c_int, []),
+    "spx_set_analysis_seam": (None, [C.c_int]),
+    "spx_debug_last_analysis_seam": (C.c_int, []),
+    "spx_set_analysis_seam_spins": (None, [C.c_uint]),
+    "spx_debug_seam_fallbacks": (C.c_longlong, [C.c_void_p]),
     "spx_debug_last_call_chunks": (C.c_int, []),
     "spx_debug_last_lookup_grid": (C.c_int, [C.POINTER(C.c_int)]),
     "spx_debug_last_replay_grid": (C.c_int, [C.POINTER(C.c_int)]),
diff --git a/speedy_amd/csrc/spx_analysis.hip b/speedy_amd/csrc/spx_analysis.hip
--- a/speedy_amd/csrc/spx_analysis.hip
+++ b/speedy_amd/csrc/spx_analysis.hip
@@ -443,6 +443,9 @@
 #ifndef SPX_AN_W_BIG
 #define SPX_AN_W_BIG 2
 #endif
+#define SPX_AN_MODE_MASK 3
+#define SPX_AN_SEAM 4
+#define SPX_AN_SPINS_SHIFT 3
 template <int TF, int WCT>
 __global__ void __launch_bounds__(SPX_BLOCK, an_lean_layout(TF, WCT) ? 5 : (WCT == 240 || WCT == 120 || WCT == 180) ? 4 : WCT == 330 ? SPX_AN_W_330 : (WCT == 661 || WCT == 720) ? SPX_AN_W_BIG : (WCT == 480 || WCT == 360) ? 2 : 1)
 spx_analysis_kernel(SpxPlanDev P, const SpxStreamDev* __restrict__ streams, int n_streams,
@@ -483,7 +486,8 @@
   const double* ltw = P.tw;
   const double* ltw2 = P.tw2;
   short* smono = reinterpret_cast<short*>(LT ? lds + an_lt_front_bytes() + wb : lds + wb + mags_b + small_b);
-  const bool direct = LT && frame_mode == 3;
+  const bool direct = LT && (frame_mode & SPX_AN_MODE_MASK) == 3;
+  const bool seam = LT && (frame_mode & SPX_AN_SEAM) != 0;
 
   double* bufA = work + (size_t)wave * (WCT != 0 ? 2 : 4) * W;
   double* bufB = (WCT != 0) ? bufA : bufA + 2 * W;
@@ -491,7 +495,7 @@
   const int jfirst = (j0 > 0) ? j0 - 1 : 0;
   const int64_t sbase = (int64_t)jfirst * B;
   const int nstage = (j1 - jfirst) * B + (W - B);
-  if (frames != nullptr || direct) {
+  if ((frames != nullptr && !seam) || direct) {
   } else if (C == 1) {
     const int16_t* __restrict__ src = in + sbase;
     for (int k0 = tid; k0 < nstage; k0 += 8 * SPX_BLOCK) {
@@ -527,144 +531,203 @@
     };
     int nx[6] = {0, 0, 0, 0, 0, 0};
     float hold[4] = {0.0f, 0.0f, 0.0f, 0.0f};
-    if (direct) fetch6(wave, nx);
-    for (int s = wave; s <= TF; s += 4) {
+    typedef __attribute__((address_space(1))) unsigned* seam_u32;
+    typedef const __attribute__((address_space(1))) float* seam_f32;
+    const bool seam_take = seam && tile > S.first_tile;
+    const int wv = __builtin_amdgcn_readfirstlane(wave);
+    constexpr int SEAM_END = TF + 1;
+    float halo[4];
+    bool halo_here = false;
+    bool halo_lost = false;
+    int s = (wv == 0) ? TF : wv;
+    if (direct) fetch6(s, nx);
+    auto do_slot = [&](const int s, const int sn) __attribute__((always_inline)) {
       const int j = j0 - 1 + s;
-      const bool keep = s + 4 > TF;
+      const bool keep = s >= SPX_LT_FRONT_ROWS;
       float* mrow = mags + (size_t)s * MS;
       if (j < 0 || j >= j1) {
         if (!keep) for (int k = lane; k < 240; k += SPX_WAVE) mrow[k] = 0.0f;
-#pragma unroll
-        for (int u = 0; u < 4; u++) hold[u] = 0.0f;
-        if (direct) fetch6(s + 4, nx);
-        continue;
-      }
-      int ln = lane;
-      asm volatile("" : "+v"(ln));
-      __builtin_assume(ln >= 0 && ln < SPX_WAVE);
-      const lc_ptr lcb[4] = {(lc_ptr)per_frame(lc0), (lc_ptr)per_frame(lc0 + 256), (lc_ptr)per_frame(lc0 + 512), (lc_ptr)per_frame(lc0 + 768)};
-      typedef const __attribute__((address_space(1))) unsigned char* lc_bytes;
-      unsigned lane_off = 16u * (unsigned)lane;
-      asm volatile("" : "+v"(lane_off));
-      auto lc = [&](int c) -> double2 {
-        const lc_v2d v = *(lc_ptr)((lc_bytes)lcb[c >> 2] + lane_off + 1024u * (unsigned)(c & 3));
-        return make_double2(v.x, v.y);
-      };
-      int m[6];
-      if (direct) {
-#pragma unroll
-        for (int u = 0; u < 6; u++) m[u] = nx[u];
+        else {
+#pragma unroll
+          for (int u = 0; u < 4; u++) hold[u] = 0.0f;
+        }
+        if (direct) fetch6(sn, nx);
       } else {
-        take6(smono + (size_t)(j - jfirst) * B + 2 * bb, j, m);
-      }
-      {
-        const lc_v4f wn = *(lc_ptr4)((lc_bytes)lcb[SPX_LC_WN >> 2] + lane_off + 1024u * (SPX_LC_WN & 3));
-        const double2 w1a = lc(SPX_LC_W1 + 0), w1b = lc(SPX_LC_W1 + 1), w1c = lc(SPX_LC_W1 + 2);
-        if (on60) {
-          const double d0 = (double)m[0], d2 = (double)m[2];
-          const cplx a0 = {spx_preemph_win(d0, (double)m[4], wn.x), spx_preemph_win((double)m[1], d0, wn.y)},
-                     a1 = {spx_preemph_win(d2, (double)m[5], wn.z), spx_preemph_win((double)m[3], d2, wn.w)};
-          const cplx b0 = {a0.r + a1.r, a0.i + a1.i}, b2 = {a0.r - a1.r, a0.i - a1.i};
-          const cplx b1 = {a0.r + a1.i, a0.i - a1.r}, b3 = {a0.r - a1.i, a0.i + a1.r};
-          st(bufA, 4 * ln, b0);
-          st(bufA, 4 * ln + 1, cmul_tw(b1, w1a));
-          st(bufA, 4 * ln + 2, cmul_tw(b2, w1b));
-          st(bufA, 4 * ln + 3, cmul_tw(b3, w1c));
-        }
-      }
-      {
-        const double2 w2a = lc(SPX_LC_W2 + 0), w2b = lc(SPX_LC_W2 + 1), w2c = lc(SPX_LC_W2 + 2);
+        int ln = lane;
+        asm volatile("" : "+v"(ln));
+        __builtin_assume(ln >= 0 && ln < SPX_WAVE);
+        const lc_ptr lcb[4] = {(lc_ptr)per_frame(lc0), (lc_ptr)per_frame(lc0 + 256), (lc_ptr)per_frame(lc0 + 512), (lc_ptr)per_frame(lc0 + 768)};
+        typedef const __attribute__((address_space(1))) unsigned char* lc_bytes;
+        unsigned lane_off = 16u * (unsigned)lane;
+        asm volatile("" : "+v"(lane_off));
+        auto lc = [&](int c) -> double2 {
+          const lc_v2d v = *(lc_ptr)((lc_bytes)lcb[c >> 2] + lane_off + 1024u * (unsigned)(c & 3));
+          return make_double2(v.x, v.y);
+        };
+        int m[6];
+        if (direct) {
+#pragma unroll
+          for (int u = 0; u < 6; u++) m[u] = nx[u];
+        } else {
+          take6(smono + (size_t)(j - jfirst) * B + 2 * bb, j, m);
+        }
+        {
+          const lc_v4f wn = *(lc_ptr4)((lc_bytes)lcb[SPX_LC_WN >> 2] + lane_off + 1024u * (SPX_LC_WN & 3));
+          const double2 w1a = lc(SPX_LC_W1 + 0), w1b = lc(SPX_LC_W1 + 1), w1c = lc(SPX_LC_W1 + 2);
+          if (on60) {
+            const double d0 = (double)m[0], d2 = (double)m[2];
+            const cplx a0 = {spx_preemph_win(d0, (double)m[4], wn.x), spx_preemph_win((double)m[1], d0, wn.y)},
+                       a1 = {spx_preemph_win(d2, (double)m[5], wn.z), spx_preemph_win((double)m[3], d2, wn.w)};
+            const cplx b0 = {a0.r + a1.r, a0.i + a1.i}, b2 = {a0.r - a1.r, a0.i - a1.i};
+            const cplx b1 = {a0.r + a1.i, a0.i - a1.r}, b3 = {a0.r - a1.i, a0.i + a1.r};
+            st(bufA, 4 * ln, b0);
+            st(bufA, 4 * ln + 1, cmul_tw(b1, w1a));
+            st(bufA, 4 * ln + 2, cmul_tw(b2, w1b));
+            st(bufA, 4 * ln + 3, cmul_tw(b3, w1c));
+          }
+        }
+        {
+          const double2 w2a = lc(SPX_LC_W2 + 0), w2b = lc(SPX_LC_W2 + 1), w2c = lc(SPX_LC_W2 + 2);
+          wave_sync();
+          ASTAMP(0);
+          if (on60) {
+            const cplx a0 = ld(bufA, ln), a1 = ld(bufA, ln + 60), a2 = ld(bufA, ln + 120), a3 = ld(bufA, ln + 180);
+            wave_sync();
+            const cplx t0 = {a0.r + a2.r, a0.i + a2.i}, t1 = {a0.r - a2.r, a0.i - a2.i};
+            const cplx t2 = {a1.r + a3.r, a1.i + a3.i}, t3 = {a1.r - a3.r, a1.i - a3.i};
+            const cplx b0 = {t0.r + t2.r, t0.i + t2.i}, b2 = {t0.r - t2.r, t0.i - t2.i};
+            const cplx b1 = {t1.r + t3.i, t1.i - t3.r}, b3 = {t1.r - t3.i, t1.i + t3.r};
+            const int o = (ln & 3) + 16 * (ln >> 2);
+            st(bufB, o, b0);
+            st(bufB, o + 4, cmul_tw(b1, w2a));
+            st(bufB, o + 8, cmul_tw(b2, w2b));
+            st(bufB, o + 12, cmul_tw(b3, w2c));
+          }
+        }
+        {
+          double2 w3[2][2];
+#pragma unroll
+          for (int u = 0; u < 2; u++) { w3[u][0] = lc(SPX_LC_W3 + 2 * u); w3[u][1] = lc(SPX_LC_W3 + 2 * u + 1); }
+          wave_sync();
+          cplx q0[2], q1[2], q2[2];
+#pragma unroll
+          for (int u = 0; u < 2; u++) {
+            const int b3i = (ln + 64 * u < 80) ? ln + 64 * u : 0;
+            q0[u] = ld(bufB, b3i); q1[u] = ld(bufB, b3i + 80); q2[u] = ld(bufB, b3i + 160);
+          }
+          wave_sync();
+#pragma unroll
+          for (int u = 0; u < 2; u++) {
+            const int b3i = ln + 64 * u;
+            if (b3i < 80) {
+              const cplx a0 = q0[u], a1 = q1[u], a2 = q2[u];
+              const cplx t1 = {a1.r + a2.r, a1.i + a2.i};
+              const cplx t2 = {spx_bf3h(a0.r, t1.r), spx_bf3h(a0.i, t1.i)};
+              const cplx t3 = {S3_1 * (a1.r - a2.r), S3_1 * (a1.i - a2.i)};
+              const cplx b0 = {a0.r + t1.r, a0.i + t1.i};
+              const cplx b1 = {t2.r + t3.i, t2.i - t3.r}, b2 = {t2.r - t3.i, t2.i + t3.r};
+              const int o = (b3i & 15) + 48 * (b3i >> 4);
+              st(bufA, o, b0);
+              st(bufA, o + 16, cmul_tw(b1, w3[u][0]));
+              st(bufA, o + 32, cmul_tw(b2, w3[u][1]));
+            }
+          }
+        }
         wave_sync();
-        ASTAMP(0);
-        if (on60) {
-          const cplx a0 = ld(bufA, ln), a1 = ld(bufA, ln + 60), a2 = ld(bufA, ln + 120), a3 = ld(bufA, ln + 180);
+        if (on48) {
+          const cplx a0 = ld(bufA, ln), a1 = ld(bufA, ln + 48), a2 = ld(bufA, ln + 96), a3 = ld(bufA, ln + 144),
+                     a4 = ld(bufA, ln + 192);
           wave_sync();
-          const cplx t0 = {a0.r + a2.r, a0.i + a2.i}, t1 = {a0.r - a2.r, a0.i - a2.i};
-          const cplx t2 = {a1.r + a3.r, a1.i + a3.i}, t3 = {a1.r - a3.r, a1.i - a3.i};
-          const cplx b0 = {t0.r + t2.r, t0.i + t2.i}, b2 = {t0.r - t2.r, t0.i - t2.i};
-          const cplx b1 = {t1.r + t3.i, t1.i - t3.r}, b3 = {t1.r - t3.i, t1.i + t3.r};
-          const int o = (ln & 3) + 16 * (ln >> 2);
-          st(bufB, o, b0);
-          st(bufB, o + 4, cmul_tw(b1, w2a));
-          st(bufB, o + 8, cmul_tw(b2, w2b));
-          st(bufB, o + 12, cmul_tw(b3, w2c));
-        }
-      }
-      {
-        double2 w3[2][2];
-#pragma unroll
-        for (int u = 0; u < 2; u++) { w3[u][0] = lc(SPX_LC_W3 + 2 * u); w3[u][1] = lc(SPX_LC_W3 + 2 * u + 1); }
+          const cplx t1 = {a1.r + a4.r, a1.i + a4.i}, t2 = {a2.r + a3.r, a2.i + a3.i};
+          const cplx t3 = {a1.r - a4.r, a1.i - a4.i}, t4 = {a2.r - a3.r, a2.i - a3.i};
+          const cplx b0 = {(a0.r + t1.r) + t2.r, (a0.i + t1.i) + t2.i};
+          const cplx m1 = {spx_bf5m(a0.r, C5_1, t1.r, C5_2, t2.r), spx_bf5m(a0.i, C5_1, t1.i, C5_2, t2.i)};
+          const cplx m2 = {spx_bf5m(a0.r, C5_2, t1.r, C5_1, t2.r), spx_bf5m(a0.i, C5_2, t1.i, C5_1, t2.i)};
+          const cplx n1 = {spx_bf5n(S5_1, t3.r, S5_2, t4.r), spx_bf5n(S5_1, t3.i, S5_2, t4.i)};
+          const cplx n2 = {spx_bf5d(S5_2, t3.r, S5_1, t4.r), spx_bf5d(S5_2, t3.i, S5_1, t4.i)};
+          const cplx b1 = {m1.r + n1.i, m1.i - n1.r}, b4 = {m1.r - n1.i, m1.i + n1.r};
+          const cplx b2 = {m2.r + n2.i, m2.i - n2.r}, b3 = {m2.r - n2.i, m2.i + n2.r};
+          st(bufB, ln, b0);
+          st(bufB, ln + 48, b1);
+          st(bufB, ln + 96, b2);
+          st(bufB, ln + 144, b3);
+          st(bufB, ln + 192, b4);
+        }
+        if (direct) fetch6(sn, nx);
+        double2 wu[4];
+#pragma unroll
+        for (int u = 0; u < 4; u++) wu[u] = lc(SPX_LC_WU + u);
         wave_sync();
-        cplx q0[2], q1[2], q2[2];
-#pragma unroll
-        for (int u = 0; u < 2; u++) {
-          const int b3i = (ln + 64 * u < 80) ? ln + 64 * u : 0;
-          q0[u] = ld(bufB, b3i); q1[u] = ld(bufB, b3i + 80); q2[u] = ld(bufB, b3i + 160);
+        ASTAMP(1);
+        float* spec_out = taps.spectrogram ? taps.spectrogram + (size_t)(S.frame_off + j) * 480 : nullptr;
+#pragma unroll
+        for (int u = 0; u < 4; u++) {
+          const int k = ln + 64 * u;
+          if (k < 240) {
+            const int k2 = (k == 0) ? 0 : 240 - k;
+            const cplx a = ld(bufB, k), c = ld(bufB, k2);
+            const double b_r = c.r, b_i = -c.i;
+            const float mag = spx_untangle_mag(a.r, a.i, b_r, b_i, wu[u]);
+            if (keep) hold[u] = mag;
+            else mrow[k] = mag;
+            if (spec_out) {
+              spec_out[k] = mag;
+              if (k > 0) spec_out[480 - k] = mag;
+              else spec_out[240] = (float)__builtin_fabs(a.r - a.i);
+            }
+          }
         }
         wave_sync();
-#pragma unroll
-        for (int u = 0; u < 2; u++) {
-          const int b3i = ln + 64 * u;
-          if (b3i < 80) {
-            const cplx a0 = q0[u], a1 = q1[u], a2 = q2[u];
-            const cplx t1 = {a1.r + a2.r, a1.i + a2.i};
-            const cplx t2 = {spx_bf3h(a0.r, t1.r), spx_bf3h(a0.i, t1.i)};
-            const cplx t3 = {S3_1 * (a1.r - a2.r), S3_1 * (a1.i - a2.i)};
-            const cplx b0 = {a0.r + t1.r, a0.i + t1.i};
-            const cplx b1 = {t2.r + t3.i, t2.i - t3.r}, b2 = {t2.r - t3.i, t2.i + t3.r};
-            const int o = (b3i & 15) + 48 * (b3i >> 4);
-            st(bufA, o, b0);
-            st(bufA, o + 16, cmul_tw(b1, w3[u][0]));
-            st(bufA, o + 32, cmul_tw(b2, w3[u][1]));
-          }
-        }
-      }
-      wave_sync();
-      if (on48) {
-        const cplx a0 = ld(bufA, ln), a1 = ld(bufA, ln + 48), a2 = ld(bufA, ln + 96), a3 = ld(bufA, ln + 144),
-                   a4 = ld(bufA, ln + 192);
-        wave_sync();
-        const cplx t1 = {a1.r + a4.r, a1.i + a4.i}, t2 = {a2.r + a3.r, a2.i + a3.i};
-        const cplx t3 = {a1.r - a4.r, a1.i - a4.i}, t4 = {a2.r - a3.r, a2.i - a3.i};
-        const cplx b0 = {(a0.r + t1.r) + t2.r, (a0.i + t1.i) + t2.i};
-        const cplx m1 = {spx_bf5m(a0.r, C5_1, t1.r, C5_2, t2.r), spx_bf5m(a0.i, C5_1, t1.i, C5_2, t2.i)};
-        const cplx m2 = {spx_bf5m(a0.r, C5_2, t1.r, C5_1, t2.r), spx_bf5m(a0.i, C5_2, t1.i, C5_1, t2.i)};
-        const cplx n1 = {spx_bf5n(S5_1, t3.r, S5_2, t4.r), spx_bf5n(S5_1, t3.i, S5_2, t4.i)};
-        const cplx n2 = {spx_bf5d(S5_2, t3.r, S5_1, t4.r), spx_bf5d(S5_2, t3.i, S5_1, t4.i)};
-        const cplx b1 = {m1.r + n1.i, m1.i - n1.r}, b4 = {m1.r - n1.i, m1.i + n1.r};
-        const cplx b2 = {m2.r + n2.i, m2.i - n2.r}, b3 = {m2.r - n2.i, m2.i + n2.r};
-        st(bufB, ln, b0);
-        st(bufB, ln + 48, b1);
-        st(bufB, ln + 96, b2);
-        st(bufB, ln + 144, b3);
-        st(bufB, ln + 192, b4);
-      }
-      if (direct) fetch6(s + 4, nx);
-      double2 wu[4];
-#pragma unroll
-      for (int u = 0; u < 4; u++) wu[u] = lc(SPX_LC_WU + u);
-      wave_sync();
-      ASTAMP(1);
-      float* spec_out = taps.spectrogram ? taps.spectrogram + (size_t)(S.frame_off + j) * 480 : nullptr;
-#pragma unroll
-      for (int u = 0; u < 4; u++) {
-        const int k = ln + 64 * u;
-        if (k < 240) {
-          const int k2 = (k == 0) ? 0 : 240 - k;
-          const cplx a = ld(bufB, k), c = ld(bufB, k2);
-          const double b_r = c.r, b_i = -c.i;
-          const float mag = spx_untangle_mag(a.r, a.i, b_r, b_i, wu[u]);
-          hold[u] = mag;
-          if (!keep) mrow[k] = mag;
-          if (spec_out) {
-            spec_out[k] = mag;
-            if (k > 0) spec_out[480 - k] = mag;
-            else spec_out[240] = (float)__builtin_fabs(a.r - a.i);
-          }
-        }
-      }
-      wave_sync();
-      ASTAMP(2);
+        ASTAMP(2);
+      }
+    };
+    for (;;) {
+      const int sn = (wv == 0) ? (s == TF ? (seam_take ? 4 : 0) : (s == 0 ? 4 : (s + 4 < TF ? s + 4 : SEAM_END)))
+                               : (s + 4 <= TF ? s + 4 : SEAM_END);
+      do_slot(s, sn);
+      const bool give = seam && wv == 0 && s == TF && j0 + TF < T;
+      const bool take = seam_take && wv == 3 && sn == SEAM_END;
+      if (give || take) {
+        int sj0 = j0, slo = lo, smode = frame_mode;
+        long long sfo = S.frame_off;
+        int* sflags = tile_flags;
+        float* seam_rows = const_cast<float*>(frames);
+        asm volatile("" : "+s"(sj0), "+s"(slo), "+s"(smode), "+s"(sfo), "+s"(sflags), "+s"(seam_rows));
+        seam_u32 const seam_words = (seam_u32)sflags;
+        const size_t at = (size_t)(sfo >> 4) + (size_t)slo + (size_t)((sj0 - 1 + (give ? TF : 0)) >> 4);
+        if (give) {
+          seam_u32 row = (seam_u32)seam_rows + at * 240;
+#pragma unroll
+          for (int u = 0; u < 4; u++) {
+            const int k = lane + 64 * u;
+            if (k < 240) __hip_atomic_store(row + k, __builtin_bit_cast(unsigned, hold[u]), __ATOMIC_RELAXED, __HIP_MEMORY_SCOPE_AGENT);
+          }
+          asm volatile("s_waitcnt vmcnt(0)" ::: "memory");
+          if (lane == 0) __hip_atomic_store(seam_words + SPX_SEAM_HDR + at, 1u, __ATOMIC_RELAXED, __HIP_MEMORY_SCOPE_AGENT);
+        } else {
+          const unsigned spins = (unsigned)smode >> SPX_AN_SPINS_SHIFT;
+          int seen = 0;
+          for (unsigned i = 0; i < spins; i++) {
+            if (__hip_atomic_load(seam_words + SPX_SEAM_HDR + at, __ATOMIC_RELAXED, __HIP_MEMORY_SCOPE_AGENT) != 0u) { seen = 1; break; }
+            __builtin_amdgcn_s_sleep(32);
+          }
+          halo_here = __builtin_amdgcn_readfirstlane(seen) != 0;
+          if (halo_here) {
+            __builtin_amdgcn_fence(__ATOMIC_ACQUIRE, "agent");
+            seam_f32 row = (seam_f32)seam_rows + at * 240;
+#pragma unroll
+            for (int u = 0; u < 4; u++) {
+              const int k = lane + 64 * u;
+              halo[u] = row[k < 240 ? k : 0];
+            }
+          } else {
+            if (lane == 0) __hip_atomic_fetch_add(seam_words, 1u, __ATOMIC_RELAXED, __HIP_MEMORY_SCOPE_AGENT);
+            halo_lost = true;
+          }
+        }
+      }
+      if (sn == SEAM_END) break;
+      s = sn;
     }
     __syncthreads();
     {
@@ -674,6 +737,17 @@
         const int k = lane + 64 * u;
         if (k < 240) mrow[k] = hold[u];
       }
+    }
+    if (halo_here) {
+#pragma unroll
+      for (int u = 0; u < 4; u++) {
+        const int k = lane + 64 * u;
+        if (k < 240) mags[k] = halo[u];
+      }
+    }
+    if (halo_lost) {
+      if (direct) fetch6(0, nx);
+      do_slot(0, SEAM_END);
     }
   } else if constexpr (WCT == 240) {
     const double2* twp = reinterpret_cast<const double2*>(P.tw);
@@ -1467,7 +1541,7 @@
     write_rec(tid, lsd);
   }
   }
-  if (tile_flags) {
+  if (tile_flags && !seam) {
     asm volatile("s_waitcnt vmcnt(0)" ::: "memory");
     __syncthreads();
     if (tid == 0) {
@@ -1561,14 +1635,24 @@
   return spx_kernel_vgprs(spx_analysis_select(P.tile_frames, plan_ct_window(P)).fn, scratch_bytes);
 }
 
-void spx_launch_analysis(const SpxPlanDev& P, const SpxStreamDev* streams, int n_streams, int n_tiles,
-                         const int16_t* in, SpxFrameRec* rec, SpxTapsDev taps, const int* tile_order, int* tile_flags,
-                         bool mono, hipStream_t st) {
-  if (n_tiles <= 0) return;
+bool spx_analysis_seam_serves(const SpxPlanDev& P) { return an_lean_layout(P.tile_frames, plan_ct_window(P)); }
+int spx_launch_analysis(const SpxPlanDev& P, const SpxStreamDev* streams, int n_streams, int n_tiles,
+                        const int16_t* in, SpxFrameRec* rec, SpxTapsDev taps, const int* tile_order, int* tile_flags,
+                        bool mono, hipStream_t st, const SpxSeam* seam) {
+  if (n_tiles <= 0) return 0;
   const int ctw = plan_ct_window(P);
   const bool direct = mono && an_lean_layout(P.tile_frames, ctw);
+  const bool take = seam && seam->words && seam->rows && an_lean_layout(P.tile_frames, ctw) && !tile_order && !tile_flags;
+  if (take) {
+    const unsigned spins = seam->spins < SPX_SEAM_MAX_SPINS ? seam->spins : SPX_SEAM_MAX_SPINS;
+    SpxLaunch<SpxAnalysisArgs>::go(spx_analysis_select(P.tile_frames, ctw), n_tiles, analysis_lds_bytes(P, ctw, direct), st, P, streams,
+                                   n_streams, in, rec, taps, nullptr, reinterpret_cast<int*>(seam->words), seam->rows,
+                                   (direct ? 3 : 0) | SPX_AN_SEAM | (int)(spins << SPX_AN_SPINS_SHIFT));
+    return 1;
+  }
   SpxLaunch<SpxAnalysisArgs>::go(spx_analysis_select(P.tile_frames, ctw), n_tiles, analysis_lds_bytes(P, ctw, direct), st, P, streams,
                                  n_streams, in, rec, taps, tile_order, tile_flags, nullptr, direct ? 3 : 0);
+  return 0;
 }
 
 void spx_launch_analysis_frames(const SpxPlanDev& P, const SpxStreamDev* streams, int n_tiles, const float* frames,
diff --git a/speedy_amd/csrc/spx_diag.hip b/speedy_amd/csrc/spx_diag.hip
--- a/speedy_amd/csrc/spx_diag.hip
+++ b/speedy_amd/csrc/spx_diag.hip
@@ -68,6 +68,27 @@
 void spx_set_concurrent(int on) { g_concurrent = on != 0; }
 void spx_set_tension_form(int form) { g_tension_form = form != 0; }
 int spx_debug_last_tension_form(void) { return g_last_tension_form.load(std::memory_order_relaxed); }
+void spx_set_analysis_seam(int on) { g_analysis_seam = on != 0; }
+int spx_debug_last_analysis_seam(void) { return g_last_analysis_seam.load(std::memory_order_relaxed); }
+void spx_set_analysis_seam_spins(unsigned spins) { g_analysis_seam_spins = spins < SPX_SEAM_MAX_SPINS ? spins : SPX_SEAM_MAX_SPINS; }
+long long spx_debug_seam_fallbacks(const void* workspace) {
+  std::vector<const unsigned*> counters;
+  {
+    std::lock_guard<std::mutex> g(g_seam_mu);
+    auto it = g_seam_counters.find(workspace);
+    if (it != g_seam_counters.end()) counters = it->second;
+    if (!workspace) for (auto& e : g_seam_counters) counters.insert(counters.end(), e.second.begin(), e.second.end());
+  }
+  if (counters.empty()) return 0;
+  if (hipDeviceSynchronize() != hipSuccess) return -1;
+  long long sum = 0;
+  for (const unsigned* c : counters) {
+    unsigned v = 0;
+    if (hipMemcpy(&v, c, sizeof(v), hipMemcpyDeviceToHost) != hipSuccess) return -1;
+    sum += v;
+  }
+  return sum;
+}
 int spx_debug_last_call_chunks(void) { return g_last_call_chunks.load(std::memory_order_relaxed); }
 void spx_set_pipeline_chunks(int chunks) { g_chunks_set = true; g_chunks = chunks < 1 ? 1 : (chunks > SPX_MAX_CHUNKS ? SPX_MAX_CHUNKS : chunks); }
 static double g_last_tension_ms = 0.0, g_last_rate_ms = 0.0, g_last_map_rows_ms = 0.0, g_last_dtw_ms = 0.0, g_last_dtw_tail_ms = 0.0;
diff --git a/speedy_amd/csrc/spx_engine.h b/speedy_amd/csrc/spx_engine.h
--- a/speedy_amd/csrc/spx_engine.h
+++ b/speedy_amd/csrc/spx_engine.h
@@ -119,6 +119,12 @@
 extern std::atomic<int> g_concurrent;
 extern std::atomic<int> g_tension_form;
 extern std::atomic<int> g_last_tension_form;
+extern std::atomic<int> g_analysis_seam;
+extern std::atomic<unsigned> g_analysis_seam_spins;
+extern std::atomic<int> g_last_analysis_seam;
+void spx_seam_note(const void* owner, const unsigned* counter, bool first);
+extern std::mutex g_seam_mu;
+extern std::map<const void*, std::vector<const unsigned*>> g_seam_counters;
 extern std::atomic<int> g_last_call_chunks;
 extern std::atomic<bool> g_chunks_set;
 extern std::atomic<int> g_chunks;
@@ -160,10 +166,32 @@
 spx_plan* shared_plan_full(int sample_rate, int match_matlab);
 
 struct Layout {
-  size_t off_streams, off_states, off_rec, off_scratch, off_order, off_flags, off_ready, total;
+  size_t off_streams, off_states, off_rec, off_scratch, off_order, off_flags, off_ready, off_seam, off_seam_rows, total;
   int64_t max_tiles;
   int64_t total_frames;
-};
+  size_t seam_places;
+};
+static inline Layout spx_carve_layout(const SpxPlanDev& d, const spx_stream_job* jobs, int n, int small_tile) {
+  Layout L;
+  int64_t tf = 0;
+  for (int i = 0; i < n; i++) tf += (jobs[i].nonlinear != 0.0f) ? frames_for(d, jobs[i].n_in) : 0;
+  L.total_frames = tf;
+  SpxCarve ws;
+  L.off_streams = ws.take(sizeof(SpxStreamDev) * (size_t)n * SPX_MAX_CHUNKS);
+  L.off_states = ws.take(sizeof(SpxStreamState) * (size_t)n);
+  L.off_rec = ws.take(sizeof(SpxFrameRec) * (size_t)(tf + 1));
+  L.off_scratch = ws.take(sizeof(float) * 4 * (size_t)(tf + 1));
+  const int TFr = std::min(small_tile, d.tile_frames > 0 ? d.tile_frames : small_tile);
+  L.max_tiles = tf / TFr + n + 1;
+  L.off_order = ws.take(sizeof(int) * (size_t)L.max_tiles);
+  L.off_flags = ws.take(sizeof(int) * (size_t)L.max_tiles);
+  L.off_ready = ws.take(sizeof(int) * ((size_t)n + 1));
+  L.seam_places = d.W == 240 ? spx_seam_places(tf, n) : 0;
+  L.off_seam = ws.take(L.seam_places ? sizeof(unsigned) * (SPX_SEAM_HDR + L.seam_places) : 0);
+  L.off_seam_rows = ws.take(sizeof(float) * 240 * L.seam_places);
+  L.total = ws.o;
+  return L;
+}
 Layout layout_for(const SpxPlanDev& d, const spx_stream_job* jobs, int n);
 int dev_side_streams(int dev, hipStream_t* side, hipStream_t* side2);
 int walk_stream_count();
@@ -223,6 +251,7 @@
   void* in_ready = nullptr;
   bool split_part = false;
   bool sub = false;
+  const void* ws_owner = nullptr;
   void* done_event = nullptr;
   bool detached = false;
 };
diff --git a/speedy_amd/csrc/spx_engine.hip b/speedy_amd/csrc/spx_engine.hip
--- a/speedy_amd/csrc/spx_engine.hip
+++ b/speedy_amd/csrc/spx_engine.hip
@@ -13,6 +13,18 @@
 std::atomic<int> g_concurrent{1};
 std::atomic<int> g_tension_form{0};
 std::atomic<int> g_last_tension_form{SPX_TENSION_POLL};
+std::atomic<int> g_analysis_seam{1};
+std::atomic<unsigned> g_analysis_seam_spins{64};
+std::atomic<int> g_last_analysis_seam{0};
+std::mutex g_seam_mu;
+std::map<const void*, std::vector<const unsigned*>> g_seam_counters;
+void spx_seam_note(const void* owner, const unsigned* counter, bool first) {
+  std::lock_guard<std::mutex> g(g_seam_mu);
+  if (g_seam_counters.size() > 256 && !g_seam_counters.count(owner)) g_seam_counters.clear();
+  std::vector<const unsigned*>& v = g_seam_counters[owner];
+  if (first) v.clear();
+  if (counter) v.push_back(counter);
+}
 std::atomic<int> g_last_call_chunks{0};
 std::atomic<bool> g_chunks_set{false};
 std::atomic<int> g_chunks{1};
@@ -102,24 +114,7 @@
   return 0;
 }
 
-Layout layout_for(const SpxPlanDev& d, const spx_stream_job* jobs, int n) {
-  Layout L;
-  int64_t tf = 0;
-  for (int i = 0; i < n; i++) tf += (jobs[i].nonlinear != 0.0f) ? frames_for(d, jobs[i].n_in) : 0;
-  L.total_frames = tf;
-  SpxCarve ws;
-  L.off_streams = ws.take(sizeof(SpxStreamDev) * (size_t)n * SPX_MAX_CHUNKS);
-  L.off_states = ws.take(sizeof(SpxStreamState) * (size_t)n);
-  L.off_rec = ws.take(sizeof(SpxFrameRec) * (size_t)(tf + 1));
-  L.off_scratch = ws.take(sizeof(float) * 4 * (size_t)(tf + 1));
-  const int TFr = std::min(spx_analysis_small_tile_frames(), d.tile_frames > 0 ? d.tile_frames : spx_analysis_small_tile_frames());
-  L.max_tiles = tf / TFr + n + 1;
-  L.off_order = ws.take(sizeof(int) * (size_t)L.max_tiles);
-  L.off_flags = ws.take(sizeof(int) * (size_t)L.max_tiles);
-  L.off_ready = ws.take(sizeof(int) * ((size_t)n + 1));
-  L.total = ws.o;
-  return L;
-}
+Layout layout_for(const SpxPlanDev& d, const spx_stream_job* jobs, int n) { return spx_carve_layout(d, jobs, n, spx_analysis_small_tile_frames()); }
 
 
 static void build_streams(const SpxPlanDev& d, const spx_stream_job* jobs, int n, int nch,
@@ -467,6 +462,12 @@
   int* d_order = reinterpret_cast<int*>(w + L.off_order);
   int* d_flags = reinterpret_cast<int*>(w + L.off_flags);
   int* d_ready = reinterpret_cast<int*>(w + L.off_ready);
+  SpxSeam seam = {reinterpret_cast<unsigned*>(w + L.off_seam), reinterpret_cast<float*>(w + L.off_seam_rows),
+                  g_analysis_seam_spins.load(std::memory_order_relaxed)};
+  const bool use_seam = do_a && !concurrent && L.seam_places > 0 && g_analysis_seam.load(std::memory_order_relaxed) != 0 &&
+                        spx_analysis_seam_serves(d);
+  if (do_a) spx_seam_note(opt.ws_owner ? opt.ws_owner : ws, use_seam ? seam.words : nullptr, !opt.sub);
+  int seam_form = 0;
   SpxTapsDev td = taps_of(taps);
   const bool timed = g_timing.load() && ((do_a && do_w) || retarget);
   if (do_a && do_w) g_last_concurrent.store(concurrent ? 1 : (ahead ? 2 : 0), std::memory_order_relaxed);
@@ -526,7 +527,9 @@
                           ring_previous_in_flight(plan);
   const std::vector<int>& side_table = opt.rate ? opt.rate->table : (retarget ? opt.retarget->table : order);
   int* const d_side_table = opt.rate ? reinterpret_cast<int*>(opt.rate->d_table) : (retarget ? static_cast<int*>(opt.retarget->d_table) : d_order);
-  const int rc = stage_tables(plan, sv, side_table, dstreams, d_side_table, d_flags, concurrent ? (unsigned)tiles[0] : 0u, d_ready,
+  if (use_seam && L.seam_places + SPX_SEAM_HDR > 0xffffffffull) return fail(-1, "spx_batch: internal: more seam places than the staging kernel clears");
+  const int rc = stage_tables(plan, sv, side_table, dstreams, d_side_table, use_seam ? reinterpret_cast<int*>(seam.words) : d_flags,
+                    use_seam ? (unsigned)(SPX_SEAM_HDR + L.seam_places) : (concurrent ? (unsigned)tiles[0] : 0u), d_ready,
                     (concurrent || ahead) ? (unsigned)n + 1u : 0u, (ahead || chunk_ahead) ? sa : st, &staged_ev,
                     ahead_gate ? plan->ahead_started : nullptr, plan->ahead_n, 8000u);
   if (rc) return rc;
@@ -545,8 +548,10 @@
     if (concurrent && do_w && idle_start) spx_launch_gate(d_ready + n, n, 1200u, sa);
     if (do_a && tiles[c] > 0) {
       SpxTimed tm(timed, 0, sa);
-      spx_launch_analysis(d, dj, n, tiles[c], in, rec, td, concurrent ? d_order : nullptr, concurrent ? d_flags : nullptr, maxC == 1, sa);
-    }
+      seam_form |= spx_launch_analysis(d, dj, n, tiles[c], in, rec, td, concurrent ? d_order : nullptr, concurrent ? d_flags : nullptr, maxC == 1, sa,
+                                       use_seam ? &seam : nullptr);
+    }
+    if (do_a && c == nch - 1) g_last_analysis_seam.store(seam_form, std::memory_order_relaxed);
     if (force && force->after_analysis && c == nch - 1) HIPCHK(hipEventRecord(force->after_analysis, sa));
     if (sa != st) HIPCHK(hipEventRecord(plan->ev_chunk[c], sa));
     if (sa != st && !concurrent && !ahead) HIPCHK(hipStreamWaitEvent(st, plan->ev_chunk[c], 0));
@@ -656,6 +661,7 @@
     o.ahead_req = o.overlap_req = true;
     o.split_part = true;
     o.sub = i > 0;
+    o.ws_owner = ws;
     o.in_ready = opt.in_ready;
     if (i == P.k - 1) o.done_event = opt.done_event;
     const int rc = run_impl({plan, jobs + a, m, in, out, n_out + a, static_cast<unsigned char*>(ws) + P.ws_off[i], P.ws_bytes[i],
diff --git a/speedy_amd/csrc/spx_internal.h b/speedy_amd/csrc/spx_internal.h
--- a/speedy_amd/csrc/spx_internal.h
+++ b/speedy_amd/csrc/spx_internal.h
@@ -148,9 +148,18 @@
   float* normalized;
 };
 
-void spx_launch_analysis(const SpxPlanDev& P, const SpxStreamDev* streams, int n_streams, int n_tiles,
-                         const int16_t* in, SpxFrameRec* rec, SpxTapsDev taps, const int* tile_order, int* tile_flags,
-                         bool mono, hipStream_t st);
+#define SPX_SEAM_HDR 64
+#define SPX_SEAM_MAX_SPINS (1u << 20)
+struct SpxSeam {
+  unsigned* words;
+  float* rows;
+  unsigned spins;
+};
+static inline size_t spx_seam_places(int64_t total_frames, int n_streams) { return (size_t)(total_frames >> 4) + (size_t)n_streams + 1; }
+bool spx_analysis_seam_serves(const SpxPlanDev& P);
+int spx_launch_analysis(const SpxPlanDev& P, const SpxStreamDev* streams, int n_streams, int n_tiles,
+                        const int16_t* in, SpxFrameRec* rec, SpxTapsDev taps, const int* tile_order, int* tile_flags,
+                        bool mono, hipStream_t st, const SpxSeam* seam = nullptr);
 void spx_launch_analysis_frames(const SpxPlanDev& P, const SpxStreamDev* streams, int n_tiles, const float* frames,
                                 bool preemph, SpxFrameRec* rec, SpxTapsDev taps, hipStream_t st);
 #define SPX_TENSION_POLL 0
```

Result: no change. 51380 (median of 6 runs) (+0.7%).
